# ViTAE-Transformer/LeMeViT

Measured on AMD Instinct MI355X. Metric: images/sec LeMeViT-Base 224^2 bf16 fwd+bwd, higher is better.
Workload: dtype bf16; 1 GPU; lemevit_base 224x224 bf16-autocast train step (fwd+bwd+AdamW), batch 128/GPU, drop_path 0.1, random-init weights; global_batch=128, parallelism=dp1, launch=eager, weight-gradient GEMMs on a side stream

## Files before the change

include/lemevit_hip.h:

```cpp
#ifndef LEMEVIT_HIP_H
#define LEMEVIT_HIP_H

#include <stddef.h>
#include <stdint.h>

#ifdef __cplusplus
extern "C" {
#endif

#define LMV_ABI_VERSION 14

enum { LMV_F32 = 0, LMV_BF16 = 1, LMV_U8 = 2  };
enum {
  LMV_OK = 0,
  LMV_ERR_SHAPE = -1,
  LMV_ERR_DTYPE = -2,
  LMV_ERR_WORKSPACE = -3,
  LMV_ERR_LAUNCH = -4
};

int lmv_abi_version(void);
const char* lmv_last_error(void);
int lmv_config_set(const char* key, int value);
int lmv_config_get(const char* key, int* value);

enum { LMV_ACT_NONE = 0, LMV_ACT_GELU = 1, LMV_ACT_GELU_GRAD = 2, LMV_ACT_GELU_BWD = 3 };

typedef struct {
  const void* a;
  const void* w;
  const float* bias;
  const void* res;
  const float* row_scale;
  const void* aux;
  void* out;
  void* out_pre;
  float* bias_grad;
  int64_t rows;
  int32_t rows_per_sample;
  int32_t _pad;
} lmv_linear_problem;

int lmv_linear_fwd(const lmv_linear_problem* p, int nproblems, int N, int K, int act, int dtype, void* stream);
int lmv_linear_dx(const lmv_linear_problem* p, int nproblems, int N, int K, int act, int dtype, void* stream);
size_t lmv_linear_dw_workspace_bytes(const lmv_linear_problem* p, int nproblems, int N, int K, int dtype);
int lmv_linear_dw(const lmv_linear_problem* p, int nproblems, int N, int K, void* workspace, size_t workspace_bytes, int dtype, void* stream);
#define LMV_REDUCE_MAX_SEGS 12
#define LMV_REDUCE_SLABS 0
#define LMV_REDUCE_ROWS  1
typedef struct {
  const float* ws;
  float* out_w;
  float* out_b;
  int64_t slab_stride;
  int64_t nw;
  int32_t nslabs, nb;
  int32_t kind, mode;
} lmv_reduce_seg;
int lmv_linear_dw_partial(const lmv_linear_problem* p, int nproblems, int N, int K, void* workspace, size_t workspace_bytes, int dtype, void* stream,
                          lmv_reduce_seg* segs, int* nsegs);
int lmv_reduce_batch(const lmv_reduce_seg* segs, int nsegs, void* stream);

int lmv_ln_fold(const float* w, const float* bias, const float* gamma, const float* beta, int N, int K, void* wf, float* colsum, float* bf,
                int dtype, void* stream);
int lmv_ln_linear_fwd(const lmv_linear_problem* p, int nproblems, int N, int K, float eps, int act, int dtype, void* stream);
typedef struct {
  const void* x;
  void* out;
  const float* row_scale;
  int64_t rows;
  int32_t rows_per_sample;
  int32_t _pad;
} lmv_mlp_problem;
typedef struct {
  const void* w1f; const float* colsum1; const float* b1f;
  const void* w2; const float* b2;
} lmv_mlp_weights;
int lmv_mlp_fused_supported(int C, int hidden, int dtype);
int lmv_gelu_poly_eval(const float* x, float* y, int64_t n, void* stream);
int lmv_mlp_fused_fwd(const lmv_mlp_problem* p, int nproblems, const lmv_mlp_weights* w, int C, int hidden, float eps, int dtype, void* stream);
typedef struct { const void* g; const void* u; void* dn2; int64_t rows; } lmv_mlp_dx_problem;
int lmv_mlp_dx_fused_supported(int C, int hidden, int dtype);
int lmv_mlp_dx_fused(const lmv_mlp_dx_problem* p, int nproblems, const void* fc2_wt, const void* fc1_wt, int C, int hidden, int dtype, void* stream);
int lmv_attn_out_proj_residual(const lmv_linear_problem* p, int nproblems, int C, int dtype, void* stream);

typedef struct {
  const void* x;
  void* y;
  float* stats;
  const void* dy;
  const void* dres;
  void* dx;
  int64_t rows;
  const float* dx_scale;
  void* dx_scaled;
  int64_t rows_per_sample;
} lmv_ln_segment;

int lmv_layernorm_fwd(const lmv_ln_segment* seg, int nseg, const float* gamma, const float* beta, int C, float eps,
                      int dtype, void* stream);
int lmv_layernorm_gelu_fwd(const lmv_ln_segment* seg, int nseg, const float* gamma, const float* beta, int C, float eps,
                           int dtype, void* stream);
int lmv_layernorm_gelu_bwd(const lmv_ln_segment* seg, int nseg, const float* gamma, const float* beta, float* dgamma, float* dbeta, int C,
                           void* workspace, size_t workspace_bytes, int dtype, void* stream);
size_t lmv_layernorm_bwd_workspace_bytes(int64_t total_rows, int C, int dtype);
int lmv_layernorm_bwd(const lmv_ln_segment* seg, int nseg, const float* gamma, float* dgamma, float* dbeta, int C,
                      void* workspace, size_t workspace_bytes, int dtype, void* stream);
int lmv_layernorm_bwd_partial(const lmv_ln_segment* seg, int nseg, const float* gamma, int C, void* workspace, size_t workspace_bytes,
                              int* partial_rows, int dtype, void* stream);
int lmv_layernorm_bwd_reduce(const void* workspace, int partial_rows, int C, float* dgamma, float* dbeta, void* stream);
int lmv_ln_linear_exact_fwd_supported(int N, int K, int dtype);
int lmv_ln_linear_exact_fwd(const lmv_linear_problem* p, const lmv_ln_segment* seg, int nproblems, int N, int K, const float* gamma, const float* beta,
                            float eps, int dtype, void* stream);
int lmv_linear_res_ln_fwd_supported(int N, int K, int dtype);
int lmv_linear_res_ln_fwd(const lmv_linear_problem* p, const lmv_ln_segment* seg, int nproblems, int N, int K, const float* gamma, const float* beta,
                          float eps, int dtype, void* stream);
int lmv_linear_dx_ln_bwd_supported(int C, int N, int dtype);
size_t lmv_linear_dx_ln_bwd_workspace_bytes(int64_t total_rows, int C);
int lmv_linear_dx_ln_bwd(const lmv_linear_problem* p, const lmv_ln_segment* seg, int nproblems, int C, int N, const float* gamma,
                         void* workspace, size_t workspace_bytes, int* partial_rows, int dtype, void* stream);

size_t lmv_batchnorm_workspace_bytes(int C);
int lmv_batchnorm_train_fwd(const void* x, const float* gamma, const float* beta, float* running_mean, float* running_var, float momentum,
                            float eps, int act, void* y, float* stats, int64_t rows, int C, void* workspace, size_t workspace_bytes,
                            int dtype, void* stream);
int lmv_batchnorm_train_bwd(const void* dy, const void* x, const float* gamma, const float* beta, const float* stats, int act, void* dx,
                            float* dgamma, float* dbeta, int64_t rows, int C, void* workspace, size_t workspace_bytes, int dtype,
                            void* stream);
int lmv_batchnorm_apply_fwd(const void* x, const float* gamma, const float* beta, const float* stats, int act, void* y, int64_t rows, int C,
                            int dtype, void* stream);

int lmv_dwconv3x3_residual_fwd(const void* x, const float* weight, const float* bias, void* y,
                               int B, int H, int W, int C, int dtype, void* stream);
int lmv_dwconv3x3_residual_bwd_data(const void* dy, const float* weight, void* dx,
                                    int B, int H, int W, int C, int dtype, void* stream);
size_t lmv_dwconv3x3_bwd_weight_workspace_bytes(int B, int H, int W, int C, int dtype);
int lmv_dwconv3x3_bwd_weight(const void* dy, const void* x, float* dweight, float* dbias,
                             int B, int H, int W, int C, void* workspace, size_t workspace_bytes, int dtype, void* stream);
int lmv_dwconv3x3_bwd_weight_partial(const void* dy, const void* x, int B, int H, int W, int C, void* workspace, size_t workspace_bytes,
                                     int* partial_rows, int dtype, void* stream);

typedef struct {
  const void* q; const void* k; const void* v;
  void* o;
  float* lse;
  const void* d_o;
  void* dq; void* dk; void* dv;
  int64_t q_bs, q_rs, k_bs, k_rs, v_bs, v_rs, o_bs, o_rs;
  int32_t B, H, Lq, Lk;
  float scale;
  int32_t _pad;
} lmv_attn_desc;

size_t lmv_attn_workspace_bytes(int B, int H, int Lq, int Lk, int backward);
int lmv_attn_fwd(const lmv_attn_desc* d, void* workspace, size_t workspace_bytes, int dtype, void* stream);
int lmv_attn_bwd(const lmv_attn_desc* d, void* workspace, size_t workspace_bytes, int dtype, void* stream);
int lmv_attn_fwd_pair(const lmv_attn_desc* d, void* workspace, size_t workspace_bytes, int dtype, void* stream);
int lmv_attn_bwd_pair(const lmv_attn_desc* d, void* workspace, size_t workspace_bytes, int dtype, void* stream);
int lmv_attn_probs(const lmv_attn_desc* d, float* p, int head_mean, int dtype, void* stream);

int lmv_sa_core_fwd(const void* qkv, void* o, float* lse, int B, int L, int C, void* ws, size_t ws_bytes, int dtype, void* stream);
int lmv_ca_core_fwd(const void* q, const void* kv, void* o, float* lse, int B, int M, int N, int C,
                    void* ws, size_t ws_bytes, int dtype, void* stream);
int lmv_dca_core_fwd(const void* qkv1, const void* qkv2, void* ox, void* oc, float* lse_x, float* lse_c,
                     int B, int N, int M, int C, void* ws, size_t ws_bytes, int dtype, void* stream);

int lmv_cast(const void* src, int src_dtype, void* dst, int dst_dtype, int64_t n, void* stream);
int lmv_im2col3x3s2_c3(const void* x, int x_dtype, void* patches, int dtype, int B, int H, int W, int64_t sb, int64_t sc, int64_t sh,
                       int64_t sw, void* stream);
int lmv_im2col3x3s2_nchw(const void* x, int x_dtype, void* patches, int dtype, int B, int Cin, int H, int W, int KP, int64_t sb, int64_t sc, int64_t sh, int64_t sw,
                         void* stream);
int lmv_conv3x3s2_nchw_dx(const void* dy, const void* wm, void* dx, int dx_dtype, int B, int Cin, int H, int W, int Co, int KP, int64_t sb, int64_t sc, int64_t sh,
                          int64_t sw, int dtype, void* stream);
int lmv_row_scale(const void* x, const float* scale, void* y, int64_t rows, int C, int rows_per_sample, int dtype, void* stream);
typedef struct lmv_row_scale_segment {
  const void* x; const float* scale; void* y;
  int64_t rows; int rows_per_sample;
} lmv_row_scale_segment;
int lmv_row_scale_multi(const lmv_row_scale_segment* seg, int nseg, int C, int dtype, void* stream);
#define LMV_TRANSPOSE_MAX_SEGS 48
typedef struct { const void* src; void* dst; int32_t rows, cols; } lmv_transpose_seg;
int lmv_transpose_batch(const lmv_transpose_seg* segs, int nsegs, int dtype, void* stream);
int lmv_im2col3x3s2_nhwc(const void* x, void* patches, int B, int H, int W, int C, int KP, int dtype, void* stream);
int lmv_col2im3x3s2_nhwc(const void* dpatches, void* dx, int B, int H, int W, int C, int KP, int dtype, void* stream);
int lmv_conv3x3s2_fwd(const void* x, const void* wm, const float* bias, void* y, int B, int H, int W, int Cin, int Cout, int KP, int act, int dtype, void* stream);
size_t lmv_conv3x3s2_dw_workspace_bytes(int B, int H, int W, int Cin, int Cout, int KP, int dtype);
int lmv_conv3x3s2_dw(const void* dy, const void* x, float* dwm, float* dbias, int B, int H, int W, int Cin, int Cout, int KP, void* workspace, size_t workspace_bytes, int dtype,
                     void* stream);
enum { LMV_FOLD_CI_TAP = 0, LMV_FOLD_TAP_CI = 1 };
int lmv_conv_bn_fold(const float* w, const float* b, const float* gamma, const float* beta, const float* mean, const float* var, float eps, int Co, int Cin, int KP,
                     int layout, void* wm, float* bf, float* sc, int dtype, void* stream);
int lmv_conv_bn_fold_bwd(const float* dwm, const float* dbf, const float* w, const float* b, const float* gamma, const float* mean, const float* var, float eps, int Co,
                         int Cin, int KP, int layout, float* dW, float* db, float* dgamma, float* dbeta, void* stream);
int lmv_token_mean2_fwd(const void* x, int L, const void* c, int M, int C, int B, void* out, int dtype, void* stream);
int lmv_token_mean2_bwd(const void* g, void* dx, int L, void* dc, int M, int C, int B, int dtype, void* stream);
int lmv_token_mean2_affine_fwd(const void* x, int L, const void* c, int M, int C, int B, const float* xscale, const float* xshift, void* out, int dtype,
                               void* stream);
int lmv_adamw_flat(float* param, const float* grad, float* exp_avg, float* exp_avg_sq, const float* wd_mask, void* shadow_bf16,
                   int64_t n, float lr, float beta1, float beta2, float eps, float weight_decay, int step, const int* step_dev,
                   void* stream);
typedef struct { const float* ptr; int64_t n; } lmv_norm_seg;
#define LMV_GRAD_STAT_FLOATS 8
#define LMV_NORM_CHUNK 16384
enum { LMV_NORM_SKIP_NONFINITE = 1 };
size_t lmv_grad_norm_workspace_bytes(const lmv_norm_seg* segs, int nsegs);
int lmv_grad_norm(const lmv_norm_seg* segs, int nsegs, float max_norm, int flags, float* stat, int* step_dev, void* ws, size_t ws_bytes,
                  void* stream);
int lmv_adamw_flat_clip(float* param, const float* grad, float* exp_avg, float* exp_avg_sq, const float* wd_mask, void* shadow_bf16,
                        int64_t n, float lr, float beta1, float beta2, float eps, float weight_decay, int step, const int* step_dev,
                        const float* stat, float clip_value, void* stream);
#define LMV_ADAMW_UNIT 8
#define LMV_ADAMW_MAX_GROUPS 256
typedef struct { float lr; float weight_decay; } lmv_adamw_group;
int lmv_adamw_flat_groups(float* param, const float* grad, float* exp_avg, float* exp_avg_sq, void* shadow_bf16, int64_t n,
                          const uint8_t* group_of_unit, const lmv_adamw_group* groups, int ngroups, float beta1, float beta2, float eps, int step,
                          const int* step_dev, const float* stat, float clip_value, void* stream);
int lmv_ema_flat(float* ema, const float* param, int64_t n, float decay, void* stream);

typedef struct lmv_mix_record { float w; int32_t yl, yh, xl, xh; float lam_t; } lmv_mix_record;
int lmv_mix_images(const void* x, int x_dtype, int64_t sb, int64_t sc, int64_t sh, int64_t sw, void* out, int out_dtype, int B, int C, int H, int W,
                   const lmv_mix_record* table, const lmv_mix_record* host_records, const float* scale, const float* shift, void* stream);
int lmv_soft_ce(const void* logits, int dtype, int64_t row_stride, int B, int N, const int64_t* labels, const lmv_mix_record* table, float smoothing,
                const void* target, int target_dtype, int64_t target_stride, float* row_loss, float* mean_loss, void* dlogits, void* stream);

#define LMV_ERASE_MAX_BOXES 4
enum { LMV_ERASE_CONST = 0, LMV_ERASE_RAND = 1, LMV_ERASE_PIXEL = 2 };
typedef struct lmv_erase_record { int32_t box[LMV_ERASE_MAX_BOXES][4]; } lmv_erase_record;
int lmv_augment_images(const void* x, int x_dtype, int64_t sb, int64_t sc, int64_t sh, int64_t sw, void* out, int out_dtype, int B, int C, int H, int W,
                       const lmv_mix_record* mix_table, const lmv_mix_record* host_records, const lmv_erase_record* erase_table, const uint32_t* erase_key,
                       int erase_mode, const lmv_erase_record* host_erase_records, const float* scale, const float* shift, void* stream);

enum { LMV_BLOCK_S = 0, LMV_BLOCK_D = 1, LMV_BLOCK_C = 2 };
enum { LMV_BLOCK_NO_JOIN = 1, LMV_BLOCK_FUSED = 2, LMV_BLOCK_DATA_ONLY = 4 };
typedef struct lmv_block_desc {
  int32_t kind, dtype, B, H, W, M, C, hidden;
  float eps;
// ... 80 lines not shown
```

lemevit_amd/_lib.py:

```python
from __future__ import annotations

import ctypes as C
import os

import torch

_HERE = os.path.dirname(os.path.abspath(__file__))
LIB_PATH = os.environ.get("LMV_LIB_PATH") or os.path.join(_HERE, "csrc", "liblemevit_hip.so")

LMV_F32, LMV_BF16, LMV_U8 = 0, 1, 2
ACT_NONE, ACT_GELU, ACT_GELU_GRAD, ACT_GELU_BWD = 0, 1, 2, 3
FOLD_CI_TAP, FOLD_TAP_CI = 0, 1
ABI_VERSION = 14
BLOCK_NO_JOIN, BLOCK_FUSED, BLOCK_DATA_ONLY = 1, 2, 4
GRAD_STAT_FLOATS, NORM_CHUNK, NORM_SKIP_NONFINITE = 8, 16384, 1
ADAMW_UNIT, ADAMW_MAX_GROUPS = 8, 256
ERASE_MAX_BOXES = 4
ERASE_CONST, ERASE_RAND, ERASE_PIXEL = 0, 1, 2


class LinearProblem(C.Structure):
    _fields_ = [("a", C.c_void_p), ("w", C.c_void_p), ("bias", C.c_void_p), ("res", C.c_void_p),
                ("row_scale", C.c_void_p), ("aux", C.c_void_p), ("out", C.c_void_p), ("out_pre", C.c_void_p),
                ("bias_grad", C.c_void_p), ("rows", C.c_int64), ("rows_per_sample", C.c_int32), ("_pad", C.c_int32)]


class MlpProblem(C.Structure):
    _fields_ = [("x", C.c_void_p), ("out", C.c_void_p), ("row_scale", C.c_void_p), ("rows", C.c_int64), ("rows_per_sample", C.c_int32), ("_pad", C.c_int32)]


class MlpDxProblem(C.Structure):
    _fields_ = [("g", C.c_void_p), ("u", C.c_void_p), ("dn2", C.c_void_p), ("rows", C.c_int64)]


class MlpWeights(C.Structure):
    _fields_ = [("w1f", C.c_void_p), ("colsum1", C.c_void_p), ("b1f", C.c_void_p), ("w2", C.c_void_p), ("b2", C.c_void_p)]


class ReduceSeg(C.Structure):
    _fields_ = [("ws", C.c_void_p), ("out_w", C.c_void_p), ("out_b", C.c_void_p), ("slab_stride", C.c_int64), ("nw", C.c_int64),
                ("nslabs", C.c_int32), ("nb", C.c_int32), ("kind", C.c_int32), ("mode", C.c_int32)]


class LnSegment(C.Structure):
    _fields_ = [("x", C.c_void_p), ("y", C.c_void_p), ("stats", C.c_void_p), ("dy", C.c_void_p), ("dres", C.c_void_p),
                ("dx", C.c_void_p), ("rows", C.c_int64), ("dx_scale", C.c_void_p), ("dx_scaled", C.c_void_p), ("rows_per_sample", C.c_int64)]


class RowScaleSegment(C.Structure):
    _fields_ = [("x", C.c_void_p), ("scale", C.c_void_p), ("y", C.c_void_p), ("rows", C.c_int64), ("rows_per_sample", C.c_int)]


class AttnDesc(C.Structure):
    _fields_ = [("q", C.c_void_p), ("k", C.c_void_p), ("v", C.c_void_p), ("o", C.c_void_p), ("lse", C.c_void_p),
                ("d_o", C.c_void_p), ("dq", C.c_void_p), ("dk", C.c_void_p), ("dv", C.c_void_p),
                ("q_bs", C.c_int64), ("q_rs", C.c_int64), ("k_bs", C.c_int64), ("k_rs", C.c_int64),
                ("v_bs", C.c_int64), ("v_rs", C.c_int64), ("o_bs", C.c_int64), ("o_rs", C.c_int64),
                ("B", C.c_int32), ("H", C.c_int32), ("Lq", C.c_int32), ("Lk", C.c_int32),
                ("scale", C.c_float), ("_pad", C.c_int32)]


class BlockDesc(C.Structure):
    _fields_ = ([(n, C.c_int32) for n in ("kind", "dtype", "B", "H", "W", "M", "C", "hidden")] + [("eps", C.c_float), ("flags", C.c_int32)] +
                [(n, C.c_void_p) for n in ("pos_w", "pos_b", "n1_w", "n1_b")] + [("attn_w", C.c_void_p * 4), ("attn_b", C.c_void_p * 4)] +
                [(n, C.c_void_p) for n in ("n2_w", "n2_b", "fc1_w", "fc1_b", "fc2_w", "fc2_b")] + [("masks", C.c_void_p * 4)] +
                [(n, C.c_void_p) for n in ("g_pos_w", "g_pos_b", "g_n1_w", "g_n1_b")] + [("g_attn_w", C.c_void_p * 4), ("g_attn_b", C.c_void_p * 4)] +
                [(n, C.c_void_p) for n in ("g_n2_w", "g_n2_b", "g_fc1_w", "g_fc1_b", "g_fc2_w", "g_fc2_b")] +
                [("fold_attn_w", C.c_void_p * 2), ("fold_attn_s", C.c_void_p * 2), ("fold_attn_b", C.c_void_p * 2)] +
                [(n, C.c_void_p) for n in ("fold_fc1_w", "fold_fc1_s", "fold_fc1_b", "fc2_wt", "fc1_wt")] + [("attn_wt", C.c_void_p * 2)])


class SStageBlockParams(C.Structure):
    _fields_ = ([(n, C.c_int32) for n in ("C", "heads", "hidden", "_pad")] +
                [(n, C.c_void_p) for n in ("qkv_w", "proj_w", "fc1_w", "fc2_w", "n1_w", "n1_b", "qkv_b", "proj_b", "n2_w", "n2_b", "fc1_b", "fc2_b", "pos_w", "pos_b")])


class SStageDesc(C.Structure):
    _fields_ = ([(n, C.c_int32) for n in ("B", "H", "W", "M", "C", "heads", "hidden", "nblocks", "dtype")] + [("eps", C.c_float), ("wpk", C.c_void_p), ("vec", C.c_void_p), ("timing", C.c_void_p), ("timing_block", C.c_int32), ("kind", C.c_int32)])


class DStageBlockParams(C.Structure):
    _fields_ = ([(n, C.c_int32) for n in ("C", "heads", "hidden", "_pad")] +
                [(n, C.c_void_p) for n in ("qkv1_w", "qkv2_w", "projx_w", "projc_w", "fc1_w", "fc2_w", "n1_w", "n1_b", "qkv1_b", "qkv2_b", "projx_b", "projc_b",
                                           "n2_w", "n2_b", "fc1_b", "fc2_b", "pos_w", "pos_b")])


class TransposeSeg(C.Structure):
    _fields_ = [("src", C.c_void_p), ("dst", C.c_void_p), ("rows", C.c_int32), ("cols", C.c_int32)]


class NormSeg(C.Structure):
    _fields_ = [("ptr", C.c_void_p), ("n", C.c_int64)]


class AdamWGroup(C.Structure):
    _fields_ = [("lr", C.c_float), ("weight_decay", C.c_float)]


class MixRecord(C.Structure):
    _fields_ = [("w", C.c_float), ("yl", C.c_int32), ("yh", C.c_int32), ("xl", C.c_int32), ("xh", C.c_int32), ("lam_t", C.c_float)]


class EraseRecord(C.Structure):
    _fields_ = [("box", (C.c_int32 * 4) * ERASE_MAX_BOXES)]


_P, _I, _L, _F, _Z = C.c_void_p, C.c_int, C.c_int64, C.c_float, C.c_size_t

SIGNATURES = {
    "lmv_abi_version": (_I, []),
    "lmv_config_set": (_I, [C.c_char_p, _I]),
    "lmv_config_get": (_I, [C.c_char_p, C.POINTER(C.c_int)]),
    "lmv_last_error": (C.c_char_p, []),
    "lmv_linear_fwd": (_I, [C.POINTER(LinearProblem), _I, _I, _I, _I, _I, _P]),
    "lmv_linear_dx": (_I, [C.POINTER(LinearProblem), _I, _I, _I, _I, _I, _P]),
    "lmv_linear_dw_workspace_bytes": (_Z, [C.POINTER(LinearProblem), _I, _I, _I, _I]),
    "lmv_linear_dw": (_I, [C.POINTER(LinearProblem), _I, _I, _I, _P, _Z, _I, _P]),
    "lmv_linear_dw_partial": (_I, [C.POINTER(LinearProblem), _I, _I, _I, _P, _Z, _I, _P, C.POINTER(ReduceSeg), C.POINTER(C.c_int)]),
    "lmv_reduce_batch": (_I, [C.POINTER(ReduceSeg), _I, _P]),
    "lmv_ln_fold": (_I, [_P, _P, _P, _P, _I, _I, _P, _P, _P, _I, _P]),
    "lmv_ln_linear_fwd": (_I, [C.POINTER(LinearProblem), _I, _I, _I, _F, _I, _I, _P]),
    "lmv_mlp_fused_supported": (_I, [_I, _I, _I]),
    "lmv_gelu_poly_eval": (_I, [_P, _P, C.c_int64, _P]),
    "lmv_mlp_fused_fwd": (_I, [C.POINTER(MlpProblem), _I, C.POINTER(MlpWeights), _I, _I, _F, _I, _P]),
    "lmv_mlp_dx_fused_supported": (_I, [_I, _I, _I]),
    "lmv_mlp_dx_fused": (_I, [C.POINTER(MlpDxProblem), _I, _P, _P, _I, _I, _I, _P]),
    "lmv_attn_out_proj_residual": (_I, [C.POINTER(LinearProblem), _I, _I, _I, _P]),
    "lmv_layernorm_fwd": (_I, [C.POINTER(LnSegment), _I, _P, _P, _I, _F, _I, _P]),
    "lmv_layernorm_gelu_fwd": (_I, [C.POINTER(LnSegment), _I, _P, _P, _I, _F, _I, _P]),
    "lmv_layernorm_gelu_bwd": (_I, [C.POINTER(LnSegment), _I, _P, _P, _P, _P, _I, _P, _Z, _I, _P]),
    "lmv_layernorm_bwd_workspace_bytes": (_Z, [_L, _I, _I]),
    "lmv_layernorm_bwd": (_I, [C.POINTER(LnSegment), _I, _P, _P, _P, _I, _P, _Z, _I, _P]),
    "lmv_layernorm_bwd_partial": (_I, [C.POINTER(LnSegment), _I, _P, _I, _P, _Z, C.POINTER(C.c_int), _I, _P]),
    "lmv_layernorm_bwd_reduce": (_I, [_P, _I, _I, _P, _P, _P]),
    "lmv_ln_linear_exact_fwd_supported": (_I, [_I, _I, _I]),
    "lmv_ln_linear_exact_fwd": (_I, [C.POINTER(LinearProblem), C.POINTER(LnSegment), _I, _I, _I, _P, _P, _F, _I, _P]),
    "lmv_linear_res_ln_fwd_supported": (_I, [_I, _I, _I]),
    "lmv_linear_res_ln_fwd": (_I, [C.POINTER(LinearProblem), C.POINTER(LnSegment), _I, _I, _I, _P, _P, _F, _I, _P]),
    "lmv_linear_dx_ln_bwd_supported": (_I, [_I, _I, _I]),
    "lmv_linear_dx_ln_bwd_workspace_bytes": (_Z, [_L, _I]),
    "lmv_linear_dx_ln_bwd": (_I, [C.POINTER(LinearProblem), C.POINTER(LnSegment), _I, _I, _I, _P, _P, _Z, C.POINTER(C.c_int), _I, _P]),
    "lmv_batchnorm_workspace_bytes": (_Z, [_I]),
    "lmv_batchnorm_train_fwd": (_I, [_P, _P, _P, _P, _P, _F, _F, _I, _P, _P, _L, _I, _P, _Z, _I, _P]),
    "lmv_batchnorm_train_bwd": (_I, [_P, _P, _P, _P, _P, _I, _P, _P, _P, _L, _I, _P, _Z, _I, _P]),
    "lmv_batchnorm_apply_fwd": (_I, [_P, _P, _P, _P, _I, _P, _L, _I, _I, _P]),
    "lmv_dwconv3x3_residual_fwd": (_I, [_P, _P, _P, _P, _I, _I, _I, _I, _I, _P]),
    "lmv_dwconv3x3_residual_bwd_data": (_I, [_P, _P, _P, _I, _I, _I, _I, _I, _P]),
    "lmv_dwconv3x3_bwd_weight_workspace_bytes": (_Z, [_I, _I, _I, _I, _I]),
    "lmv_dwconv3x3_bwd_weight": (_I, [_P, _P, _P, _P, _I, _I, _I, _I, _P, _Z, _I, _P]),
    "lmv_dwconv3x3_bwd_weight_partial": (_I, [_P, _P, _I, _I, _I, _I, _P, _Z, C.POINTER(C.c_int), _I, _P]),
    "lmv_attn_workspace_bytes": (_Z, [_I, _I, _I, _I, _I]),
    "lmv_attn_fwd": (_I, [C.POINTER(AttnDesc), _P, _Z, _I, _P]),
    "lmv_attn_bwd": (_I, [C.POINTER(AttnDesc), _P, _Z, _I, _P]),
    "lmv_attn_fwd_pair": (_I, [C.POINTER(AttnDesc), _P, _Z, _I, _P]),
    "lmv_attn_bwd_pair": (_I, [C.POINTER(AttnDesc), _P, _Z, _I, _P]),
    "lmv_attn_probs": (_I, [C.POINTER(AttnDesc), _P, _I, _I, _P]),
    "lmv_sa_core_fwd": (_I, [_P, _P, _P, _I, _I, _I, _P, _Z, _I, _P]),
    "lmv_ca_core_fwd": (_I, [_P, _P, _P, _P, _I, _I, _I, _I, _P, _Z, _I, _P]),
    "lmv_dca_core_fwd": (_I, [_P, _P, _P, _P, _P, _P, _I, _I, _I, _I, _P, _Z, _I, _P]),
    "lmv_cast": (_I, [_P, _I, _P, _I, _L, _P]),
    "lmv_im2col3x3s2_c3": (_I, [_P, _I, _P, _I, _I, _I, _I, _L, _L, _L, _L, _P]),
    "lmv_im2col3x3s2_nchw": (_I, [_P, _I, _P, _I, _I, _I, _I, _I, _I, _L, _L, _L, _L, _P]),
    "lmv_conv3x3s2_nchw_dx": (_I, [_P, _P, _P, _I, _I, _I, _I, _I, _I, _I, _L, _L, _L, _L, _I, _P]),
    "lmv_row_scale_multi": (_I, [_P, _I, _I, _I, _P]),
    "lmv_transpose_batch": (_I, [C.POINTER(TransposeSeg), _I, _I, _P]),
    "lmv_row_scale": (_I, [_P, _P, _P, _L, _I, _I, _I, _P]),
    "lmv_im2col3x3s2_nhwc": (_I, [_P, _P, _I, _I, _I, _I, _I, _I, _P]),
    "lmv_conv3x3s2_fwd": (_I, [_P, _P, _P, _P, _I, _I, _I, _I, _I, _I, _I, _I, _P]),
    "lmv_conv3x3s2_dw_workspace_bytes": (_Z, [_I, _I, _I, _I, _I, _I, _I]),
    "lmv_conv3x3s2_dw": (_I, [_P, _P, _P, _P, _I, _I, _I, _I, _I, _I, _P, _Z, _I, _P]),
    "lmv_conv_bn_fold": (_I, [_P, _P, _P, _P, _P, _P, _F, _I, _I, _I, _I, _P, _P, _P, _I, _P]),
    "lmv_conv_bn_fold_bwd": (_I, [_P, _P, _P, _P, _P, _P, _P, _F, _I, _I, _I, _I, _P, _P, _P, _P, _P]),
    "lmv_col2im3x3s2_nhwc": (_I, [_P, _P, _I, _I, _I, _I, _I, _I, _P]),
    "lmv_token_mean2_fwd": (_I, [_P, _I, _P, _I, _I, _I, _P, _I, _P]),
    "lmv_token_mean2_affine_fwd": (_I, [_P, _I, _P, _I, _I, _I, _P, _P, _P, _I, _P]),
    "lmv_token_mean2_bwd": (_I, [_P, _P, _I, _P, _I, _I, _I, _I, _P]),
    "lmv_adamw_flat": (_I, [_P, _P, _P, _P, _P, _P, _L, _F, _F, _F, _F, _F, _I, _P, _P]),
    "lmv_grad_norm_workspace_bytes": (_Z, [C.POINTER(NormSeg), _I]),
    "lmv_grad_norm": (_I, [C.POINTER(NormSeg), _I, _F, _I, _P, _P, _P, _Z, _P]),
    "lmv_adamw_flat_clip": (_I, [_P, _P, _P, _P, _P, _P, _L, _F, _F, _F, _F, _F, _I, _P, _P, _F, _P]),
    "lmv_adamw_flat_groups": (_I, [_P, _P, _P, _P, _P, _L, _P, _P, _I, _F, _F, _F, _I, _P, _P, _F, _P]),
    "lmv_ema_flat": (_I, [_P, _P, _L, _F, _P]),
    "lmv_mix_images": (_I, [_P, _I, _L, _L, _L, _L, _P, _I, _I, _I, _I, _I, _P, _P, _P, _P, _P]),
    "lmv_soft_ce": (_I, [_P, _I, _L, _I, _I, _P, _P, _F, _P, _I, _L, _P, _P, _P, _P]),
    "lmv_augment_images": (_I, [_P, _I, _L, _L, _L, _L, _P, _I, _I, _I, _I, _I, _P, _P, _P, _P, _I, _P, _P, _P, _P]),
    "lmv_block_arena_bytes": (_Z, [C.POINTER(BlockDesc)]),
    "lmv_block_bwd_scratch_bytes": (_Z, [C.POINTER(BlockDesc)]),
    "lmv_block_fwd": (_I, [C.POINTER(BlockDesc), _P, _P, _P, _P, _P, _Z, _I, _P]),
    "lmv_block_fwd_range": (_I, [C.POINTER(BlockDesc), _P, _P, _P, _P, _P, _Z, _I, _I, _I, _P]),
    "lmv_block_bwd": (_I, [C.POINTER(BlockDesc), _P, _P, _P, _Z, _P, _P, _P, _P, _P, _Z, _P, _P]),
    "lmv_block_fwd_scratch_bytes": (_Z, [C.POINTER(BlockDesc)]),
    "lmv_block_fwd_range_scratch": (_I, [C.POINTER(BlockDesc), _P, _P, _P, _P, _P, _Z, _I, _I, _I, _P, _Z, _P]),
    "lmv_debug_wgrad_launches": (C.c_longlong, []),
    "lmv_sstage_supported": (_I, [_I, _I, _I, _I, _I, _I, _I]),
    "lmv_sstage_wpk_bytes": (_Z, [_I, _I]),
    "lmv_sstage_vec_floats": (_Z, [_I, _I]),
    "lmv_sstage_workspace_bytes": (_Z, [_I, _I]),
    "lmv_sstage_max_images": (_I, [_I]),
    "lmv_sstage_max_concurrent": (_I, [_I]),
    "lmv_sstage_pack": (_I, [C.POINTER(SStageBlockParams), _P, _P, _P]),
    "lmv_sstage_fwd": (_I, [C.POINTER(SStageDesc), _P, _P, _P, _P, _P, _Z, _P]),
    "lmv_stem_supported": (_I, [_I, _I, _I, _I, _I]),
    "lmv_stem_wpk_bytes": (_Z, [_I, _I]),
    "lmv_stem_pack": (_I, [_P, _P, _I, _I, _I, _P, _P]),
    "lmv_stem_fwd": (_I, [_P, _I, _L, _L, _L, _L, _I, _I, _I, _I, _I, _P, _P, _P, _P, _P]),
    "lmv_stem_debug_timing": (None, [_P]),
    "lmv_stage_error_count": (_I, [_I]),
    "lmv_debug_stage_error_set": (_I, [_I]),
    "lmv_debug_launch_timing": (_I, [_I]),
    "lmv_debug_launch_timing_read": (_I, [_P, _P, _P, _P, _I]),
    "lmv_dstage_supported": (_I, [_I, _I, _I, _I, _I, _I, _I]),
    "lmv_dstage_wpk_bytes": (_Z, [_I, _I]),
    "lmv_dstage_vec_floats": (_Z, [_I, _I]),
    "lmv_dstage_workspace_bytes": (_Z, [_I, _I]),
    "lmv_dstage_max_concurrent": (_I, [_I, _I, _I]),
    "lmv_dstage_pack": (_I, [C.POINTER(DStageBlockParams), _P, _P, _P]),
    "lmv_dstage_fwd": (_I, [C.POINTER(SStageDesc), _P, _P, _P, _P, _P, _Z, _P]),
}


def _load():
    if not os.path.exists(LIB_PATH):
        raise RuntimeError(
            f"lemevit_amd: HIP kernel library not found at {LIB_PATH}. There is no CPU/PyTorch fallback; "
            "build it with `make -C lemevit_amd/csrc` (hipcc, --offload-arch=gfx950).")
    try:
        lib = C.CDLL(LIB_PATH)
    except OSError as e:
        raise RuntimeError(f"lemevit_amd: cannot load {LIB_PATH}: {e}") from e
    for name, (res, args) in SIGNATURES.items():
        fn = getattr(lib, name)
        fn.restype = res
        fn.argtypes = args
    v = lib.lmv_abi_version()
    if v != ABI_VERSION:
        raise RuntimeError(f"lemevit_amd: ABI version mismatch (library {v}, binding {ABI_VERSION}); rebuild csrc")
    return lib


lib = _load()


def config_set(key: str, value: int) -> None:
    if lib.lmv_config_set(key.encode(), int(value)):
        raise RuntimeError(f"lmv_config_set: {lib.lmv_last_error().decode(errors='replace')}")


def config_get(key: str) -> int:
    v = C.c_int(0)
    if lib.lmv_config_get(key.encode(), C.byref(v)):
        raise RuntimeError(f"lmv_config_get: {lib.lmv_last_error().decode(errors='replace')}")
    return int(v.value)


def check(rc: int, what: str) -> None:
    if rc != 0:
        raise RuntimeError(f"{what} failed (code {rc}): {lib.lmv_last_error().decode(errors='replace')}")
```

lemevit_amd/csrc/block.hip:

```cpp
#include <math.h>
#include <mutex>
#include "common.h"

namespace {

struct Bump {
  unsigned char* base; size_t off, cap;
  void* take(size_t n) {
    const size_t a = (off + 255) & ~(size_t)255;
    off = a + n;
    return base ? (void*)(base + a) : (void*)(uintptr_t)256;
  }
};

struct Dims {
  int kind, dtype, B, H, W, N, M, C, Hd, heads;
  size_t es;
  int64_t rows[2];
};

int dims_of(const lmv_block_desc* d, Dims* o) {
  if (!d) LMV_FAIL(LMV_ERR_SHAPE, "block: null descriptor");
  if (d->kind < LMV_BLOCK_S || d->kind > LMV_BLOCK_C) LMV_FAIL(LMV_ERR_SHAPE, "block: kind %d (0 = S, 1 = D, 2 = C)", d->kind);
  if (d->dtype != LMV_F32 && d->dtype != LMV_BF16) LMV_FAIL(LMV_ERR_DTYPE, "block: unsupported dtype %d", d->dtype);
  if (d->B <= 0 || d->H <= 0 || d->W <= 0 || d->M <= 0 || d->C <= 0 || (d->C % 32)) LMV_FAIL(LMV_ERR_SHAPE, "block: bad dims B=%d H=%d W=%d M=%d C=%d", d->B, d->H, d->W, d->M, d->C);
  o->kind = d->kind; o->dtype = d->dtype; o->B = d->B; o->H = d->H; o->W = d->W; o->N = d->H * d->W; o->M = d->M; o->C = d->C;
  o->Hd = d->hidden > 0 ? d->hidden : 4 * d->C; o->heads = d->C / 32;
  o->es = d->dtype == LMV_BF16 ? 2 : 4;
  o->rows[0] = (int64_t)d->B * o->N; o->rows[1] = (int64_t)d->B * d->M;
  return LMV_OK;
}

inline int proj_w(const Dims& D, int s) { return D.kind == LMV_BLOCK_C ? (s == 0 ? 2 * D.C : D.C) : 3 * D.C; }

struct Fwd {
  void *xp, *n1[2], *pj[2], *ao[2], *t2[2], *n2[2], *u[2], *h[2], *ws;
  float *st1[2], *lse[2], *st2[2];
  size_t ws_bytes;
};

inline size_t fwd_ws_attn(const Dims& D, int b) {
  size_t w, w2 = 0;
  if (D.kind == LMV_BLOCK_C) w = lmv_attn_workspace_bytes(b, D.heads, D.M, D.N, 0);
  else if (D.kind == LMV_BLOCK_D) { w = lmv_attn_workspace_bytes(b, D.heads, D.N, D.M, 0); w2 = lmv_attn_workspace_bytes(b, D.heads, D.M, D.N, 0); }
  else { w = lmv_attn_workspace_bytes(b, D.heads, D.N, D.N, 0); w2 = lmv_attn_workspace_bytes(b, D.heads, D.M, D.M, 0); }
  if (w2 > w) w = w2;
  return w < 256 ? 256 : w;
}
inline size_t fwd_ws_off(const Dims& D, int i0) { return i0 <= 0 ? 0 : fwd_ws_attn(D, i0) + (size_t)512 * i0; }
inline size_t fwd_ws_bytes(const Dims& D, int b) { return fwd_ws_attn(D, b) + (size_t)512 * b + 256; }

inline bool data_only(const lmv_block_desc* d) { return (d->flags & LMV_BLOCK_DATA_ONLY) != 0; }

void layout_transient(const Dims& D, Bump& t, Fwd* f) {
  const bool cb = D.kind == LMV_BLOCK_C;
  for (int s = 0; s < 2; ++s) {
    const bool has = !(cb && s == 0);
    f->n1[s] = t.take(D.rows[s] * D.C * D.es);
    f->n2[s] = has ? t.take(D.rows[s] * D.C * D.es) : nullptr;
    f->h[s] = has ? t.take(D.rows[s] * D.Hd * D.es) : nullptr;
  }
}

void layout_fwd(const Dims& D, Bump& a, Fwd* f, bool dataonly = false, Bump* tr = nullptr) {
  const bool cb = D.kind == LMV_BLOCK_C;
  if (dataonly) {
    for (int s = 0; s < 2; ++s) f->n1[s] = f->n2[s] = f->h[s] = nullptr;
    if (tr) layout_transient(D, *tr, f);
    f->xp = a.take(D.rows[0] * D.C * D.es);
    for (int s = 0; s < 2; ++s) {
      f->st1[s] = (float*)a.take(D.rows[s] * 2 * sizeof(float));
      f->pj[s] = a.take(D.rows[s] * proj_w(D, s) * D.es);
      const bool has = !(cb && s == 0);
      f->ao[s] = has ? a.take(D.rows[s] * D.C * D.es) : nullptr;
      f->lse[s] = has ? (float*)a.take((size_t)D.B * D.heads * (s == 0 ? D.N : D.M) * sizeof(float)) : nullptr;
      f->t2[s] = has ? a.take(D.rows[s] * D.C * D.es) : nullptr;
      f->st2[s] = has ? (float*)a.take(D.rows[s] * 2 * sizeof(float)) : nullptr;
      f->u[s] = has ? a.take(D.rows[s] * D.Hd * D.es) : nullptr;
    }
    f->ws_bytes = fwd_ws_bytes(D, D.B);
    f->ws = a.take(f->ws_bytes);
    return;
  }
  f->xp = a.take(D.rows[0] * D.C * D.es);
  for (int s = 0; s < 2; ++s) {
    f->n1[s] = a.take(D.rows[s] * D.C * D.es);
    f->st1[s] = (float*)a.take(D.rows[s] * 2 * sizeof(float));
    f->pj[s] = a.take(D.rows[s] * proj_w(D, s) * D.es);
    const bool has = !(cb && s == 0);
    f->ao[s] = has ? a.take(D.rows[s] * D.C * D.es) : nullptr;
    f->lse[s] = has ? (float*)a.take((size_t)D.B * D.heads * (s == 0 ? D.N : D.M) * sizeof(float)) : nullptr;
    f->t2[s] = has ? a.take(D.rows[s] * D.C * D.es) : nullptr;
    f->n2[s] = has ? a.take(D.rows[s] * D.C * D.es) : nullptr;
    f->st2[s] = has ? (float*)a.take(D.rows[s] * 2 * sizeof(float)) : nullptr;
    f->u[s] = has ? a.take(D.rows[s] * D.Hd * D.es) : nullptr;
    f->h[s] = has ? a.take(D.rows[s] * D.Hd * D.es) : nullptr;
  }
  f->ws_bytes = fwd_ws_bytes(D, D.B);
  f->ws = a.take(f->ws_bytes);
}

void attn_desc(lmv_attn_desc* a, const Dims& D, const void* q, int qw, int qo, const void* k, int kw, int ko, const void* v, int vw, int vo,
               void* o, float* lse, int Lq, int Lk, float scale) {
  *a = lmv_attn_desc{};
  a->q = (const unsigned char*)q + qo * D.es; a->k = (const unsigned char*)k + ko * D.es; a->v = (const unsigned char*)v + vo * D.es;
  a->o = o; a->lse = lse;
  a->q_bs = (int64_t)Lq * qw; a->q_rs = qw; a->k_bs = (int64_t)Lk * kw; a->k_rs = kw; a->v_bs = (int64_t)Lk * vw; a->v_rs = vw;
  a->o_bs = (int64_t)Lq * D.C; a->o_rs = D.C;
  a->B = D.B; a->H = D.heads; a->Lq = Lq; a->Lk = Lk; a->scale = scale;
}
void attn_grads(lmv_attn_desc* a, const Dims& D, const void* d_o, void* dq, int qo, void* dk, int ko, void* dv, int vo) {
  a->d_o = d_o;
  a->dq = (unsigned char*)dq + qo * D.es; a->dk = (unsigned char*)dk + ko * D.es; a->dv = (unsigned char*)dv + vo * D.es;
}

lmv_linear_problem prob(const void* a, const void* w, void* out, int64_t rows) {
  lmv_linear_problem p{};
  p.a = a; p.w = w; p.out = out; p.rows = rows;
  return p;
}

#define LMV_TRY(expr) do { const int rc__ = (expr); if (rc__) return rc__; } while (0)

const float SDPA_SCALE = 0.17677669529663687f;
inline void dca_scales(const Dims& D, float* sx, float* sc) {
  const double base = pow((double)D.C, -0.5);
  *sx = (float)(log((double)D.M) / log((double)D.N) * base);
  *sc = (float)base;
}

inline bool fused_on(const lmv_block_desc* d, const Dims& D, int save) {
  return (d->flags & LMV_BLOCK_FUSED) && !save && D.dtype == LMV_BF16 && d->fold_fc1_w && d->fold_fc1_s && d->fold_fc1_b && d->fold_attn_w[0] && d->fold_attn_s[0] &&
         d->fold_attn_b[0] && (D.kind == LMV_BLOCK_S || (d->fold_attn_w[1] && d->fold_attn_s[1] && d->fold_attn_b[1]));
}
inline bool fold_qkv(const Dims& D) { return D.C >= 192; }

inline bool mlp_split384(const Dims& D) { const int64_t r = D.rows[0] + D.rows[1]; return D.C == 384 && D.Hd == 1536 && r >= 16384 && r <= 65536; }
inline bool res_ln_ok(const lmv_block_desc* d, const Dims& D, int save) {
  if (D.kind != LMV_BLOCK_S || D.dtype != LMV_BF16 || D.rows[0] + D.rows[1] < 16384 || D.rows[0] + D.rows[1] > 32768) return false;
  if (!lmv_linear_res_ln_fwd_supported(D.C, D.C, D.dtype)) return false;
  return !(fused_on(d, D, save) && !mlp_split384(D));
}

int mlp_fwd(const lmv_block_desc* d, const Dims& D, const Fwd& f, int s0, void* const* outs, const float* const* ds, int save, void* st, bool ln_done = false) {
  const int ns = 2 - s0;
  const bool split384 = mlp_split384(D);
  if (fused_on(d, D, save) && !split384) {
    if (lmv_mlp_fused_supported(D.C, D.Hd, D.dtype)) {
      lmv_mlp_problem q[2] = {};
      for (int i = 0; i < ns; ++i) { const int s = s0 + i; q[i].x = f.t2[s]; q[i].out = outs[s]; q[i].row_scale = ds[s]; q[i].rows = D.rows[s]; q[i].rows_per_sample = s == 0 ? D.N : D.M; }
      lmv_mlp_weights w{d->fold_fc1_w, d->fold_fc1_s, d->fold_fc1_b, d->fc2_w, d->fc2_b};
      return lmv_mlp_fused_fwd(q, ns, &w, D.C, D.Hd, d->eps, D.dtype, st);
    }
    lmv_linear_problem p[2];
    for (int i = 0; i < ns; ++i) { const int s = s0 + i; p[i] = prob(f.t2[s], d->fold_fc1_w, f.h[s], D.rows[s]); p[i].bias = d->fold_fc1_b; p[i].aux = d->fold_fc1_s; }
    LMV_TRY(lmv_ln_linear_fwd(p, ns, D.Hd, D.C, d->eps, LMV_ACT_GELU, D.dtype, st));
    for (int i = 0; i < ns; ++i) {
      const int s = s0 + i;
      p[i] = prob(f.h[s], d->fc2_w, outs[s], D.rows[s]); p[i].bias = d->fc2_b; p[i].res = f.t2[s]; p[i].row_scale = ds[s];
      p[i].rows_per_sample = s == 0 ? D.N : D.M;
    }
    return lmv_linear_fwd(p, ns, D.C, D.Hd, LMV_ACT_NONE, D.dtype, st);
  }
  if (!ln_done) {
    lmv_ln_segment seg[2] = {};
    for (int i = 0; i < ns; ++i) { const int s = s0 + i; seg[i].x = f.t2[s]; seg[i].y = f.n2[s]; seg[i].stats = save ? f.st2[s] : nullptr; seg[i].rows = D.rows[s]; }
    LMV_TRY(lmv_layernorm_fwd(seg, ns, d->n2_w, d->n2_b, D.C, d->eps, D.dtype, st));
  }
  lmv_linear_problem p[2];
  for (int i = 0; i < ns; ++i) { const int s = s0 + i; p[i] = prob(f.n2[s], d->fc1_w, f.h[s], D.rows[s]); p[i].bias = d->fc1_b; p[i].out_pre = save ? f.u[s] : nullptr; }
  LMV_TRY(lmv_linear_fwd(p, ns, D.Hd, D.C, LMV_ACT_GELU, D.dtype, st));
  for (int i = 0; i < ns; ++i) {
    const int s = s0 + i;
    p[i] = prob(f.h[s], d->fc2_w, outs[s], D.rows[s]); p[i].bias = d->fc2_b; p[i].res = f.t2[s]; p[i].row_scale = ds[s];
    p[i].rows_per_sample = s == 0 ? D.N : D.M;
  }
  return lmv_linear_fwd(p, ns, D.C, D.Hd, LMV_ACT_NONE, D.dtype, st);
}

struct Side {
  hipStream_t main, side; hipEvent_t fork, join; bool used;
  void* ws; size_t ws_bytes;
  void* ws_tail; size_t ws_tail_bytes;
  lmv_reduce_seg segs[LMV_REDUCE_MAX_SEGS]; int nsegs = 0;
  bool dataonly = false;
  hipStream_t begin() {
    if (!side) return main;
    lmv_count_wgrad();
    (void)hipEventRecord(fork, main);
    (void)hipStreamWaitEvent(side, fork, 0);
    used = true;
    return side;
  }
  void finish() {
    if (side && used) { (void)hipEventRecord(join, side); (void)hipStreamWaitEvent(main, join, 0); used = false; }
  }
};

struct EventPool {
  std::mutex mu;
  hipEvent_t free_ev[64][32];
  int nfree[64] = {};
  int take(hipEvent_t* fork, hipEvent_t* join) {
    int dev = 0;
    (void)hipGetDevice(&dev);
    dev &= 63;
    hipEvent_t out[2];
    int got = 0;
    {
      std::lock_guard<std::mutex> lk(mu);
      while (got < 2 && nfree[dev] > 0) out[got++] = free_ev[dev][--nfree[dev]];
    }
    for (; got < 2; ++got)
      if (hipEventCreateWithFlags(&out[got], hipEventDisableTiming) != hipSuccess) {
        give(dev, out, got);
        LMV_FAIL(LMV_ERR_LAUNCH, "block_bwd: cannot create stream events");
      }
    *fork = out[0]; *join = out[1];
    return LMV_OK;
  }
  void give(int dev, const hipEvent_t* ev, int n) {
    std::lock_guard<std::mutex> lk(mu);
    for (int i = 0; i < n; ++i) {
      if (nfree[dev] < 32) free_ev[dev][nfree[dev]++] = ev[i];
      else (void)hipEventDestroy(ev[i]);
    }
  }
  void give(hipEvent_t fork, hipEvent_t join) {
    int dev = 0;
    (void)hipGetDevice(&dev);
    const hipEvent_t ev[2] = {fork, join};
    give(dev & 63, ev, 2);
  }
};
EventPool& event_pool() { static EventPool p; return p; }

int dw(Side& sd, const lmv_linear_problem* p, int np, int N, int K, int dtype) {
  lmv_count_wgrad();
  const size_t need = lmv_linear_dw_workspace_bytes(p, np, N, K, dtype);
  if (need > sd.ws_bytes) LMV_FAIL(LMV_ERR_WORKSPACE, "block_bwd: weight-gradient workspace %zu > %zu bytes", need, sd.ws_bytes);
  return lmv_linear_dw(p, np, N, K, sd.ws, sd.ws_bytes, dtype, sd.begin());
}
int flush_reduces(Side& sd) {
  if (!sd.nsegs) return LMV_OK;
  lmv_count_wgrad();
  const int rc = lmv_reduce_batch(sd.segs, sd.nsegs, sd.begin());
  sd.nsegs = 0;
  return rc;
}

struct Bwd {
  void *g[2], *du[2], *dn2[2], *dt2[2], *g2[2], *dao[2], *dpj[2], *dn1[2], *dxp, *ws_main, *ws_side, *ws_conv, *ws_ln[2];
  size_t ws_main_bytes, ws_side_bytes, ws_conv_bytes, ws_ln_bytes;
};

size_t max_dw_ws(const Dims& D) {
  const void* fake = (const void*)(uintptr_t)256;
  size_t m = 256;
  auto one = [&](int np, int64_t r0, int64_t r1, int N, int K, bool shared) {
    lmv_linear_problem p[2];
    float* o0 = (float*)(uintptr_t)256; float* o1 = shared ? o0 : (float*)(uintptr_t)512;
    p[0] = prob(fake, fake, o0, r0); p[0].bias_grad = (float*)(uintptr_t)1024;
    p[1] = prob(fake, fake, o1, r1); p[1].bias_grad = shared ? p[0].bias_grad : (float*)(uintptr_t)2048;
    const size_t w = lmv_linear_dw_workspace_bytes(p, np, N, K, D.dtype);
    if (w > m) m = w;
  };
  const int C = D.C, Hd = D.Hd;
  if (D.kind == LMV_BLOCK_C) {
    one(1, D.rows[1], 0, C, Hd, true); one(1, D.rows[1], 0, Hd, C, true);
    one(1, D.rows[1], 0, C, C, true); one(1, D.rows[1], 0, C, C, true); one(1, D.rows[0], 0, 2 * C, C, true);
  } else {
    const bool sh = D.kind == LMV_BLOCK_S;
    one(2, D.rows[0], D.rows[1], C, Hd, true); one(2, D.rows[0], D.rows[1], Hd, C, true);
    one(2, D.rows[0], D.rows[1], C, C, sh); one(2, D.rows[0], D.rows[1], 3 * C, C, sh);
  }
  return (m + 255) & ~(size_t)255;
}

void layout_bwd(const Dims& D, Bump& a, Bwd* b) {
  const bool cb = D.kind == LMV_BLOCK_C;
  for (int s = 0; s < 2; ++s) {
    const bool has = !(cb && s == 0);
    b->g[s] = has ? a.take(D.rows[s] * D.C * D.es) : nullptr;
    b->du[s] = has ? a.take(D.rows[s] * D.Hd * D.es) : nullptr;
    b->dn2[s] = has ? a.take(D.rows[s] * D.C * D.es) : nullptr;
    b->dt2[s] = has ? a.take(D.rows[s] * D.C * D.es) : nullptr;
    b->g2[s] = has ? a.take(D.rows[s] * D.C * D.es) : nullptr;
    b->dao[s] = has ? a.take(D.rows[s] * D.C * D.es) : nullptr;
    b->dpj[s] = a.take(D.rows[s] * proj_w(D, s) * D.es);
    b->dn1[s] = a.take(D.rows[s] * D.C * D.es);
  }
  b->dxp = a.take(D.rows[0] * D.C * D.es);
  size_t w = lmv_layernorm_bwd_workspace_bytes(D.rows[0] + D.rows[1], D.C, D.dtype);
  size_t w2;
  if (cb) w2 = lmv_attn_workspace_bytes(D.B, D.heads, D.M, D.N, 1);
  else if (D.kind == LMV_BLOCK_D) { w2 = lmv_attn_workspace_bytes(D.B, D.heads, D.N, D.M, 1); const size_t w3 = lmv_attn_workspace_bytes(D.B, D.heads, D.M, D.N, 1); if (w3 > w2) w2 = w3; }
  else { w2 = lmv_attn_workspace_bytes(D.B, D.heads, D.N, D.N, 1); const size_t w3 = lmv_attn_workspace_bytes(D.B, D.heads, D.M, D.M, 1); if (w3 > w2) w2 = w3; }
  if (w2 > w) w = w2;
  if (w < 256) w = 256;
  b->ws_main_bytes = w; b->ws_main = a.take(w);
  b->ws_side_bytes = max_dw_ws(D); b->ws_side = a.take(b->ws_side_bytes);
  b->ws_conv_bytes = lmv_dwconv3x3_bwd_weight_workspace_bytes(D.B, D.H, D.W, D.C, D.dtype); b->ws_conv = a.take(b->ws_conv_bytes);
  b->ws_ln_bytes = lmv_layernorm_bwd_workspace_bytes(D.rows[0] + D.rows[1], D.C, D.dtype);
  { const size_t w2 = lmv_linear_dx_ln_bwd_workspace_bytes(D.rows[0] + D.rows[1], D.C); if (w2 > b->ws_ln_bytes) b->ws_ln_bytes = w2; }
  for (int i = 0; i < 2; ++i) b->ws_ln[i] = a.take(b->ws_ln_bytes);
}

int ln_bwd(Side& sd, const lmv_ln_segment* seg, int nseg, const float* gamma, float* dgamma, float* dbeta, const Dims& D, void* ws, size_t ws_bytes) {
  if (sd.dataonly) return lmv_layernorm_bwd_partial(seg, nseg, gamma, D.C, nullptr, 0, nullptr, D.dtype, sd.main);
  int rows = 0;
  LMV_TRY(lmv_layernorm_bwd_partial(seg, nseg, gamma, D.C, ws, ws_bytes, &rows, D.dtype, sd.main));
  if (sd.nsegs + 1 > LMV_REDUCE_MAX_SEGS) LMV_FAIL(LMV_ERR_WORKSPACE, "block_bwd: too many deferred reductions");
  lmv_reduce_seg& sg = sd.segs[sd.nsegs++];
  sg = lmv_reduce_seg{};
  sg.ws = (const float*)ws; sg.out_w = dgamma; sg.out_b = dbeta; sg.slab_stride = 2 * D.C; sg.nw = D.C; sg.nslabs = rows; sg.nb = D.C;
  sg.kind = LMV_REDUCE_ROWS; sg.mode = 0;
  return LMV_OK;
}

inline bool dx_ln_fused_ok(const Dims& D, const void* wt, int N) {
  const int64_t rows = D.rows[0] + D.rows[1];
  return wt && D.dtype == LMV_BF16 && lmv_linear_dx_ln_bwd_supported(D.C, N, D.dtype) && rows >= 16384 && rows <= 32768;
}
int dx_ln_bwd(Side& sd, const lmv_linear_problem* p, const lmv_ln_segment* seg, int nseg, int N, const float* gamma, float* dgamma, float* dbeta, const Dims& D,
              void* ws, size_t ws_bytes) {
  if (sd.dataonly) return lmv_linear_dx_ln_bwd(p, seg, nseg, D.C, N, gamma, nullptr, 0, nullptr, D.dtype, sd.main);
  int rows = 0;
  LMV_TRY(lmv_linear_dx_ln_bwd(p, seg, nseg, D.C, N, gamma, ws, ws_bytes, &rows, D.dtype, sd.main));
  if (sd.nsegs + 1 > LMV_REDUCE_MAX_SEGS) LMV_FAIL(LMV_ERR_WORKSPACE, "block_bwd: too many deferred reductions");
  lmv_reduce_seg& sg = sd.segs[sd.nsegs++];
  sg = lmv_reduce_seg{};
  sg.ws = (const float*)ws; sg.out_w = dgamma; sg.out_b = dbeta; sg.slab_stride = 2 * D.C; sg.nw = D.C; sg.nslabs = rows; sg.nb = D.C;
  sg.kind = LMV_REDUCE_ROWS; sg.mode = 0;
  return LMV_OK;
}

inline bool mlp_dx_fused_on(const lmv_block_desc* d, const Dims& D) {
  const int mode = lmv_config().mlp_dx_fused;
  if (mode == 0 || D.dtype != LMV_BF16 || !d->fc2_wt || !d->fc1_wt || !lmv_mlp_dx_fused_supported(D.C, D.Hd, D.dtype)) return false;
  return mode == 2;
}

int mlp_bwd(const lmv_block_desc* d, const Dims& D, const Fwd& f, const Bwd& b, int s0, const void* const* douts, const float* const* ds, const float* const* nds,
            const void** g2_out, Side& sd) {
  const int ns = 2 - s0;
  hipStream_t st = sd.main;
  const void* g[2];
  lmv_row_scale_segment rs[2]; int nrs = 0;
  for (int s = s0; s < 2; ++s) {
    g[s] = douts[s];
    if (ds[s]) { rs[nrs].x = douts[s]; rs[nrs].scale = ds[s]; rs[nrs].y = b.g[s]; rs[nrs].rows = D.rows[s]; rs[nrs].rows_per_sample = s == 0 ? D.N : D.M; ++nrs; g[s] = b.g[s]; }
  }
  if (nrs) LMV_TRY(lmv_row_scale_multi(rs, nrs, D.C, D.dtype, st));
  lmv_linear_problem p[2];
  lmv_ln_segment seg[2] = {};
  for (int i = 0; i < ns; ++i) {
    const int s = s0 + i;
    seg[i].x = f.t2[s]; seg[i].dy = b.dn2[s]; seg[i].stats = f.st2[s]; seg[i].dres = douts[s]; seg[i].dx = b.dt2[s]; seg[i].rows = D.rows[s];
    g2_out[s] = b.dt2[s];
    if (nds && nds[s]) { seg[i].dx_scale = nds[s]; seg[i].dx_scaled = b.g2[s]; seg[i].rows_per_sample = s == 0 ? D.N : D.M; g2_out[s] = b.g2[s]; }
  }
  if (sd.dataonly && mlp_dx_fused_on(d, D)) {
    lmv_mlp_dx_problem q[2] = {};
    for (int i = 0; i < ns; ++i) { const int s = s0 + i; q[i].g = g[s]; q[i].u = f.u[s]; q[i].dn2 = b.dn2[s]; q[i].rows = D.rows[s]; }
    LMV_TRY(lmv_mlp_dx_fused(q, ns, d->fc2_wt, d->fc1_wt, D.C, D.Hd, D.dtype, st));
    return ln_bwd(sd, seg, ns, d->n2_w, d->g_n2_w, d->g_n2_b, D, b.ws_ln[0], b.ws_ln_bytes);
  }
  if (!sd.dataonly) {
    for (int i = 0; i < ns; ++i) { const int s = s0 + i; p[i] = prob(g[s], f.h[s], d->g_fc2_w, D.rows[s]); p[i].bias_grad = d->g_fc2_b; }
    LMV_TRY(dw(sd, p, ns, D.C, D.Hd, D.dtype));
  }
  if (d->fc2_wt && D.dtype == LMV_BF16) {
    for (int i = 0; i < ns; ++i) { const int s = s0 + i; p[i] = prob(g[s], d->fc2_wt, b.du[s], D.rows[s]); p[i].aux = f.u[s]; }
    LMV_TRY(lmv_linear_fwd(p, ns, D.Hd, D.C, LMV_ACT_GELU_GRAD, D.dtype, st));
  } else {
    for (int i = 0; i < ns; ++i) { const int s = s0 + i; p[i] = prob(g[s], d->fc2_w, b.du[s], D.rows[s]); p[i].aux = f.u[s]; }
    LMV_TRY(lmv_linear_dx(p, ns, D.C, D.Hd, LMV_ACT_GELU_GRAD, D.dtype, st));
  }
  if (!sd.dataonly) {
    for (int i = 0; i < ns; ++i) { const int s = s0 + i; p[i] = prob(b.du[s], f.n2[s], d->g_fc1_w, D.rows[s]); p[i].bias_grad = d->g_fc1_b; }
    LMV_TRY(dw(sd, p, ns, D.Hd, D.C, D.dtype));
  }
  const bool fuse2 = dx_ln_fused_ok(D, d->fc1_wt, D.Hd);
  if (fuse2) {
  } else if (d->fc1_wt && D.dtype == LMV_BF16) {
    for (int i = 0; i < ns; ++i) { const int s = s0 + i; p[i] = prob(b.du[s], d->fc1_wt, b.dn2[s], D.rows[s]); }
    LMV_TRY(lmv_linear_fwd(p, ns, D.C, D.Hd, LMV_ACT_NONE, D.dtype, st));
  } else {
    for (int i = 0; i < ns; ++i) { const int s = s0 + i; p[i] = prob(b.du[s], d->fc1_w, b.dn2[s], D.rows[s]); }
    LMV_TRY(lmv_linear_dx(p, ns, D.Hd, D.C, LMV_ACT_NONE, D.dtype, st));
  }
  if (fuse2) {
    for (int i = 0; i < ns; ++i) { const int s = s0 + i; p[i] = prob(b.du[s], d->fc1_wt, b.dn2[s], D.rows[s]); }
    return dx_ln_bwd(sd, p, seg, ns, D.Hd, d->n2_w, d->g_n2_w, d->g_n2_b, D, b.ws_ln[0], b.ws_ln_bytes);
  }
  return ln_bwd(sd, seg, ns, d->n2_w, d->g_n2_w, d->g_n2_b, D, b.ws_ln[0], b.ws_ln_bytes);
}

int check_ptrs(const lmv_block_desc* d, bool grads) {
  const void* need[] = {d->pos_w, d->pos_b, d->n1_w, d->n1_b, d->attn_w[0], d->attn_b[0], d->attn_w[1], d->attn_b[1], d->n2_w, d->n2_b, d->fc1_w, d->fc1_b, d->fc2_w, d->fc2_b};
  for (const void* p : need) if (!p) LMV_FAIL(LMV_ERR_SHAPE, "block: null parameter pointer");
  if (d->kind != LMV_BLOCK_S && (!d->attn_w[2] || !d->attn_b[2])) LMV_FAIL(LMV_ERR_SHAPE, "block: null parameter pointer");
  if (d->kind == LMV_BLOCK_D && (!d->attn_w[3] || !d->attn_b[3])) LMV_FAIL(LMV_ERR_SHAPE, "block: null parameter pointer");
  if (grads) {
    const void* gn[] = {d->g_pos_w, d->g_pos_b, d->g_n1_w, d->g_n1_b, d->g_attn_w[0], d->g_attn_b[0], d->g_attn_w[1], d->g_attn_b[1], d->g_n2_w, d->g_n2_b, d->g_fc1_w, d->g_fc1_b,
                        d->g_fc2_w, d->g_fc2_b};
    for (const void* p : gn) if (!p) LMV_FAIL(LMV_ERR_SHAPE, "block_bwd: null gradient pointer");
    if (d->kind != LMV_BLOCK_S && (!d->g_attn_w[2] || !d->g_attn_b[2])) LMV_FAIL(LMV_ERR_SHAPE, "block_bwd: null gradient pointer");
    if (d->kind == LMV_BLOCK_D && (!d->g_attn_w[3] || !d->g_attn_b[3])) LMV_FAIL(LMV_ERR_SHAPE, "block_bwd: null gradient pointer");
  }
  return LMV_OK;
}

}

extern "C" size_t lmv_block_arena_bytes(const lmv_block_desc* d) {
  Dims D;
  if (dims_of(d, &D)) return 0;
  Bump a{nullptr, 0, 0};
  Fwd f;
  layout_fwd(D, a, &f, data_only(d));
  return a.off + 256;
}

extern "C" size_t lmv_block_fwd_scratch_bytes(const lmv_block_desc* d) {
  Dims D;
  if (dims_of(d, &D)) return 0;
  Bump t{nullptr, 0, 0};
  Fwd f;
  layout_transient(D, t, &f);
  return t.off + 256;
}

extern "C" size_t lmv_block_bwd_scratch_bytes(const lmv_block_desc* d) {
  Dims D;
  if (dims_of(d, &D)) return 0;
  Bump a{nullptr, 0, 0};
  Bwd b;
  layout_bwd(D, a, &b);
  return a.off + 256;
}

namespace {
int block_fwd_body(const lmv_block_desc* d, const Dims& D, const Fwd& f, const void* x, const void* c, void* x_out, void* c_out, int save, void* stream);
}

extern "C" int lmv_block_fwd_range(const lmv_block_desc* d, const void* x, const void* c, void* x_out, void* c_out, void* arena, size_t arena_bytes, int save,
                                   int image0, int nimages, void* stream) {
  return lmv_block_fwd_range_scratch(d, x, c, x_out, c_out, arena, arena_bytes, save, image0, nimages, nullptr, 0, stream);
}

extern "C" int lmv_block_fwd_range_scratch(const lmv_block_desc* d, const void* x, const void* c, void* x_out, void* c_out, void* arena, size_t arena_bytes, int save,
                                           int image0, int nimages, void* scratch, size_t scratch_bytes, void* stream) {
  Dims DF;
  LMV_TRY(dims_of(d, &DF));
  LMV_TRY(check_ptrs(d, false));
  const bool cb = DF.kind == LMV_BLOCK_C;
  if (!x || !c || !c_out || (!cb && !x_out) || !arena || !lmv_aligned16(arena)) LMV_FAIL(LMV_ERR_SHAPE, "block_fwd: null / misaligned tensor");
  if (image0 < 0 || nimages <= 0 || image0 + nimages > DF.B) LMV_FAIL(LMV_ERR_SHAPE, "block_fwd: images [%d, %d) outside the batch of %d", image0, image0 + nimages, DF.B);
  const bool dataonly = data_only(d);
  if (dataonly && (!scratch || !lmv_aligned16(scratch))) LMV_FAIL(LMV_ERR_SHAPE, "block_fwd: LMV_BLOCK_DATA_ONLY needs the transient buffer of lmv_block_fwd_range_scratch");
  Bump a{(unsigned char*)arena, 0, arena_bytes};
  Bump t{(unsigned char*)scratch, 0, scratch_bytes};
  Fwd f;
  layout_fwd(DF, a, &f, dataonly, &t);
  if (a.off > arena_bytes) LMV_FAIL(LMV_ERR_WORKSPACE, "block_fwd: arena %zu < %zu bytes", arena_bytes, a.off);
  if (dataonly && t.off > scratch_bytes) LMV_FAIL(LMV_ERR_WORKSPACE, "block_fwd: transient buffer %zu < %zu bytes", scratch_bytes, t.off);
  if (image0 == 0 && nimages == DF.B) return block_fwd_body(d, DF, f, x, c, x_out, c_out, save, stream);
  lmv_block_desc dr = *d;
  dr.B = nimages;
  for (int k = 0; k < 4; ++k) if (dr.masks[k]) dr.masks[k] += image0;
  Dims D;
  LMV_TRY(dims_of(&dr, &D));
  const size_t es = D.es;
  auto adv = [&](void* ptr, int s, size_t width_bytes) -> void* { return ptr ? (void*)((unsigned char*)ptr + (size_t)image0 * (s == 0 ? D.N : D.M) * width_bytes) : nullptr; };
  f.xp = adv(f.xp, 0, D.C * es);
  for (int s = 0; s < 2; ++s) {
    f.n1[s] = adv(f.n1[s], s, D.C * es); f.st1[s] = (float*)adv(f.st1[s], s, 2 * sizeof(float)); f.pj[s] = adv(f.pj[s], s, proj_w(D, s) * es);
    f.ao[s] = adv(f.ao[s], s, D.C * es); f.lse[s] = (float*)adv(f.lse[s], s, D.heads * sizeof(float)); f.t2[s] = adv(f.t2[s], s, D.C * es);
    f.n2[s] = adv(f.n2[s], s, D.C * es); f.st2[s] = (float*)adv(f.st2[s], s, 2 * sizeof(float)); f.u[s] = adv(f.u[s], s, D.Hd * es); f.h[s] = adv(f.h[s], s, D.Hd * es);
  }
  const size_t w0 = fwd_ws_off(DF, image0), w1 = fwd_ws_attn(DF, nimages);
  if (w0 + w1 > f.ws_bytes) LMV_FAIL(LMV_ERR_WORKSPACE, "block_fwd: attention workspace slice [%zu, %zu) outside %zu bytes", w0, w0 + w1, f.ws_bytes);
  f.ws = (unsigned char*)f.ws + w0; f.ws_bytes = w1;
  return block_fwd_body(&dr, D, f, adv(const_cast<void*>(x), 0, D.C * es), adv(const_cast<void*>(c), 1, D.C * es), adv(x_out, 0, D.C * es), adv(c_out, 1, D.C * es), save, stream);
}

extern "C" int lmv_block_fwd(const lmv_block_desc* d, const void* x, const void* c, void* x_out, void* c_out, void* arena, size_t arena_bytes, int save, void* stream) {
  return lmv_block_fwd_range(d, x, c, x_out, c_out, arena, arena_bytes, save, 0, d ? d->B : 0, stream);
}

namespace {

int block_fwd_body(const lmv_block_desc* d, const Dims& D, const Fwd& f, const void* x, const void* c, void* x_out, void* c_out, int save, void* stream) {
  const bool cb = D.kind == LMV_BLOCK_C;
  const int C = D.C, N = D.N, M = D.M;
  LMV_TRY(lmv_dwconv3x3_residual_fwd(x, d->pos_w, d->pos_b, f.xp, D.B, D.H, D.W, C, D.dtype, stream));
  const bool fq = fused_on(d, D, save) && fold_qkv(D);
  const bool ex = !fq && D.dtype == LMV_BF16 && D.kind != LMV_BLOCK_S &&
                  lmv_ln_linear_exact_fwd_supported(cb ? 2 * D.C : 3 * D.C, D.C, D.dtype) && lmv_ln_linear_exact_fwd_supported(D.C, D.C, D.dtype);
  const void* src[2] = {f.xp, c};
  if (!fq && !ex) {
    lmv_ln_segment seg[2] = {};
    seg[0].x = f.xp; seg[0].y = f.n1[0]; seg[0].stats = save ? f.st1[0] : nullptr; seg[0].rows = D.rows[0];
    seg[1].x = c; seg[1].y = f.n1[1]; seg[1].stats = save ? f.st1[1] : nullptr; seg[1].rows = D.rows[1];
    LMV_TRY(lmv_layernorm_fwd(seg, 2, d->n1_w, d->n1_b, C, d->eps, D.dtype, stream));
    src[0] = f.n1[0]; src[1] = f.n1[1];
  }
  auto project = [&](lmv_linear_problem* p, int np, const int* streams, const int* slots, int width) -> int {
    for (int i = 0; i < np; ++i) {
      const int s = streams[i], k = slots[i];
      p[i] = prob(src[s], fq ? d->fold_attn_w[k] : d->attn_w[k], f.pj[s], D.rows[s]);
      p[i].bias = fq ? d->fold_attn_b[k] : d->attn_b[k];
      if (fq) p[i].aux = d->fold_attn_s[k];
    }
    if (ex) {
      lmv_ln_segment seg[2] = {};
      for (int i = 0; i < np; ++i) { const int s = streams[i]; seg[i].y = save ? f.n1[s] : nullptr; seg[i].stats = save ? f.st1[s] : nullptr; seg[i].rows = D.rows[s]; }
      return lmv_ln_linear_exact_fwd(p, seg, np, width, C, d->n1_w, d->n1_b, d->eps, D.dtype, stream);
    }
    return fq ? lmv_ln_linear_fwd(p, np, width, C, d->eps, LMV_ACT_NONE, D.dtype, stream) : lmv_linear_fwd(p, np, width, C, LMV_ACT_NONE, D.dtype, stream);
  };
  lmv_linear_problem p[2];
  lmv_attn_desc ad[2];
  void* outs[2] = {x_out, c_out};
  bool ln2_done = false;
  if (D.kind == LMV_BLOCK_S) {
    { const int st_[2] = {0, 1}, sl_[2] = {0, 0}; LMV_TRY(project(p, 2, st_, sl_, 3 * C)); }
    for (int s = 0; s < 2; ++s) { const int L = s == 0 ? N : M; attn_desc(&ad[s], D, f.pj[s], 3 * C, 0, f.pj[s], 3 * C, C, f.pj[s], 3 * C, 2 * C, f.ao[s], save ? f.lse[s] : nullptr, L, L, SDPA_SCALE); }
    LMV_TRY(lmv_attn_fwd_pair(ad, f.ws, f.ws_bytes, D.dtype, stream));
    for (int s = 0; s < 2; ++s) {
      p[s] = prob(f.ao[s], d->attn_w[1], f.t2[s], D.rows[s]); p[s].bias = d->attn_b[1]; p[s].res = s == 0 ? f.xp : c;
      p[s].row_scale = d->masks[s == 0 ? 0 : 2]; p[s].rows_per_sample = s == 0 ? N : M;
    }
    if (res_ln_ok(d, D, save)) {
      lmv_ln_segment seg[2] = {};
      for (int s = 0; s < 2; ++s) { seg[s].y = f.n2[s]; seg[s].stats = save ? f.st2[s] : nullptr; seg[s].rows = D.rows[s]; }
      LMV_TRY(lmv_linear_res_ln_fwd(p, seg, 2, C, C, d->n2_w, d->n2_b, d->eps, D.dtype, stream));
      ln2_done = true;
    } else {
      LMV_TRY(lmv_linear_fwd(p, 2, C, C, LMV_ACT_NONE, D.dtype, stream));
    }
  } else if (D.kind == LMV_BLOCK_D) {
    float sx, sc;
    dca_scales(D, &sx, &sc);
    { const int st_[2] = {0, 1}, sl_[2] = {0, 1}; LMV_TRY(project(p, 2, st_, sl_, 3 * C)); }
    attn_desc(&ad[0], D, f.pj[0], 3 * C, 0, f.pj[1], 3 * C, C, f.pj[1], 3 * C, 2 * C, f.ao[0], save ? f.lse[0] : nullptr, N, M, sx);
    attn_desc(&ad[1], D, f.pj[1], 3 * C, 0, f.pj[0], 3 * C, C, f.pj[0], 3 * C, 2 * C, f.ao[1], save ? f.lse[1] : nullptr, M, N, sc);
    LMV_TRY(lmv_attn_fwd(&ad[0], f.ws, f.ws_bytes, D.dtype, stream));
    LMV_TRY(lmv_attn_fwd(&ad[1], f.ws, f.ws_bytes, D.dtype, stream));
    for (int s = 0; s < 2; ++s) {
      p[s] = prob(f.ao[s], d->attn_w[2 + s], f.t2[s], D.rows[s]); p[s].bias = d->attn_b[2 + s]; p[s].res = s == 0 ? f.xp : c;
      p[s].row_scale = d->masks[s == 0 ? 0 : 2]; p[s].rows_per_sample = s == 0 ? N : M;
    }
    LMV_TRY(lmv_linear_fwd(p, 2, C, C, LMV_ACT_NONE, D.dtype, stream));
  } else {
    { const int st_[1] = {0}, sl_[1] = {1}; LMV_TRY(project(p, 1, st_, sl_, 2 * C)); }
    { const int st_[1] = {1}, sl_[1] = {0}; LMV_TRY(project(p, 1, st_, sl_, C)); }
    attn_desc(&ad[0], D, f.pj[1], C, 0, f.pj[0], 2 * C, 0, f.pj[0], 2 * C, C, f.ao[1], save ? f.lse[1] : nullptr, M, N, SDPA_SCALE);
    LMV_TRY(lmv_attn_fwd(&ad[0], f.ws, f.ws_bytes, D.dtype, stream));
    p[0] = prob(f.ao[1], d->attn_w[2], f.t2[1], D.rows[1]); p[0].bias = d->attn_b[2]; p[0].res = c; p[0].row_scale = d->masks[0]; p[0].rows_per_sample = M;
    LMV_TRY(lmv_linear_fwd(p, 1, C, C, LMV_ACT_NONE, D.dtype, stream));
  }
  const float* ds[2] = {cb ? nullptr : d->masks[1], cb ? d->masks[1] : d->masks[3]};
  return mlp_fwd(d, D, f, cb ? 1 : 0, outs, ds, save, stream, ln2_done);
}

}

extern "C" int lmv_block_bwd(const lmv_block_desc* d, const void* x, const void* c, const void* arena, size_t arena_bytes, const void* dx_out, const void* dc_out, void* dx, void* dc,
                             void* scratch, size_t scratch_bytes, void* stream, void* side_stream) {
  Dims D;
  LMV_TRY(dims_of(d, &D));
  const bool dataonly = data_only(d);
  LMV_TRY(check_ptrs(d, !dataonly));
  const bool cb = D.kind == LMV_BLOCK_C;
  if (dataonly) side_stream = nullptr;
  if ((!x && !dataonly) || !c || !arena || !dc_out || (!cb && !dx_out) || !dx || !dc || !scratch || !lmv_aligned16(scratch)) LMV_FAIL(LMV_ERR_SHAPE, "block_bwd: null / misaligned tensor");
  Bump a{(unsigned char*)const_cast<void*>(arena), 0, arena_bytes};
  Fwd f;
  layout_fwd(D, a, &f, dataonly);
  if (a.off > arena_bytes) LMV_FAIL(LMV_ERR_WORKSPACE, "block_bwd: arena %zu < %zu bytes", arena_bytes, a.off);
  Bump s{(unsigned char*)scratch, 0, scratch_bytes};
  Bwd b;
  layout_bwd(D, s, &b);
  if (s.off > scratch_bytes) LMV_FAIL(LMV_ERR_WORKSPACE, "block_bwd: scratch %zu < %zu bytes", scratch_bytes, s.off);
  Side sd{};
  sd.main = (hipStream_t)stream; sd.side = (hipStream_t)side_stream; sd.ws = b.ws_side; sd.ws_bytes = b.ws_side_bytes;
  sd.ws_tail = b.ws_conv; sd.ws_tail_bytes = b.ws_conv_bytes;
  sd.dataonly = dataonly;
  if (side_stream) LMV_TRY(event_pool().take(&sd.fork, &sd.join));
  hipStream_t st = sd.main;
  const int C = D.C, N = D.N, M = D.M;
  lmv_linear_problem p[2];
  lmv_attn_desc ad[2];
  const void* g2[2] = {nullptr, nullptr};
  int rc = LMV_OK;
  auto body = [&]() -> int {
    if (cb) {
      const void* douts[2] = {nullptr, dc_out};
      const float* ds[2] = {nullptr, d->masks[1]};
      LMV_TRY(mlp_bwd(d, D, f, b, 1, douts, ds, nullptr, g2, sd));
      const void* dc1 = b.dt2[1];
      const void* g = dc1;
      if (d->masks[0]) { LMV_TRY(lmv_row_scale(dc1, d->masks[0], b.g2[1], D.rows[1], C, M, D.dtype, st)); g = b.g2[1]; }
      if (!dataonly) {
        p[0] = prob(g, f.ao[1], d->g_attn_w[2], D.rows[1]); p[0].bias_grad = d->g_attn_b[2];
        LMV_TRY(dw(sd, p, 1, C, C, D.dtype));
      }
      p[0] = prob(g, d->attn_w[2], b.dao[1], D.rows[1]);
      LMV_TRY(lmv_linear_dx(p, 1, C, C, LMV_ACT_NONE, D.dtype, st));
      attn_desc(&ad[0], D, f.pj[1], C, 0, f.pj[0], 2 * C, 0, f.pj[0], 2 * C, C, f.ao[1], f.lse[1], M, N, SDPA_SCALE);
      attn_grads(&ad[0], D, b.dao[1], b.dpj[1], 0, b.dpj[0], 0, b.dpj[0], C);
      LMV_TRY(lmv_attn_bwd(&ad[0], b.ws_main, b.ws_main_bytes, D.dtype, st));
      if (!dataonly) {
        p[0] = prob(b.dpj[1], f.n1[1], d->g_attn_w[0], D.rows[1]); p[0].bias_grad = d->g_attn_b[0];
        LMV_TRY(dw(sd, p, 1, C, C, D.dtype));
        p[0] = prob(b.dpj[0], f.n1[0], d->g_attn_w[1], D.rows[0]); p[0].bias_grad = d->g_attn_b[1];
        LMV_TRY(dw(sd, p, 1, 2 * C, C, D.dtype));
      }
      p[0] = prob(b.dpj[1], d->attn_w[0], b.dn1[1], D.rows[1]);
      LMV_TRY(lmv_linear_dx(p, 1, C, C, LMV_ACT_NONE, D.dtype, st));
      p[0] = prob(b.dpj[0], d->attn_w[1], b.dn1[0], D.rows[0]);
      LMV_TRY(lmv_linear_dx(p, 1, 2 * C, C, LMV_ACT_NONE, D.dtype, st));
      lmv_ln_segment seg[2] = {};
      seg[0].x = c; seg[0].dy = b.dn1[1]; seg[0].stats = f.st1[1]; seg[0].dres = dc1; seg[0].dx = dc; seg[0].rows = D.rows[1];
      seg[1].x = f.xp; seg[1].dy = b.dn1[0]; seg[1].stats = f.st1[0]; seg[1].dres = nullptr; seg[1].dx = b.dxp; seg[1].rows = D.rows[0];
      LMV_TRY(ln_bwd(sd, seg, 2, d->n1_w, d->g_n1_w, d->g_n1_b, D, b.ws_ln[1], b.ws_ln_bytes));
    } else {
      const void* douts[2] = {dx_out, dc_out};
      const float* ds[2] = {d->masks[1], d->masks[3]};
      const float* nds[2] = {d->masks[0], d->masks[2]};
      LMV_TRY(mlp_bwd(d, D, f, b, 0, douts, ds, nds, g2, sd));
      const bool sh = D.kind == LMV_BLOCK_S;
      if (!dataonly) {
        for (int s2 = 0; s2 < 2; ++s2) { p[s2] = prob(g2[s2], f.ao[s2], sh ? d->g_attn_w[1] : d->g_attn_w[2 + s2], D.rows[s2]); p[s2].bias_grad = sh ? d->g_attn_b[1] : d->g_attn_b[2 + s2]; }
        LMV_TRY(dw(sd, p, 2, C, C, D.dtype));
// ... 68 lines not shown
```

lemevit_amd/csrc/common.h:

```cpp
#pragma once
#include <hip/hip_runtime.h>
#include <stdint.h>
#include <stdio.h>
#include "../../include/lemevit_hip.h"

typedef unsigned short bf16_t;
typedef __attribute__((ext_vector_type(8))) __bf16 bf16x8_t;
typedef __attribute__((ext_vector_type(4))) __bf16 bf16x4_t;
typedef __attribute__((ext_vector_type(4))) float f32x4_t;

#define LMV_WAVE 64

void lmv_set_error(const char* fmt, ...);
#define LMV_FAIL(code, ...)          \
  do {                               \
    lmv_set_error(__VA_ARGS__);      \
    return (code);                   \
  } while (0)
unsigned* lmv_stage_errword(void* stream);
int lmv_stage_capacity(const void* kernel, int threads, size_t lds_bytes);

extern bool g_lmv_timing_on;
void lmv_timing_begin(void* stream, double flops, double bytes, int kind);
void lmv_timing_end(void* stream);
void lmv_timing_set_kind(int kind);
enum { LMV_TK_GEMM_NT = 0, LMV_TK_SSTAGE = 1, LMV_TK_DSTAGE = 2, LMV_TK_STEM = 3, LMV_TK_GEMM_DX = 4, LMV_TK_GEMM_DW = 5, LMV_TK_SPLITK_REDUCE = 6, LMV_TK_ATTN_FWD = 7,
       LMV_TK_RS_GEMM = 8, LMV_TK_WN_GEMM = 9, LMV_TK_ATTN_BWD = 10, LMV_TK_RSW_GEMM = 11, LMV_TK_MLP_DX = 12 };
struct LmvTimedLaunch {
  void* st; bool on;
  LmvTimedLaunch(void* stream, double flops, double bytes, int kind = 0) : st(stream), on(g_lmv_timing_on) { if (on) lmv_timing_begin(st, flops, bytes, kind); }
  void kind(int k) { if (on) lmv_timing_set_kind(k); }
  ~LmvTimedLaunch() { if (on) lmv_timing_end(st); }
};
void lmv_count_wgrad();
#define LMV_CHECK_LAUNCH(name)                                                \
  do {                                                                        \
    hipError_t e__ = hipGetLastError();                                       \
    if (e__ != hipSuccess) LMV_FAIL(LMV_ERR_LAUNCH, "%s: %s", name, hipGetErrorString(e__)); \
  } while (0)

int lmv_launch_partial_reduce(const float* partial, int nrows, int width, float* out_a, int na, float* out_b, int mode, hipStream_t st);

static __device__ __forceinline__ void lmv_partial_reduce_block(float4* red, int blk, const float* __restrict__ partial, int nrows, int width,
                                                                float* __restrict__ out_a, int na, float* __restrict__ out_b, int mode) {
  const int cx = threadIdx.x & 7, rg = threadIdx.x >> 3, i = (blk * 8 + cx) * 4;
  float4 a = make_float4(0.f, 0.f, 0.f, 0.f);
  if (i < width) {
    const float* p = partial + i;
    int r = rg;
    for (; r + 96 < nrows; r += 128) {
      const float4 v0 = *reinterpret_cast<const float4*>(p + (int64_t)r * width);
      const float4 v1 = *reinterpret_cast<const float4*>(p + (int64_t)(r + 32) * width);
      const float4 v2 = *reinterpret_cast<const float4*>(p + (int64_t)(r + 64) * width);
      const float4 v3 = *reinterpret_cast<const float4*>(p + (int64_t)(r + 96) * width);
      a.x += (v0.x + v1.x) + (v2.x + v3.x); a.y += (v0.y + v1.y) + (v2.y + v3.y);
      a.z += (v0.z + v1.z) + (v2.z + v3.z); a.w += (v0.w + v1.w) + (v2.w + v3.w);
    }
    for (; r < nrows; r += 32) {
      const float4 v = *reinterpret_cast<const float4*>(p + (int64_t)r * width);
      a.x += v.x; a.y += v.y; a.z += v.z; a.w += v.w;
    }
  }
  red[rg * 8 + cx] = a;
  __syncthreads();
  if (rg == 0 && i < width) {
#pragma unroll 8
    for (int k = 1; k < 32; ++k) { const float4 v = red[k * 8 + cx]; a.x += v.x; a.y += v.y; a.z += v.z; a.w += v.w; }
    const float s[4] = {a.x, a.y, a.z, a.w};
#pragma unroll
    for (int e = 0; e < 4; ++e) {
      const int j = i + e;
      if (mode == 0) { if (j < na) out_a[j] += s[e]; else out_b[j - na] += s[e]; }
      else { const int t = j / na, ch = j - t * na; if (t < 9) out_a[ch * 9 + t] += s[e]; else out_b[ch] += s[e]; }
    }
  }
}

struct LmvConfig {
  int gemm_rs = 1;
  int gemm_wn = 1;
  int mlp_rw96 = 1;
  int mlp_tm = 0;
  int mlp_dx_fused = 1;
  int stage_ticket_skew = 0;
};
LmvConfig& lmv_config();

bool lmv_rs_eligible(const lmv_linear_problem* p, int nproblems, int N, int K, int act, bool force);
int lmv_rs_linear(const lmv_linear_problem* p, int nproblems, int N, int K, int act, hipStream_t st);
bool lmv_wn_eligible(const lmv_linear_problem* p, int nproblems, int N, int K, int act, bool force);
bool lmv_mlp_rw96_eligible(const lmv_mlp_problem* p, int nproblems, int C, int hidden);
int lmv_mlp_rw96_fwd(const lmv_mlp_problem* p, int nproblems, const lmv_mlp_weights* w, float eps, hipStream_t st);
int lmv_wn_linear(const lmv_linear_problem* p, int nproblems, int N, int K, int act, hipStream_t st);
int lmv_gelu_bwd_linear(const lmv_linear_problem* p, int nproblems, int N, int K, int dtype, hipStream_t st);

static inline bool lmv_aligned16(const void* p) { return (((uintptr_t)p) & 15u) == 0; }

__device__ __forceinline__ float bf2f(bf16_t v) { return __uint_as_float(((unsigned)v) << 16); }
typedef __attribute__((ext_vector_type(2))) __bf16 bf16x2_t;
typedef __attribute__((ext_vector_type(2))) float f32x2_t;
__device__ __forceinline__ unsigned pack_bf2(float lo, float hi) {
  const f32x2_t f = {lo, hi};
  return __builtin_bit_cast(unsigned, __builtin_convertvector(f, bf16x2_t));
}
__device__ __forceinline__ bf16_t f2bf(float f) { return (bf16_t)(pack_bf2(f, 0.f) & 0xffffu); }

template <typename T> struct DT;
template <> struct DT<float> {
  static constexpr int EPC = 4;
  static __device__ __forceinline__ float ld(const float* p) { return *p; }
  static __device__ __forceinline__ void st(float* p, float v) { *p = v; }
};
template <> struct DT<bf16_t> {
  static constexpr int EPC = 8;
  static __device__ __forceinline__ float ld(const bf16_t* p) { return bf2f(*p); }
  static __device__ __forceinline__ void st(bf16_t* p, float v) { *p = f2bf(v); }
};

template <typename T> __device__ __forceinline__ void chunk_to_f(const uint4& c, float* f);
template <> __device__ __forceinline__ void chunk_to_f<float>(const uint4& c, float* f) {
  f[0] = __uint_as_float(c.x); f[1] = __uint_as_float(c.y); f[2] = __uint_as_float(c.z); f[3] = __uint_as_float(c.w);
}
template <> __device__ __forceinline__ void chunk_to_f<bf16_t>(const uint4& c, float* f) {
  f[0] = __uint_as_float(c.x << 16); f[1] = __uint_as_float(c.x & 0xffff0000u);
  f[2] = __uint_as_float(c.y << 16); f[3] = __uint_as_float(c.y & 0xffff0000u);
  f[4] = __uint_as_float(c.z << 16); f[5] = __uint_as_float(c.z & 0xffff0000u);
  f[6] = __uint_as_float(c.w << 16); f[7] = __uint_as_float(c.w & 0xffff0000u);
}
template <typename T> __device__ __forceinline__ uint4 f_to_chunk(const float* f);
template <> __device__ __forceinline__ uint4 f_to_chunk<float>(const float* f) {
  return make_uint4(__float_as_uint(f[0]), __float_as_uint(f[1]), __float_as_uint(f[2]), __float_as_uint(f[3]));
}
template <> __device__ __forceinline__ uint4 f_to_chunk<bf16_t>(const float* f) {
  return make_uint4(pack_bf2(f[0], f[1]), pack_bf2(f[2], f[3]), pack_bf2(f[4], f[5]), pack_bf2(f[6], f[7]));
}

__device__ __forceinline__ void ld4(const float* p, float* f) {
  float4 v = *reinterpret_cast<const float4*>(p); f[0] = v.x; f[1] = v.y; f[2] = v.z; f[3] = v.w;
}
__device__ __forceinline__ void ld4(const bf16_t* p, float* f) {
  uint2 v = *reinterpret_cast<const uint2*>(p);
  f[0] = __uint_as_float(v.x << 16); f[1] = __uint_as_float(v.x & 0xffff0000u);
  f[2] = __uint_as_float(v.y << 16); f[3] = __uint_as_float(v.y & 0xffff0000u);
}
__device__ __forceinline__ void st4(float* p, const float* f) { *reinterpret_cast<float4*>(p) = make_float4(f[0], f[1], f[2], f[3]); }
__device__ __forceinline__ void st4(bf16_t* p, const float* f) { *reinterpret_cast<uint2*>(p) = make_uint2(pack_bf2(f[0], f[1]), pack_bf2(f[2], f[3])); }

__device__ __forceinline__ float gelu_f(float x) { return 0.5f * x * (1.0f + erff(x * 0.70710678118654752f)); }
__device__ __forceinline__ float gelu_grad_f(float x) {
  return 0.5f * (1.0f + erff(x * 0.70710678118654752f)) + x * 0.39894228040143268f * expf(-0.5f * x * x);
}
__device__ __forceinline__ void erf_as(float x, float* erfv, float* gauss) {
  const float z = fabsf(x) * 0.70710678118654752f;
  const float t = __builtin_amdgcn_rcpf(1.0f + 0.3275911f * z);
  const float ex = __expf(-z * z);
  const float poly = t * (0.254829592f + t * (-0.284496736f + t * (1.421413741f + t * (-1.453152027f + t * 1.061405429f))));
  *erfv = copysignf(1.0f - poly * ex, x);
  *gauss = ex;
}
__device__ __forceinline__ float gelu_fast_f(float x) { float e, g; erf_as(x, &e, &g); return 0.5f * x * (1.0f + e); }
__device__ __forceinline__ float gelu_grad_fast_f(float x) {
  float e, g; erf_as(x, &e, &g);
  return 0.5f * (1.0f + e) + x * 0.39894228040143268f * g;
}

__device__ __forceinline__ f32x2_t gelu_poly2(f32x2_t x) {
  f32x2_t s = x * 0.25f;
  s[0] = __builtin_amdgcn_fmed3f(s[0], -1.0f, 1.0f); s[1] = __builtin_amdgcn_fmed3f(s[1], -1.0f, 1.0f);
  const f32x2_t u = s * s;
  f32x2_t q = {-1.6300047636032104f, -1.6300047636032104f};
  q = __builtin_elementwise_fma(q, u, f32x2_t{7.93373966217041f, 7.93373966217041f});
  q = __builtin_elementwise_fma(q, u, f32x2_t{-16.877059936523438f, -16.877059936523438f});
  q = __builtin_elementwise_fma(q, u, f32x2_t{20.921268463134766f, 20.921268463134766f});
  q = __builtin_elementwise_fma(q, u, f32x2_t{-17.09065055847168f, -17.09065055847168f});
  q = __builtin_elementwise_fma(q, u, f32x2_t{9.8812894821167f, 9.8812894821167f});
  q = __builtin_elementwise_fma(q, u, f32x2_t{-4.233964920043945f, -4.233964920043945f});
  q = __builtin_elementwise_fma(q, u, f32x2_t{1.595382571220398f, 1.595382571220398f});
  const f32x2_t phi = __builtin_elementwise_fma(s, q, f32x2_t{0.5f, 0.5f});
  return x * phi;
}

__device__ __forceinline__ float lmv_xsum4(float v) {
  auto r = __builtin_amdgcn_permlane16_swap(__float_as_uint(v), __float_as_uint(v), false, false);
  v = __uint_as_float(r[0]) + __uint_as_float(r[1]);
  auto q = __builtin_amdgcn_permlane32_swap(__float_as_uint(v), __float_as_uint(v), false, false);
  return __uint_as_float(q[0]) + __uint_as_float(q[1]);
}
__device__ __forceinline__ float lmv_xmax4(float v) {
  auto r = __builtin_amdgcn_permlane16_swap(__float_as_uint(v), __float_as_uint(v), false, false);
  v = fmaxf(__uint_as_float(r[0]), __uint_as_float(r[1]));
  auto q = __builtin_amdgcn_permlane32_swap(__float_as_uint(v), __float_as_uint(v), false, false);
  return fmaxf(__uint_as_float(q[0]), __uint_as_float(q[1]));
}
__device__ __forceinline__ float wave_sum(float v) {
#pragma unroll
  for (int o = 32; o > 0; o >>= 1) v += __shfl_xor(v, o, 64);
  return v;
}
__device__ __forceinline__ float wave_max(float v) {
#pragma unroll
  for (int o = 32; o > 0; o >>= 1) v = fmaxf(v, __shfl_xor(v, o, 64));
  return v;
}
```

lemevit_amd/csrc/misc.hip:

```cpp
#include <stdarg.h>
#include <string.h>
#include <atomic>
#include <mutex>
#include <vector>
#include "common.h"

static thread_local char g_err[512] = "";

void lmv_set_error(const char* fmt, ...) {
  va_list ap;
  va_start(ap, fmt);
  vsnprintf(g_err, sizeof(g_err), fmt, ap);
  va_end(ap);
}
extern "C" const char* lmv_last_error(void) { return g_err; }

namespace {
struct ErrWord { unsigned* host = nullptr; unsigned* dev = nullptr; };
ErrWord g_errword[64];
std::mutex g_errword_mu;
}
unsigned* lmv_stage_errword(void* stream) {
  int dev = 0;
  (void)hipGetDevice(&dev);
  std::lock_guard<std::mutex> lock(g_errword_mu);
  ErrWord& w = g_errword[dev & 63];
  if (!w.dev) {
    if (stream) {
      hipStreamCaptureStatus cs = hipStreamCaptureStatusNone;
      if (hipStreamIsCapturing((hipStream_t)stream, &cs) == hipSuccess && cs != hipStreamCaptureStatusNone) return nullptr;
    }
    void* h = nullptr; void* d = nullptr;
    if (hipHostMalloc(&h, 256, hipHostMallocMapped) != hipSuccess) return nullptr;
    memset(h, 0, 256);
    if (hipHostGetDevicePointer(&d, h, 0) != hipSuccess) { (void)hipHostFree(h); return nullptr; }
    w.host = (unsigned*)h; w.dev = (unsigned*)d;
  }
  return w.dev;
}
extern "C" int lmv_stage_error_count(int reset) {
  if (!lmv_stage_errword(nullptr)) LMV_FAIL(LMV_ERR_LAUNCH, "stage_error_count: cannot allocate the error word");
  int dev = 0;
  (void)hipGetDevice(&dev);
  volatile unsigned* h = g_errword[dev & 63].host;
  const unsigned v = *h;
  if (reset && v) *h = 0;
  return (int)(v & 0x7fffffffu);
}
extern "C" int lmv_debug_stage_error_set(int value) {
  if (!lmv_stage_errword(nullptr)) LMV_FAIL(LMV_ERR_LAUNCH, "debug_stage_error_set: cannot allocate the error word");
  int dev = 0;
  (void)hipGetDevice(&dev);
  *(volatile unsigned*)g_errword[dev & 63].host = (unsigned)value;
  return LMV_OK;
}
int lmv_stage_capacity(const void* kernel, int threads, size_t lds_bytes) {
  int dev = 0, cus = 0, per_cu = 0;
  (void)hipGetDevice(&dev);
  if (hipDeviceGetAttribute(&cus, hipDeviceAttributeMultiprocessorCount, dev) != hipSuccess || cus <= 0) return 0;
  if (hipOccupancyMaxActiveBlocksPerMultiprocessor(&per_cu, kernel, threads, lds_bytes) != hipSuccess || per_cu <= 0) return 0;
  return cus * per_cu;
}

bool g_lmv_timing_on = false;
namespace {
struct TimingRec { hipEvent_t e0, e1; double flops, bytes; int kind; };
std::vector<TimingRec> g_timing;
size_t g_timing_n = 0;
}
void lmv_timing_begin(void* stream, double flops, double bytes, int kind) {
  if (g_timing_n >= g_timing.size()) return;
  TimingRec& r = g_timing[g_timing_n];
  r.flops = flops; r.bytes = bytes; r.kind = kind;
  (void)hipEventRecord(r.e0, (hipStream_t)stream);
}
void lmv_timing_end(void* stream) {
  if (g_timing_n >= g_timing.size()) return;
  (void)hipEventRecord(g_timing[g_timing_n++].e1, (hipStream_t)stream);
}
void lmv_timing_set_kind(int kind) {
  if (g_timing_n < g_timing.size()) g_timing[g_timing_n].kind = kind;
}
extern "C" int lmv_debug_launch_timing(int capacity) {
  g_lmv_timing_on = false;
  for (auto& r : g_timing) { (void)hipEventDestroy(r.e0); (void)hipEventDestroy(r.e1); }
  g_timing.clear(); g_timing_n = 0;
  if (capacity <= 0) return LMV_OK;
  g_timing.resize((size_t)capacity);
  for (auto& r : g_timing)
    if (hipEventCreate(&r.e0) != hipSuccess || hipEventCreate(&r.e1) != hipSuccess) LMV_FAIL(LMV_ERR_LAUNCH, "launch timing: cannot create events");
  g_lmv_timing_on = true;
  return LMV_OK;
}
extern "C" int lmv_debug_launch_timing_read(float* ms, double* flops, double* bytes, int* kinds, int capacity) {
  g_lmv_timing_on = false;
  int n = 0;
  for (size_t i = 0; i < g_timing_n && n < capacity; ++i) {
    float t = 0.f;
    if (hipEventElapsedTime(&t, g_timing[i].e0, g_timing[i].e1) != hipSuccess) continue;
    ms[n] = t; flops[n] = g_timing[i].flops; bytes[n] = g_timing[i].bytes; kinds[n] = g_timing[i].kind; ++n;
  }
  return n;
}

namespace { std::atomic<long long> g_wgrad_launches{0}; }
void lmv_count_wgrad() { g_wgrad_launches.fetch_add(1, std::memory_order_relaxed); }
extern "C" long long lmv_debug_wgrad_launches(void) { return g_wgrad_launches.load(std::memory_order_relaxed); }

extern "C" int lmv_abi_version(void) { return LMV_ABI_VERSION; }

namespace {
struct ConfigKey { const char* key; int LmvConfig::*field; };
const ConfigKey kConfigKeys[] = {
    {"gemm_rs", &LmvConfig::gemm_rs}, {"gemm_wn", &LmvConfig::gemm_wn}, {"mlp_rw96", &LmvConfig::mlp_rw96}, {"mlp_tm", &LmvConfig::mlp_tm}, {"mlp_dx_fused", &LmvConfig::mlp_dx_fused},
    {"stage_ticket_skew", &LmvConfig::stage_ticket_skew},
};
LmvConfig g_config;
}
LmvConfig& lmv_config() { return g_config; }
extern "C" int lmv_config_set(const char* key, int value) {
  if (!key) LMV_FAIL(LMV_ERR_SHAPE, "config_set: null key");
  for (const ConfigKey& k : kConfigKeys)
    if (!strcmp(k.key, key)) { g_config.*(k.field) = value; return LMV_OK; }
  LMV_FAIL(LMV_ERR_SHAPE, "config_set: unknown key '%s'", key);
}
extern "C" int lmv_config_get(const char* key, int* value) {
  if (!key || !value) LMV_FAIL(LMV_ERR_SHAPE, "config_get: null argument");
  for (const ConfigKey& k : kConfigKeys)
    if (!strcmp(k.key, key)) { *value = g_config.*(k.field); return LMV_OK; }
  LMV_FAIL(LMV_ERR_SHAPE, "config_get: unknown key '%s'", key);
}

namespace {

constexpr int TPB = 256;
inline int grid_for(int64_t work_items) {
  int64_t b = (work_items + TPB - 1) / TPB;
  if (b > 2048) b = 2048;
  if (b < 1) b = 1;
  return (int)b;
}

template <typename S, typename D>
__global__ __launch_bounds__(TPB) void cast_kernel(const S* __restrict__ src, D* __restrict__ dst, int64_t n) {
  const int64_t n4 = n >> 2;
  for (int64_t i = blockIdx.x * (int64_t)TPB + threadIdx.x; i < n4; i += (int64_t)gridDim.x * TPB) {
    float f[4];
    ld4(src + i * 4, f);
    st4(dst + i * 4, f);
  }
  if (blockIdx.x == 0 && threadIdx.x < (n & 3)) {
    const int64_t i = (n4 << 2) + threadIdx.x;
    DT<D>::st(dst + i, DT<S>::ld(src + i));
  }
}

struct RowScaleSeg { const void* x; const float* scale; void* y; unsigned chunks, cpr, rps; };
struct RowScaleArgs { RowScaleSeg s[2]; unsigned total; };

template <typename T>
__global__ __launch_bounds__(TPB) void row_scale_kernel(const RowScaleArgs a) {
  constexpr int EPC = DT<T>::EPC;
  for (unsigned i = blockIdx.x * TPB + threadIdx.x; i < a.total; i += gridDim.x * TPB) {
    const bool second = i >= a.s[0].chunks;
    const RowScaleSeg& g = a.s[second ? 1 : 0];
    const unsigned j = second ? i - a.s[0].chunks : i;
    const float sc = g.scale[(j / g.cpr) / g.rps];
    float f[EPC];
    chunk_to_f<T>(reinterpret_cast<const uint4*>(g.x)[j], f);
#pragma unroll
    for (int e = 0; e < EPC; ++e) f[e] *= sc;
    reinterpret_cast<uint4*>(g.y)[j] = f_to_chunk<T>(f);
  }
}

template <typename T>
__global__ __launch_bounds__(TPB) void token_mean2_fwd_kernel(const T* __restrict__ x, int L, const T* __restrict__ c, int M, int C, int B,
                                                            T* __restrict__ out, const float* __restrict__ xs = nullptr, const float* __restrict__ xb = nullptr) {
  constexpr int EPC = DT<T>::EPC;
  const int cpr = C / EPC;
  const unsigned i = blockIdx.x * TPB + threadIdx.x;
  if (i >= (unsigned)B * cpr) return;
  const int b = i / cpr, ch = i % cpr;
  float acc[EPC], f[EPC];
#pragma unroll
  for (int e = 0; e < EPC; ++e) acc[e] = 0.f;
  const uint4* px = reinterpret_cast<const uint4*>(x) + (size_t)b * L * cpr + ch;
  int l = 0;
  for (; l + 8 <= L; l += 8) {
    uint4 v[8];
#pragma unroll
    for (int j = 0; j < 8; ++j) v[j] = px[(size_t)(l + j) * cpr];
#pragma unroll
    for (int j = 0; j < 8; ++j) {
      chunk_to_f<T>(v[j], f);
#pragma unroll
      for (int e = 0; e < EPC; ++e) acc[e] += f[e];
    }
  }
  for (; l < L; ++l) {
    chunk_to_f<T>(px[(size_t)l * cpr], f);
#pragma unroll
    for (int e = 0; e < EPC; ++e) acc[e] += f[e];
  }
  const float il = 1.f / (float)L;
#pragma unroll
  for (int e = 0; e < EPC; ++e) acc[e] *= il;
  if (xs) {
#pragma unroll
    for (int e = 0; e < EPC; ++e) acc[e] = fmaf(acc[e], xs[ch * EPC + e], xb[ch * EPC + e]);
  }
  if (c) {
    float a2[EPC];
#pragma unroll
    for (int e = 0; e < EPC; ++e) a2[e] = 0.f;
    const uint4* pc = reinterpret_cast<const uint4*>(c) + (size_t)b * M * cpr + ch;
    int m = 0;
    for (; m + 8 <= M; m += 8) {
      uint4 v[8];
#pragma unroll
      for (int j = 0; j < 8; ++j) v[j] = pc[(size_t)(m + j) * cpr];
#pragma unroll
      for (int j = 0; j < 8; ++j) {
        chunk_to_f<T>(v[j], f);
#pragma unroll
        for (int e = 0; e < EPC; ++e) a2[e] += f[e];
      }
    }
    for (; m < M; ++m) {
      chunk_to_f<T>(pc[(size_t)m * cpr], f);
#pragma unroll
      for (int e = 0; e < EPC; ++e) a2[e] += f[e];
    }
    const float im = 1.f / (float)M;
#pragma unroll
    for (int e = 0; e < EPC; ++e) acc[e] += a2[e] * im;
  }
  reinterpret_cast<uint4*>(out)[i] = f_to_chunk<T>(acc);
}

template <typename T>
__global__ __launch_bounds__(TPB) void token_mean2_bwd_kernel(const T* __restrict__ g, T* __restrict__ dx, int L, T* __restrict__ dc, int M, int C, int B) {
  constexpr int EPC = DT<T>::EPC;
  const int cpr = C / EPC;
  const unsigned tot = (unsigned)B * (L + M) * cpr;
  for (unsigned i = blockIdx.x * TPB + threadIdx.x; i < tot; i += gridDim.x * TPB) {
    const unsigned row = i / cpr, ch = i % cpr;
    const unsigned b = row / (L + M), t = row % (L + M);
    float f[EPC];
    chunk_to_f<T>(reinterpret_cast<const uint4*>(g)[(size_t)b * cpr + ch], f);
    const float sc = t < (unsigned)L ? 1.f / (float)L : 1.f / (float)M;
#pragma unroll
    for (int e = 0; e < EPC; ++e) f[e] *= sc;
    if (t < (unsigned)L) reinterpret_cast<uint4*>(dx)[((size_t)b * L + t) * cpr + ch] = f_to_chunk<T>(f);
    else if (dc) reinterpret_cast<uint4*>(dc)[((size_t)b * M + (t - L)) * cpr + ch] = f_to_chunk<T>(f);
  }
}

template <typename T>
__global__ __launch_bounds__(TPB) void im2col_nhwc_kernel(const T* __restrict__ x, T* __restrict__ out, int B, int H, int W, int C, int Ho, int Wo, int KP) {
  constexpr int EPC = DT<T>::EPC;
  const int cpr = KP / EPC, cpt = C / EPC;
  const int64_t total = (int64_t)B * Ho * Wo * cpr;
  for (int64_t i = blockIdx.x * (int64_t)TPB + threadIdx.x; i < total; i += (int64_t)gridDim.x * TPB) {
    const int j = (int)(i % cpr);
    const int64_t r = i / cpr;
    const int wo = (int)(r % Wo), ho = (int)((r / Wo) % Ho), b = (int)(r / ((int64_t)Wo * Ho));
// ... 562 lines not shown
```

lemevit_amd/csrc/rwmlp.hip:

```cpp
#include <atomic>
#include "common.h"

namespace {

struct RwProb { const bf16_t* x; bf16_t* out; const float* row_scale; int M, rps, wg_begin, nwg; };
struct RwArgs {
  RwProb p[2];
  const bf16_t* w1; const float* s1; const float* b1; const bf16_t* w2; const float* b2;
  int nwg0; float eps;
};

constexpr int RW_C = 96, RW_H = 384, RW_W1ROW = 192, RW_W2ROW = 768;
constexpr int RW_W1_BYTES = RW_H * RW_W1ROW, RW_W2_BYTES = RW_C * RW_W2ROW;
constexpr int RW_LDS = RW_W1_BYTES + RW_W2_BYTES + (2 * RW_H + RW_C) * (int)sizeof(float);

__device__ __forceinline__ int rw_nmap(int t, int i) { return 8 * (i >> 2) + 4 * t + (i & 3); }
__device__ __forceinline__ int rw_swz1(int n) { return (n >> 2) & 3; }
__device__ __forceinline__ int rw_swz2(int c) { return (((c >> 3) & 3) << 2) | (c & 3); }

__device__ __forceinline__ void rw_unpack8(const bf16x8_t& c, float* f) {
  typedef __attribute__((ext_vector_type(4))) unsigned u32x4_t;
  const u32x4_t r = __builtin_bit_cast(u32x4_t, c);
#pragma unroll
  for (int e = 0; e < 4; ++e) { f[2 * e] = __uint_as_float(r[e] << 16); f[2 * e + 1] = __uint_as_float(r[e] & 0xffff0000u); }
// ... 46 lines not shown
    for (int i = 0; i < 9; ++i) {
      const int idx = tid + i * 512, c = idx / 48, c8 = idx - c * 48;
      *reinterpret_cast<uint4*>(sw2 + c * RW_W2ROW + (((c8 & ~15) | ((c8 & 15) ^ rw_swz2(c))) << 4)) = v2[i];
    }
  }
  for (int i = tid; i < RW_H; i += 512) { scs[i] = g.s1[i]; sb1[i] = g.b1[i]; }
  if (tid < RW_C) sb2[tid] = g.b2[tid];
  __syncthreads();

  const int npanels = (P.M + 31) / 32;
  const int gw = ((int)blockIdx.x - P.wg_begin) * 8 + wave, stride = P.nwg * 8;
  const int grp = lane >> 4, li = lane & 15;
  const unsigned lds0 = (unsigned)(uintptr_t)smem;
  unsigned w1off[2], w2off[2];
  int w2x[2];
#pragma unroll
  for (int t = 0; t < 2; ++t) {
    const int n = rw_nmap(t, li);
    w1off[t] = n * RW_W1ROW + ((grp ^ rw_swz1(n)) << 4);
    w2off[t] = n * RW_W2ROW;
    w2x[t] = rw_swz2(n);
  }

  auto load_panel = [&](int pn, bf16x8_t (&af)[2][3]) {
#pragma unroll
    for (int rt = 0; rt < 2; ++rt) {
      const int row = min(pn * 32 + rt * 16 + li, P.M - 1);
      const bf16_t* p = P.x + (long long)row * RW_C + grp * 8;
#pragma unroll
      for (int ks = 0; ks < 3; ++ks) af[rt][ks] = *reinterpret_cast<const bf16x8_t*>(p + ks * 32);
    }
  };

  bf16x8_t cur[2][3], nxt[2][3];
  if (gw < npanels) load_panel(gw, cur);
  for (int pn = gw; pn < npanels; pn += stride) {
    float mean[2], rstd[2], rsc[2];
#pragma unroll
    for (int rt = 0; rt < 2; ++rt) {
      float v[8], s = 0.f;
#pragma unroll
      for (int ks = 0; ks < 3; ++ks) {
        rw_unpack8(cur[rt][ks], v);
#pragma unroll
        for (int e = 0; e < 8; ++e) s += v[e];
      }
      s += __shfl_xor(s, 16, 64); s += __shfl_xor(s, 32, 64);
      mean[rt] = s * (1.f / RW_C);
      float q = 0.f;
#pragma unroll
      for (int ks = 0; ks < 3; ++ks) {
        rw_unpack8(cur[rt][ks], v);
#pragma unroll
        for (int e = 0; e < 8; ++e) { const float d = v[e] - mean[rt]; q = fmaf(d, d, q); }
      }
      q += __shfl_xor(q, 16, 64); q += __shfl_xor(q, 32, 64);
      rstd[rt] = rsqrtf(q * (1.f / RW_C) + g.eps);
      const int row = min(pn * 32 + rt * 16 + li, P.M - 1);
      rsc[rt] = P.row_scale ? P.row_scale[row / P.rps] : 1.f;
    }
    f32x4_t acc2[2][3][2];
#pragma unroll
    for (int rt = 0; rt < 2; ++rt)
#pragma unroll
      for (int s = 0; s < 3; ++s)
#pragma unroll
        for (int t = 0; t < 2; ++t) acc2[rt][s][t] = f32x4_t{0.f, 0.f, 0.f, 0.f};
    bf16x8_t w2f[3][2];
#pragma unroll 1
    for (int hc = 0; hc < RW_H / 32; ++hc) {
      if (hc == 2 && pn + stride < npanels) load_panel(pn + stride, nxt);
      f32x4_t acc1[2][2];
#pragma unroll
      for (int rt = 0; rt < 2; ++rt)
#pragma unroll
        for (int t = 0; t < 2; ++t) acc1[rt][t] = f32x4_t{0.f, 0.f, 0.f, 0.f};
      const unsigned char* w1b = sw1 + hc * 32 * RW_W1ROW;
#pragma unroll
      for (int ks = 0; ks < 3; ++ks) {
        bf16x8_t wf[2];
#pragma unroll
        for (int t = 0; t < 2; ++t) wf[t] = *reinterpret_cast<const bf16x8_t*>(w1b + w1off[t] + ks * 64);
#pragma unroll
        for (int rt = 0; rt < 2; ++rt)
#pragma unroll
          for (int t = 0; t < 2; ++t) acc1[rt][t] = __builtin_amdgcn_mfma_f32_16x16x32_bf16(wf[t], cur[rt][ks], acc1[rt][t], 0, 0, 0);
      }
      const int h0 = hc * 32 + 8 * grp;
      const float4 c0 = *reinterpret_cast<const float4*>(scs + h0), c1 = *reinterpret_cast<const float4*>(scs + h0 + 4);
      const float4 d0 = *reinterpret_cast<const float4*>(sb1 + h0), d1 = *reinterpret_cast<const float4*>(sb1 + h0 + 4);
      const int c8 = hc * 4 + grp;
#pragma unroll
      for (int s = 0; s < 3; ++s)
#pragma unroll
        for (int t = 0; t < 2; ++t) {
          const unsigned a = lds0 + RW_W1_BYTES + s * 32 * RW_W2ROW + w2off[t] + (((c8 & ~15) | ((c8 & 15) ^ w2x[t])) << 4);
          asm volatile("ds_read_b128 %0, %1" : "=v"(w2f[s][t]) : "v"(a) : "memory");
        }
      bf16x8_t hf[2];
      {
        typedef __attribute__((ext_vector_type(4))) unsigned u32x4_t;
#pragma unroll
        for (int rt = 0; rt < 2; ++rt) {
          const float nm = -mean[rt];
          u32x4_t pk;
#pragma unroll
          for (int t = 0; t < 2; ++t) {
            const float4 c4 = t ? c1 : c0, d4 = t ? d1 : d0;
            f32x2_t y0 = f32x2_t{fmaf(rstd[rt], fmaf(nm, c4.x, acc1[rt][t][0]), d4.x), fmaf(rstd[rt], fmaf(nm, c4.y, acc1[rt][t][1]), d4.y)};
            f32x2_t y1 = f32x2_t{fmaf(rstd[rt], fmaf(nm, c4.z, acc1[rt][t][2]), d4.z), fmaf(rstd[rt], fmaf(nm, c4.w, acc1[rt][t][3]), d4.w)};
            rw_gelu2x2(y0, y1);
            pk[2 * t] = pack_bf2(y0[0], y0[1]); pk[2 * t + 1] = pack_bf2(y1[0], y1[1]);
          }
          hf[rt] = __builtin_bit_cast(bf16x8_t, pk);
        }
      }
      asm volatile("s_waitcnt lgkmcnt(0)" ::: "memory");
#pragma unroll
      for (int s = 0; s < 3; ++s)
#pragma unroll
        for (int t = 0; t < 2; ++t) asm volatile("" : "+v"(w2f[s][t]));
#pragma unroll
      for (int rt = 0; rt < 2; ++rt) asm volatile("" : "+v"(hf[rt]));
#pragma unroll
      for (int s = 0; s < 3; ++s)
#pragma unroll
        for (int rt = 0; rt < 2; ++rt)
#pragma unroll
          for (int t = 0; t < 2; ++t) acc2[rt][s][t] = __builtin_amdgcn_mfma_f32_16x16x32_bf16(w2f[s][t], hf[rt], acc2[rt][s][t], 0, 0, 0);
    }
#pragma unroll
    for (int s = 0; s < 3; ++s) {
      const int c0 = s * 32 + 8 * grp;
      const float4 b0 = *reinterpret_cast<const float4*>(sb2 + c0), b1 = *reinterpret_cast<const float4*>(sb2 + c0 + 4);
#pragma unroll
      for (int rt = 0; rt < 2; ++rt) {
        const int row = pn * 32 + rt * 16 + li;
        float xr[8];
        rw_unpack8(cur[rt][s], xr);
        const float v[8] = {fmaf(rsc[rt], acc2[rt][s][0][0] + b0.x, xr[0]), fmaf(rsc[rt], acc2[rt][s][0][1] + b0.y, xr[1]),
                            fmaf(rsc[rt], acc2[rt][s][0][2] + b0.z, xr[2]), fmaf(rsc[rt], acc2[rt][s][0][3] + b0.w, xr[3]),
                            fmaf(rsc[rt], acc2[rt][s][1][0] + b1.x, xr[4]), fmaf(rsc[rt], acc2[rt][s][1][1] + b1.y, xr[5]),
                            fmaf(rsc[rt], acc2[rt][s][1][2] + b1.z, xr[6]), fmaf(rsc[rt], acc2[rt][s][1][3] + b1.w, xr[7])};
        if (row < P.M) *reinterpret_cast<bf16x8_t*>(P.out + (long long)row * RW_C + c0) = rw_pack8(v);
      }
    }
#pragma unroll
    for (int rt = 0; rt < 2; ++rt)
#pragma unroll
      for (int ks = 0; ks < 3; ++ks) cur[rt][ks] = nxt[rt][ks];
  }
}

}

bool lmv_mlp_rw96_eligible(const lmv_mlp_problem* p, int nproblems, int C, int hidden) {
  if (C != RW_C || hidden != RW_H || !lmv_config().mlp_rw96) return false;
  for (int i = 0; i < nproblems; ++i)
    if (p[i].rows <= 0 || p[i].rows > 0x7fffffffLL / 2048) return false;
  return true;
}

int lmv_mlp_rw96_fwd(const lmv_mlp_problem* p, int nproblems, const lmv_mlp_weights* w, float eps, hipStream_t st) {
  RwArgs a{};
  a.w1 = (const bf16_t*)w->w1f; a.s1 = w->colsum1; a.b1 = w->b1f; a.w2 = (const bf16_t*)w->w2; a.b2 = w->b2; a.eps = eps;
  int want[2] = {0, 0}, nwg = 0;
  for (int i = 0; i < nproblems; ++i) { const int panels = (int)((p[i].rows + 31) / 32); want[i] = (panels + 7) / 8; }
  if (want[0] + want[1] > 256) {
    const int small = want[0] <= want[1] ? 0 : 1, big = 1 - small;
    if (want[small] > 128) want[small] = 128;
    want[big] = 256 - want[small];
  }
  for (int i = 0; i < nproblems; ++i) {
    RwProb& q = a.p[i];
    q.x = (const bf16_t*)p[i].x; q.out = (bf16_t*)p[i].out; q.row_scale = p[i].row_scale; q.M = (int)p[i].rows;
    q.rps = p[i].rows_per_sample > 0 ? p[i].rows_per_sample : 1;
    q.wg_begin = nwg; q.nwg = want[i];
    nwg += want[i];
  }
  a.nwg0 = a.p[0].nwg;
  static std::atomic<unsigned long long> attr_done{0};
  int dev = 0;
  (void)hipGetDevice(&dev);
  const unsigned long long bit = 1ull << (dev & 63);
  if (!(attr_done.load(std::memory_order_acquire) & bit)) {
    if (hipFuncSetAttribute(reinterpret_cast<const void*>(rw_mlp96_kernel), hipFuncAttributeMaxDynamicSharedMemorySize, RW_LDS) != hipSuccess)
      LMV_FAIL(LMV_ERR_LAUNCH, "mlp_fused: cannot reserve LDS");
    attr_done.fetch_or(bit, std::memory_order_release);
  }
  hipLaunchKernelGGL(rw_mlp96_kernel, dim3(nwg), dim3(512), RW_LDS, st, a);
  LMV_CHECK_LAUNCH("mlp_fused (resident weights)");
  return LMV_OK;
}
```

lemevit_amd/ops.py:

```python
from __future__ import annotations

import ctypes as C
import math
from typing import List, Optional, Sequence, Tuple

import torch

from . import _lib
from ._lib import ACT_GELU, ACT_GELU_BWD, ACT_GELU_GRAD, ACT_NONE, FOLD_CI_TAP, FOLD_TAP_CI, AttnDesc, LinearProblem, LnSegment, check, lib

Tensor = torch.Tensor
HEAD_DIM = 32


def dtype_code(t: Tensor) -> int:
    if t.dtype == torch.float32:
        return _lib.LMV_F32
    if t.dtype == torch.bfloat16:
        return _lib.LMV_BF16
    raise TypeError(f"lemevit_amd: unsupported dtype {t.dtype} (float32 and bfloat16 only)")


_raw_stream = getattr(torch._C, "_cuda_getCurrentRawStream", None)


def _stream() -> int:
    if _raw_stream is not None:
        return _raw_stream(torch.cuda.current_device())
    return torch.cuda.current_stream().cuda_stream


def _ptr(t: Optional[Tensor]) -> Optional[int]:
    if t is None:
        return None
    if not t.is_cuda:
        raise RuntimeError("lemevit_amd: tensors must be on the GPU (no CPU fallback exists)")
    if not t.is_contiguous():
        raise RuntimeError("lemevit_amd: tensors must be contiguous")
    return t.data_ptr()


_ws_cache = {}


def _workspace(nbytes: int, device, stream: Optional[int] = None) -> Tensor:
    key = (device, _stream() if stream is None else stream)
    ws = _ws_cache.get(key)
    if ws is None or ws.numel() < nbytes:
        if ws is not None and stream is not None:
            ws.record_stream(torch.cuda.ExternalStream(stream, device=device))
        ws = torch.empty(max(int(nbytes * 1.25), 1 << 22), device=device, dtype=torch.uint8)
        _ws_cache[key] = ws
    return ws


def _f32(t: Optional[Tensor]) -> Optional[int]:
    if t is not None and t.dtype != torch.float32:
        raise TypeError("lemevit_amd: vector operands (bias, LN affine, scales, gradient accumulators) must be float32")
    return _ptr(t)


class Prob:
    __slots__ = ("a", "w", "bias", "res", "row_scale", "aux", "out", "out_pre", "bias_grad", "rows", "rps")

    def __init__(self, a, w, out, bias=None, res=None, row_scale=None, aux=None, out_pre=None, bias_grad=None, rps=0):
        self.a, self.w, self.out, self.bias, self.res = a, w, out, bias, res
        self.row_scale, self.aux, self.out_pre, self.bias_grad, self.rps = row_scale, aux, out_pre, bias_grad, rps
        self.rows = a.numel() // a.shape[-1]


def _pack(probs: Sequence[Prob]):
    arr = (LinearProblem * len(probs))()
    for s, p in zip(arr, probs):
        s.a, s.w, s.out = _ptr(p.a), _ptr(p.w), _ptr(p.out)
        s.bias, s.row_scale, s.bias_grad = _f32(p.bias), _f32(p.row_scale), _f32(p.bias_grad)
        s.res, s.aux, s.out_pre = _ptr(p.res), _ptr(p.aux), _ptr(p.out_pre)
        s.rows, s.rows_per_sample = p.rows, p.rps
    return arr


def linear_fwd(probs: Sequence[Prob], N: int, K: int, act: int = ACT_NONE) -> None:
    check(lib.lmv_linear_fwd(_pack(probs), len(probs), N, K, act, dtype_code(probs[0].a), _stream()), "lmv_linear_fwd")


def linear_dx(probs: Sequence[Prob], N: int, K: int, act: int = ACT_NONE) -> None:
    check(lib.lmv_linear_dx(_pack(probs), len(probs), N, K, act, dtype_code(probs[0].a), _stream()), "lmv_linear_dx")


class Folded:
    __slots__ = ("wf", "colsum", "bf")

    def __init__(self, wf, colsum, bf):
        self.wf, self.colsum, self.bf = wf, colsum, bf


def ln_fold(weight: Tensor, bias: Optional[Tensor], gamma: Tensor, beta: Tensor, dtype: torch.dtype) -> Folded:
    N, K = weight.shape
    if weight.dtype != torch.float32:
        raise TypeError("lemevit_amd: ln_fold takes the fp32 master weight")
    wf = torch.empty((N, K), device=weight.device, dtype=dtype)
    colsum = torch.empty(N, device=weight.device, dtype=torch.float32)
    bf = torch.empty(N, device=weight.device, dtype=torch.float32)
    check(lib.lmv_ln_fold(_ptr(weight), _f32(bias), _f32(gamma), _f32(beta), N, K, _ptr(wf), _ptr(colsum), _ptr(bf), dtype_code(wf), _stream()), "lmv_ln_fold")
    return Folded(wf, colsum, bf)


def ln_linear_fwd(probs: Sequence[Prob], N: int, K: int, eps: float, act: int = ACT_NONE) -> None:
    arr = _pack(probs)
    for s, p in zip(arr, probs):
        s.aux = _f32(p.aux)
    check(lib.lmv_ln_linear_fwd(arr, len(probs), N, K, eps, act, dtype_code(probs[0].a), _stream()), "lmv_ln_linear_fwd")


def mlp_fused_supported(C_: int, hidden: int, dtype: torch.dtype) -> bool:
    return dtype == torch.bfloat16 and bool(lib.lmv_mlp_fused_supported(C_, hidden, _lib.LMV_BF16))


def mlp_fused_fwd(xs: Sequence[Tensor], fc1: Folded, w2: Tensor, b2: Tensor, eps: float, scales: Optional[Sequence[Optional[Tensor]]] = None) -> List[Tensor]:
    C_ = xs[0].shape[-1]
    Hd = w2.shape[1]
    outs = [torch.empty_like(x) for x in xs]
    arr = (_lib.MlpProblem * len(xs))()
    for i, (s, x, o) in enumerate(zip(arr, xs, outs)):
        s.x, s.out, s.rows = _ptr(x), _ptr(o), x.numel() // C_
        sc = scales[i] if scales is not None else None
        s.row_scale, s.rows_per_sample = _f32(sc), (x.shape[1] if sc is not None else 0)
    w = _lib.MlpWeights(_ptr(fc1.wf), _f32(fc1.colsum), _f32(fc1.bf), _ptr(w2), _f32(b2))
    check(lib.lmv_mlp_fused_fwd(arr, len(xs), C.byref(w), C_, Hd, eps, dtype_code(xs[0]), _stream()), "lmv_mlp_fused_fwd")
    return outs


def mlp_dx_fused_supported(C_: int, hidden: int, dtype: torch.dtype) -> bool:
    return dtype == torch.bfloat16 and bool(lib.lmv_mlp_dx_fused_supported(C_, hidden, _lib.LMV_BF16))


def mlp_dx_fused(gs: Sequence[Tensor], us: Sequence[Tensor], fc2_wt: Tensor, fc1_wt: Tensor) -> List[Tensor]:
    Hd, C_ = fc2_wt.shape
    if fc1_wt.shape != (C_, Hd) or not fc2_wt.is_contiguous() or not fc1_wt.is_contiguous():
        raise TypeError("mlp_dx_fused: fc2_wt [hidden, C] and fc1_wt [C, hidden], contiguous")
    outs = [torch.empty_like(g) for g in gs]
    arr = (_lib.MlpDxProblem * len(gs))()
    for s, g, u, o in zip(arr, gs, us, outs):
        if not g.is_contiguous() or not u.is_contiguous() or u.numel() // Hd != g.numel() // C_:
            raise TypeError("mlp_dx_fused: contiguous g [rows, C] and u [rows, hidden]")
        s.g, s.u, s.dn2, s.rows = _ptr(g), _ptr(u), _ptr(o), g.numel() // C_
    check(lib.lmv_mlp_dx_fused(arr, len(gs), _ptr(fc2_wt), _ptr(fc1_wt), C_, Hd, dtype_code(gs[0]), _stream()), "lmv_mlp_dx_fused")
    return outs


def wgrad_launches() -> int:
    return int(lib.lmv_debug_wgrad_launches())


def attn_out_proj_residual(probs: Sequence[Prob], C_: int) -> None:
    check(lib.lmv_attn_out_proj_residual(_pack(probs), len(probs), C_, dtype_code(probs[0].a), _stream()), "lmv_attn_out_proj_residual")


def linear_dw(probs: Sequence[Prob], N: int, K: int, stream: Optional[int] = None) -> None:
    arr, code = _pack(probs), dtype_code(probs[0].a)
    st = _stream() if stream is None else stream
    ws = _workspace(lib.lmv_linear_dw_workspace_bytes(arr, len(probs), N, K, code), probs[0].a.device, st)
    check(lib.lmv_linear_dw(arr, len(probs), N, K, ws.data_ptr(), ws.numel(), code, st), "lmv_linear_dw")


def batchnorm_train_fwd(x2d: Tensor, gamma: Tensor, beta: Tensor, running_mean: Optional[Tensor], running_var: Optional[Tensor],
                        momentum: float, eps: float, gelu: bool = False):
    rows, C_ = x2d.shape
    y = torch.empty_like(x2d)
    stats = torch.empty((2, C_), device=x2d.device, dtype=torch.float32)
    ws = _workspace(lib.lmv_batchnorm_workspace_bytes(C_), x2d.device)
    check(lib.lmv_batchnorm_train_fwd(_ptr(x2d), _f32(gamma), _f32(beta), _f32(running_mean), _f32(running_var), momentum, eps, ACT_GELU if gelu else ACT_NONE,
                                      _ptr(y), _f32(stats), rows, C_, ws.data_ptr(), ws.numel(), dtype_code(x2d), _stream()), "lmv_batchnorm_train_fwd")
    return y, stats


def batchnorm_apply_fwd(x2d: Tensor, gamma: Tensor, beta: Tensor, stats: Tensor, gelu: bool = False) -> Tensor:
    rows, C_ = x2d.shape
    y = torch.empty_like(x2d)
    check(lib.lmv_batchnorm_apply_fwd(_ptr(x2d), _f32(gamma), _f32(beta), _f32(stats), ACT_GELU if gelu else ACT_NONE, _ptr(y), rows, C_,
                                      dtype_code(x2d), _stream()), "lmv_batchnorm_apply_fwd")
    return y


def batchnorm_train_bwd(dy2d: Tensor, x2d: Tensor, gamma: Tensor, beta: Tensor, stats: Tensor, gelu: bool = False):
    rows, C_ = x2d.shape
    dx = torch.empty_like(x2d)
    dgamma = torch.empty((C_,), device=x2d.device, dtype=torch.float32)
    dbeta = torch.empty((C_,), device=x2d.device, dtype=torch.float32)
    ws = _workspace(lib.lmv_batchnorm_workspace_bytes(C_), x2d.device)
    check(lib.lmv_batchnorm_train_bwd(_ptr(dy2d), _ptr(x2d), _f32(gamma), _f32(beta), _f32(stats), ACT_GELU if gelu else ACT_NONE, _ptr(dx), _f32(dgamma),
                                      _f32(dbeta), rows, C_, ws.data_ptr(), ws.numel(), dtype_code(x2d), _stream()), "lmv_batchnorm_train_bwd")
    return dx, dgamma, dbeta


def layernorm_fwd_multi(xs: Sequence[Tensor], gamma: Tensor, beta: Tensor, eps: float, want_stats: bool = False, gelu: bool = False):
    C_ = xs[0].shape[-1]
    seg = (LnSegment * len(xs))()
    ys, sts = [], []
    for s, x in zip(seg, xs):
        rows = x.numel() // C_
        y = torch.empty_like(x)
        st = torch.empty((rows, 2), device=x.device, dtype=torch.float32) if want_stats else None
        s.x, s.y, s.stats, s.rows = _ptr(x), _ptr(y), _ptr(st), rows
        ys.append(y); sts.append(st)
    fn = lib.lmv_layernorm_gelu_fwd if gelu else lib.lmv_layernorm_fwd
    check(fn(seg, len(xs), _f32(gamma), _f32(beta), C_, eps, dtype_code(xs[0]), _stream()), "lmv_layernorm_fwd")
    return ys, sts


def layernorm_bwd_multi(dys: Sequence[Tensor], xs: Sequence[Tensor], stats: Sequence[Tensor], gamma: Tensor, dgamma: Tensor, dbeta: Tensor,
                        dres: Sequence[Optional[Tensor]], next_scales: Optional[Sequence[Optional[Tensor]]] = None, gelu_beta: Optional[Tensor] = None,
                        split_reduce: bool = False):
    C_ = xs[0].shape[-1]
    seg = (LnSegment * len(xs))()
    dxs, scaled, total = [], [], 0
    for i, (s, dy, x, st, dr) in enumerate(zip(seg, dys, xs, stats, dres)):
        dx = torch.empty_like(x)
        s.x, s.dy, s.stats, s.dres, s.dx, s.rows = _ptr(x), _ptr(dy), _f32(st), _ptr(dr), _ptr(dx), x.numel() // C_
        sc = None if next_scales is None else next_scales[i]
        if sc is not None:
            d2 = torch.empty_like(x)
            s.dx_scale, s.dx_scaled, s.rows_per_sample = _f32(sc), _ptr(d2), x.shape[1]
            scaled.append(d2)
        else:
            scaled.append(dx)
        total += s.rows
        dxs.append(dx)
    code = dtype_code(xs[0])
    if dgamma is None and dbeta is None:
        if gelu_beta is not None:
            check(lib.lmv_layernorm_gelu_bwd(seg, len(xs), _f32(gamma), _f32(gelu_beta), None, None, C_, None, 0, code, _stream()), "lmv_layernorm_gelu_bwd")
        else:
            check(lib.lmv_layernorm_bwd_partial(seg, len(xs), _f32(gamma), C_, None, 0, None, code, _stream()), "lmv_layernorm_bwd_partial")
        return dxs if next_scales is None else (dxs, scaled)
    ws = _workspace(lib.lmv_layernorm_bwd_workspace_bytes(total, C_, code), xs[0].device)
    if split_reduce:
        rows = C.c_int(0)
        check(lib.lmv_layernorm_bwd_partial(seg, len(xs), _f32(gamma), C_, ws.data_ptr(), ws.numel(), C.byref(rows), code, _stream()), "lmv_layernorm_bwd_partial")
        check(lib.lmv_layernorm_bwd_reduce(ws.data_ptr(), rows.value, C_, _f32(dgamma), _f32(dbeta), _stream()), "lmv_layernorm_bwd_reduce")
        return dxs if next_scales is None else (dxs, scaled)
    if gelu_beta is not None:
        check(lib.lmv_layernorm_gelu_bwd(seg, len(xs), _f32(gamma), _f32(gelu_beta), _f32(dgamma), _f32(dbeta), C_, ws.data_ptr(), ws.numel(), code,
                                         _stream()), "lmv_layernorm_gelu_bwd")
    else:
        check(lib.lmv_layernorm_bwd(seg, len(xs), _f32(gamma), _f32(dgamma), _f32(dbeta), C_, ws.data_ptr(), ws.numel(), code, _stream()),
              "lmv_layernorm_bwd")
    return dxs if next_scales is None else (dxs, scaled)


def ln_exact_fused(N: int, K: int, dtype) -> bool:
    return dtype == torch.bfloat16 and bool(lib.lmv_ln_linear_exact_fwd_supported(N, K, _lib.LMV_BF16))


def ln_linear_exact_fwd(probs: Sequence[Prob], N: int, K: int, gamma: Tensor, beta: Tensor, eps: float, want_stats: bool, want_ln: bool = True):
    arr = _pack(probs)
    seg = (LnSegment * len(probs))()
    ys, sts = [], []
    for s, p in zip(seg, probs):
        y = torch.empty_like(p.a) if want_ln else None
        st = torch.empty((p.rows, 2), device=p.a.device, dtype=torch.float32) if want_stats else None
        s.y, s.stats, s.rows = (_ptr(y) if want_ln else None), _f32(st), p.rows
        ys.append(y); sts.append(st)
    check(lib.lmv_ln_linear_exact_fwd(arr, seg, len(probs), N, K, _f32(gamma), _f32(beta), eps, dtype_code(probs[0].a), _stream()), "lmv_ln_linear_exact_fwd")
    return ys, sts


def res_ln_fused(C_: int, K: int, rows: int, dtype) -> bool:
    return dtype == torch.bfloat16 and 16384 <= rows <= 32768 and bool(lib.lmv_linear_res_ln_fwd_supported(C_, K, _lib.LMV_BF16))


def linear_res_ln_fwd(probs: Sequence[Prob], N: int, K: int, gamma: Tensor, beta: Tensor, eps: float, want_stats: bool):
    arr = _pack(probs)
    seg = (LnSegment * len(probs))()
    ys, sts = [], []
    for s, p in zip(seg, probs):
        y = torch.empty_like(p.out)
        st = torch.empty((p.rows, 2), device=p.out.device, dtype=torch.float32) if want_stats else None
        s.y, s.stats, s.rows = _ptr(y), _f32(st), p.rows
        ys.append(y); sts.append(st)
    check(lib.lmv_linear_res_ln_fwd(arr, seg, len(probs), N, K, _f32(gamma), _f32(beta), eps, dtype_code(probs[0].a), _stream()), "lmv_linear_res_ln_fwd")
    return ys, sts


def linear_dx_ln_bwd(dys: Sequence[Tensor], wt: Tensor, xs: Sequence[Tensor], stats: Sequence[Tensor], gamma: Tensor, dgamma: Tensor, dbeta: Tensor,
                     dres: Sequence[Optional[Tensor]], next_scales: Optional[Sequence[Optional[Tensor]]] = None):
    C_, N = wt.shape
    seg = (LnSegment * len(xs))()
    pr = (LinearProblem * len(xs))()
    dxs, scaled, total = [], [], 0
    for i, (s, q, dy, x, st, dr) in enumerate(zip(seg, pr, dys, xs, stats, dres)):
        dx = torch.empty_like(x)
        s.x, s.stats, s.dres, s.dx, s.rows = _ptr(x), _f32(st), _ptr(dr), _ptr(dx), x.numel() // C_
        q.a, q.w, q.rows = _ptr(dy), _ptr(wt), s.rows
        sc = None if next_scales is None else next_scales[i]
        if sc is not None:
            d2 = torch.empty_like(x)
            s.dx_scale, s.dx_scaled, s.rows_per_sample = _f32(sc), _ptr(d2), x.shape[1]
            scaled.append(d2)
        else:
            scaled.append(dx)
# ... 734 lines not shown
```

Before: 4397 images/sec.

## Add fused LN+MLP train kernels for C=96 stage with fwd and bwd

Adds new persistent kernels for the C=96/hidden=384 stage. The forward kernel fuses LayerNorm, fc1, GELU and fc2 while saving n2, stats, u and h for backward. The backward kernel fuses the MLP data gradient with the LayerNorm backward and writes per-workgroup dgamma/dbeta partials that feed a deferred reduction, while the weight-gradient GEMMs are still issued on the side stream. It is on by default when a stage has at least 8192 rows, and it aims to cut the launches and HBM round-trips between the separate LN, GEMM and activation kernels, at the cost of more LDS use and a grid capped per image chunk.

```diff
diff --git a/include/lemevit_hip.h b/include/lemevit_hip.h
--- a/include/lemevit_hip.h
+++ b/include/lemevit_hip.h
@@ -82,6 +82,27 @@
 typedef struct { const void* g; const void* u; void* dn2; int64_t rows; } lmv_mlp_dx_problem;
 int lmv_mlp_dx_fused_supported(int C, int hidden, int dtype);
 int lmv_mlp_dx_fused(const lmv_mlp_dx_problem* p, int nproblems, const void* fc2_wt, const void* fc1_wt, int C, int hidden, int dtype, void* stream);
+typedef struct {
+  const void* x; void* n2; float* st2; void* u; void* h; void* out;
+  const float* row_scale;
+  int64_t rows;
+  int32_t rows_per_sample;
+  int32_t _pad;
+} lmv_mlp96_fwd_problem;
+typedef struct {
+  const void* dout; const float* ds;
+  const void* u; const void* t2; const float* st2;
+  void* g; void* du; void* dt2;
+  const float* nds; void* g2;
+  int64_t rows;
+  int32_t rows_per_sample;
+  int32_t _pad;
+} lmv_mlp96_bwd_problem;
+typedef struct { const void* fc1_w; const float* fc1_b; const void* fc2_w; const float* fc2_b; const float* gamma; const float* beta; } lmv_mlp96_weights;
+int lmv_mlp96_train_supported(int C, int hidden, int dtype);
+int lmv_mlp96_train_fwd(const lmv_mlp96_fwd_problem* p, int nproblems, const lmv_mlp96_weights* w, float eps, void* stream);
+size_t lmv_mlp96_train_bwd_workspace_bytes(void);
+int lmv_mlp96_train_bwd(const lmv_mlp96_bwd_problem* p, int nproblems, const lmv_mlp96_weights* w, void* workspace, size_t workspace_bytes, int* ws_rows, void* stream);
 int lmv_attn_out_proj_residual(const lmv_linear_problem* p, int nproblems, int C, int dtype, void* stream);
 
 typedef struct {
diff --git a/lemevit_amd/_lib.py b/lemevit_amd/_lib.py
--- a/lemevit_amd/_lib.py
+++ b/lemevit_amd/_lib.py
@@ -31,6 +31,20 @@
 
 class MlpDxProblem(C.Structure):
     _fields_ = [("g", C.c_void_p), ("u", C.c_void_p), ("dn2", C.c_void_p), ("rows", C.c_int64)]
+
+
+class Mlp96FwdProblem(C.Structure):
+    _fields_ = [("x", C.c_void_p), ("n2", C.c_void_p), ("st2", C.c_void_p), ("u", C.c_void_p), ("h", C.c_void_p), ("out", C.c_void_p), ("row_scale", C.c_void_p),
+                ("rows", C.c_int64), ("rows_per_sample", C.c_int32), ("_pad", C.c_int32)]
+
+
+class Mlp96BwdProblem(C.Structure):
+    _fields_ = [("dout", C.c_void_p), ("ds", C.c_void_p), ("u", C.c_void_p), ("t2", C.c_void_p), ("st2", C.c_void_p), ("g", C.c_void_p), ("du", C.c_void_p),
+                ("dt2", C.c_void_p), ("nds", C.c_void_p), ("g2", C.c_void_p), ("rows", C.c_int64), ("rows_per_sample", C.c_int32), ("_pad", C.c_int32)]
+
+
+class Mlp96Weights(C.Structure):
+    _fields_ = [("fc1_w", C.c_void_p), ("fc1_b", C.c_void_p), ("fc2_w", C.c_void_p), ("fc2_b", C.c_void_p), ("gamma", C.c_void_p), ("beta", C.c_void_p)]
 
 
 class MlpWeights(C.Structure):
@@ -125,6 +139,10 @@
     "lmv_mlp_fused_fwd": (_I, [C.POINTER(MlpProblem), _I, C.POINTER(MlpWeights), _I, _I, _F, _I, _P]),
     "lmv_mlp_dx_fused_supported": (_I, [_I, _I, _I]),
     "lmv_mlp_dx_fused": (_I, [C.POINTER(MlpDxProblem), _I, _P, _P, _I, _I, _I, _P]),
+    "lmv_mlp96_train_supported": (_I, [_I, _I, _I]),
+    "lmv_mlp96_train_fwd": (_I, [C.POINTER(Mlp96FwdProblem), _I, C.POINTER(Mlp96Weights), _F, _P]),
+    "lmv_mlp96_train_bwd_workspace_bytes": (_Z, []),
+    "lmv_mlp96_train_bwd": (_I, [C.POINTER(Mlp96BwdProblem), _I, C.POINTER(Mlp96Weights), _P, _Z, C.POINTER(C.c_int), _P]),
     "lmv_attn_out_proj_residual": (_I, [C.POINTER(LinearProblem), _I, _I, _I, _P]),
     "lmv_layernorm_fwd": (_I, [C.POINTER(LnSegment), _I, _P, _P, _I, _F, _I, _P]),
     "lmv_layernorm_gelu_fwd": (_I, [C.POINTER(LnSegment), _I, _P, _P, _I, _F, _I, _P]),
diff --git a/lemevit_amd/csrc/block.hip b/lemevit_amd/csrc/block.hip
--- a/lemevit_amd/csrc/block.hip
+++ b/lemevit_amd/csrc/block.hip
@@ -142,8 +142,27 @@
   return !(fused_on(d, D, save) && !mlp_split384(D));
 }
 
+constexpr int64_t MLP96_TRAIN_MIN_ROWS = 8192;
+inline bool mlp96_train_on(const lmv_block_desc* d, const Dims& D, int s0) {
+  const int mode = lmv_config().mlp96_train;
+  if (mode == 0 || data_only(d) || !lmv_mlp96_train_supported(D.C, D.Hd, D.dtype)) return false;
+  const int64_t rows = (s0 == 0 ? D.rows[0] : 0) + D.rows[1];
+  return mode == 2 || rows >= MLP96_TRAIN_MIN_ROWS;
+}
+thread_local int tl_mlp96_cap = 0;
+
 int mlp_fwd(const lmv_block_desc* d, const Dims& D, const Fwd& f, int s0, void* const* outs, const float* const* ds, int save, void* st, bool ln_done = false) {
   const int ns = 2 - s0;
+  if (save && !ln_done && mlp96_train_on(d, D, s0)) {
+    lmv_mlp96_fwd_problem q[2] = {};
+    for (int i = 0; i < ns; ++i) {
+      const int s = s0 + i;
+      q[i].x = f.t2[s]; q[i].n2 = f.n2[s]; q[i].st2 = f.st2[s]; q[i].u = f.u[s]; q[i].h = f.h[s]; q[i].out = outs[s];
+      q[i].row_scale = ds[s]; q[i].rows = D.rows[s]; q[i].rows_per_sample = s == 0 ? D.N : D.M;
+    }
+    const lmv_mlp96_weights w{d->fc1_w, d->fc1_b, d->fc2_w, d->fc2_b, d->n2_w, d->n2_b};
+    return lmv_mlp96_train_fwd_cap(q, ns, &w, d->eps, tl_mlp96_cap, (hipStream_t)st);
+  }
   const bool split384 = mlp_split384(D);
   if (fused_on(d, D, save) && !split384) {
     if (lmv_mlp_fused_supported(D.C, D.Hd, D.dtype)) {
@@ -303,6 +322,7 @@
   b->ws_conv_bytes = lmv_dwconv3x3_bwd_weight_workspace_bytes(D.B, D.H, D.W, D.C, D.dtype); b->ws_conv = a.take(b->ws_conv_bytes);
   b->ws_ln_bytes = lmv_layernorm_bwd_workspace_bytes(D.rows[0] + D.rows[1], D.C, D.dtype);
   { const size_t w2 = lmv_linear_dx_ln_bwd_workspace_bytes(D.rows[0] + D.rows[1], D.C); if (w2 > b->ws_ln_bytes) b->ws_ln_bytes = w2; }
+  if (lmv_mlp96_train_supported(D.C, D.Hd, D.dtype) && lmv_mlp96_train_bwd_workspace_bytes() > b->ws_ln_bytes) b->ws_ln_bytes = lmv_mlp96_train_bwd_workspace_bytes();
   for (int i = 0; i < 2; ++i) b->ws_ln[i] = a.take(b->ws_ln_bytes);
 }
 
@@ -345,6 +365,32 @@
             const void** g2_out, Side& sd) {
   const int ns = 2 - s0;
   hipStream_t st = sd.main;
+  if (!sd.dataonly && mlp96_train_on(d, D, s0)) {
+    lmv_mlp96_bwd_problem q[2] = {};
+    lmv_linear_problem p[2];
+    const void* gq[2] = {nullptr, nullptr};
+    for (int i = 0; i < ns; ++i) {
+      const int s = s0 + i;
+      q[i].dout = douts[s]; q[i].ds = ds[s]; q[i].u = f.u[s]; q[i].t2 = f.t2[s]; q[i].st2 = f.st2[s];
+      q[i].g = ds[s] ? b.g[s] : nullptr; q[i].du = b.du[s]; q[i].dt2 = b.dt2[s];
+      q[i].rows = D.rows[s]; q[i].rows_per_sample = s == 0 ? D.N : D.M;
+      gq[i] = ds[s] ? b.g[s] : douts[s];
+      g2_out[s] = b.dt2[s];
+      if (nds && nds[s]) { q[i].nds = nds[s]; q[i].g2 = b.g2[s]; g2_out[s] = b.g2[s]; }
+    }
+    const lmv_mlp96_weights w{d->fc1_w, d->fc1_b, d->fc2_w, d->fc2_b, d->n2_w, d->n2_b};
+    int rows = 0;
+    LMV_TRY(lmv_mlp96_train_bwd(q, ns, &w, b.ws_ln[0], b.ws_ln_bytes, &rows, st));
+    if (sd.nsegs + 1 > LMV_REDUCE_MAX_SEGS) LMV_FAIL(LMV_ERR_WORKSPACE, "block_bwd: too many deferred reductions");
+    lmv_reduce_seg& sg = sd.segs[sd.nsegs++];
+    sg = lmv_reduce_seg{};
+    sg.ws = (const float*)b.ws_ln[0]; sg.out_w = d->g_n2_w; sg.out_b = d->g_n2_b; sg.slab_stride = 2 * D.C; sg.nw = D.C; sg.nslabs = rows; sg.nb = D.C;
+    sg.kind = LMV_REDUCE_ROWS; sg.mode = 0;
+    for (int i = 0; i < ns; ++i) { const int s = s0 + i; p[i] = prob(gq[i], f.h[s], d->g_fc2_w, D.rows[s]); p[i].bias_grad = d->g_fc2_b; }
+    LMV_TRY(dw(sd, p, ns, D.C, D.Hd, D.dtype));
+    for (int i = 0; i < ns; ++i) { const int s = s0 + i; p[i] = prob(b.du[s], f.n2[s], d->g_fc1_w, D.rows[s]); p[i].bias_grad = d->g_fc1_b; }
+    return dw(sd, p, ns, D.Hd, D.C, D.dtype);
+  }
   const void* g[2];
   lmv_row_scale_segment rs[2]; int nrs = 0;
   for (int s = s0; s < 2; ++s) {
@@ -483,6 +529,9 @@
   const size_t w0 = fwd_ws_off(DF, image0), w1 = fwd_ws_attn(DF, nimages);
   if (w0 + w1 > f.ws_bytes) LMV_FAIL(LMV_ERR_WORKSPACE, "block_fwd: attention workspace slice [%zu, %zu) outside %zu bytes", w0, w0 + w1, f.ws_bytes);
   f.ws = (unsigned char*)f.ws + w0; f.ws_bytes = w1;
+  struct CapScope { CapScope(int c) { tl_mlp96_cap = c; } ~CapScope() { tl_mlp96_cap = 0; } };
+  const int share = (int)((int64_t)256 * nimages / DF.B);
+  const CapScope cap(share < 32 ? 32 : share);
   return block_fwd_body(&dr, D, f, adv(const_cast<void*>(x), 0, D.C * es), adv(const_cast<void*>(c), 1, D.C * es), adv(x_out, 0, D.C * es), adv(c_out, 1, D.C * es), save, stream);
 }
 
diff --git a/lemevit_amd/csrc/common.h b/lemevit_amd/csrc/common.h
--- a/lemevit_amd/csrc/common.h
+++ b/lemevit_amd/csrc/common.h
@@ -25,7 +25,7 @@
 void lmv_timing_end(void* stream);
 void lmv_timing_set_kind(int kind);
 enum { LMV_TK_GEMM_NT = 0, LMV_TK_SSTAGE = 1, LMV_TK_DSTAGE = 2, LMV_TK_STEM = 3, LMV_TK_GEMM_DX = 4, LMV_TK_GEMM_DW = 5, LMV_TK_SPLITK_REDUCE = 6, LMV_TK_ATTN_FWD = 7,
-       LMV_TK_RS_GEMM = 8, LMV_TK_WN_GEMM = 9, LMV_TK_ATTN_BWD = 10, LMV_TK_RSW_GEMM = 11, LMV_TK_MLP_DX = 12 };
+       LMV_TK_RS_GEMM = 8, LMV_TK_WN_GEMM = 9, LMV_TK_ATTN_BWD = 10, LMV_TK_RSW_GEMM = 11, LMV_TK_MLP_DX = 12, LMV_TK_MLP96_FWD = 13, LMV_TK_MLP96_BWD = 14 };
 struct LmvTimedLaunch {
   void* st; bool on;
   LmvTimedLaunch(void* stream, double flops, double bytes, int kind = 0) : st(stream), on(g_lmv_timing_on) { if (on) lmv_timing_begin(st, flops, bytes, kind); }
@@ -82,6 +82,8 @@
   int mlp_rw96 = 1;
   int mlp_tm = 0;
   int mlp_dx_fused = 1;
+  int mlp96_train = 1;
+  int mlp96_max_wg = 0;
   int stage_ticket_skew = 0;
 };
 LmvConfig& lmv_config();
@@ -91,6 +93,7 @@
 bool lmv_wn_eligible(const lmv_linear_problem* p, int nproblems, int N, int K, int act, bool force);
 bool lmv_mlp_rw96_eligible(const lmv_mlp_problem* p, int nproblems, int C, int hidden);
 int lmv_mlp_rw96_fwd(const lmv_mlp_problem* p, int nproblems, const lmv_mlp_weights* w, float eps, hipStream_t st);
+int lmv_mlp96_train_fwd_cap(const lmv_mlp96_fwd_problem* p, int nproblems, const lmv_mlp96_weights* w, float eps, int cap, hipStream_t st);
 int lmv_wn_linear(const lmv_linear_problem* p, int nproblems, int N, int K, int act, hipStream_t st);
 int lmv_gelu_bwd_linear(const lmv_linear_problem* p, int nproblems, int N, int K, int dtype, hipStream_t st);
 
diff --git a/lemevit_amd/csrc/misc.hip b/lemevit_amd/csrc/misc.hip
--- a/lemevit_amd/csrc/misc.hip
+++ b/lemevit_amd/csrc/misc.hip
@@ -113,6 +113,7 @@
 struct ConfigKey { const char* key; int LmvConfig::*field; };
 const ConfigKey kConfigKeys[] = {
     {"gemm_rs", &LmvConfig::gemm_rs}, {"gemm_wn", &LmvConfig::gemm_wn}, {"mlp_rw96", &LmvConfig::mlp_rw96}, {"mlp_tm", &LmvConfig::mlp_tm}, {"mlp_dx_fused", &LmvConfig::mlp_dx_fused},
+    {"mlp96_train", &LmvConfig::mlp96_train}, {"mlp96_max_wg", &LmvConfig::mlp96_max_wg},
     {"stage_ticket_skew", &LmvConfig::stage_ticket_skew},
 };
 LmvConfig g_config;
diff --git a/lemevit_amd/csrc/rwmlp.hip b/lemevit_amd/csrc/rwmlp.hip
--- a/lemevit_amd/csrc/rwmlp.hip
+++ b/lemevit_amd/csrc/rwmlp.hip
@@ -222,6 +222,555 @@
   }
 }
 
+struct RtFwdProb { const bf16_t* x; bf16_t *n2, *u, *h, *out; float* st2; const float* row_scale; int M, rps, wg_begin, nwg; };
+struct RtFwdArgs {
+  RtFwdProb p[2];
+  const bf16_t *w1, *w2; const float *b1, *b2, *gamma, *beta;
+  int nwg0; float eps;
+};
+struct RtBwdProb { const bf16_t *dout, *u, *t2; const float *st2, *ds, *nds; bf16_t *g, *du, *dt2, *g2; int M, rps, wg_begin, nwg; };
+struct RtBwdArgs {
+  RtBwdProb p[2];
+  const bf16_t *w1, *w2; const float* gamma; float* partial;
+  int nwg0;
+};
+constexpr int RT_LDS_FWD = RW_W1_BYTES + RW_W2_BYTES + (RW_H + 3 * RW_C) * (int)sizeof(float);
+constexpr int RT_LDS_BWD = RW_W1_BYTES + RW_W2_BYTES + RW_C * (int)sizeof(float);
+
+template <typename V> __device__ __forceinline__ V rt_ld(const void* base, unsigned byte_off) { return *reinterpret_cast<const V*>(reinterpret_cast<const char*>(base) + byte_off); }
+template <typename V> __device__ __forceinline__ void rt_st(void* base, unsigned byte_off, const V& v) { *reinterpret_cast<V*>(reinterpret_cast<char*>(base) + byte_off) = v; }
+__device__ __forceinline__ unsigned rw_w1_byte(int n, int c) { return n * RW_W1ROW + (((c & ~3) | ((c & 3) ^ rw_swz1(n))) << 4); }
+__device__ __forceinline__ unsigned rw_w2_byte(int c, int c8) { return c * RW_W2ROW + (((c8 & ~15) | ((c8 & 15) ^ rw_swz2(c))) << 4); }
+
+__global__ __launch_bounds__(512, 1) void rw_mlp96_train_fwd_kernel(const RtFwdArgs g) {
+  extern __shared__ __attribute__((aligned(16))) unsigned char smem[];
+  const int tid = threadIdx.x, lane = tid & 63, wave = tid >> 6;
+  const bool second = (int)blockIdx.x >= g.nwg0;
+  RtFwdProb P;
+#define RW_SEL(f) P.f = second ? g.p[1].f : g.p[0].f
+  RW_SEL(x); RW_SEL(n2); RW_SEL(u); RW_SEL(h); RW_SEL(out); RW_SEL(st2); RW_SEL(row_scale); RW_SEL(M); RW_SEL(rps); RW_SEL(wg_begin); RW_SEL(nwg);
+#undef RW_SEL
+  unsigned char* const sw1 = smem;
+  float* const sb1 = reinterpret_cast<float*>(smem + RW_W1_BYTES + RW_W2_BYTES);
+  float* const sb2 = sb1 + RW_H;
+  float* const sga = sb2 + RW_C;
+  float* const sbe = sga + RW_C;
+  {
+    uint4 v1[9], v2[9];
+#pragma unroll
+    for (int i = 0; i < 9; ++i) v1[i] = *reinterpret_cast<const uint4*>(g.w1 + (long long)(tid + i * 512) * 8);
+#pragma unroll
+    for (int i = 0; i < 9; ++i) v2[i] = *reinterpret_cast<const uint4*>(g.w2 + (long long)(tid + i * 512) * 8);
+#pragma unroll
+    for (int i = 0; i < 9; ++i) { const int idx = tid + i * 512, n = idx / 12; *reinterpret_cast<uint4*>(smem + rw_w1_byte(n, idx - n * 12)) = v1[i]; }
+#pragma unroll
+    for (int i = 0; i < 9; ++i) { const int idx = tid + i * 512, c = idx / 48; *reinterpret_cast<uint4*>(smem + RW_W1_BYTES + rw_w2_byte(c, idx - c * 48)) = v2[i]; }
+  }
+  if (tid < RW_H) sb1[tid] = g.b1[tid];
+  if (tid < RW_C) { sb2[tid] = g.b2[tid]; sga[tid] = g.gamma[tid]; sbe[tid] = g.beta[tid]; }
+  __syncthreads();
+
+  const int npanels = (P.M + 31) / 32;
+  const int gw = ((int)blockIdx.x - P.wg_begin) * 8 + wave, stride = P.nwg * 8;
+  const int grp = lane >> 4, li = lane & 15;
+  const unsigned lds0 = (unsigned)(uintptr_t)smem;
+  unsigned w1off[2], w2off[2];
+  int w2x[2];
+#pragma unroll
+  for (int t = 0; t < 2; ++t) {
+    const int n = rw_nmap(t, li);
+    w1off[t] = n * RW_W1ROW + ((grp ^ rw_swz1(n)) << 4);
+    w2off[t] = n * RW_W2ROW;
+    w2x[t] = rw_swz2(n);
+  }
+  auto load_panel = [&](int pn, bf16x8_t (&af)[2][3]) {
+#pragma unroll
+    for (int rt = 0; rt < 2; ++rt) {
+      const int row = min(pn * 32 + rt * 16 + li, P.M - 1);
+      const unsigned off = (unsigned)row * (RW_C * 2) + grp * 16;
+#pragma unroll
+      for (int ks = 0; ks < 3; ++ks) af[rt][ks] = rt_ld<bf16x8_t>(P.x, off + ks * 64);
+    }
+  };
+
+  bf16x8_t cur[2][3], nxt[2][3];
+  if (gw < npanels) load_panel(gw, cur);
+  for (int pn = gw; pn < npanels; pn += stride) {
+    bf16x8_t nrm[2][3];
+    float rsc[2];
+#pragma unroll
+    for (int rt = 0; rt < 2; ++rt) {
+      float v[3][8], s = 0.f;
+#pragma unroll
+      for (int ks = 0; ks < 3; ++ks) {
+        rw_unpack8(cur[rt][ks], v[ks]);
+        float t = 0.f;
+#pragma unroll
+        for (int e = 0; e < 8; ++e) t += v[ks][e];
+        s += t;
+      }
+      s += __shfl_xor(s, 32, 64); s += __shfl_xor(s, 16, 64);
+      const float mean = s * (1.f / (float)RW_C);
+      float q = 0.f;
+#pragma unroll
+      for (int ks = 0; ks < 3; ++ks) {
+        float t = 0.f;
+#pragma unroll
+        for (int e = 0; e < 8; ++e) { const float d = v[ks][e] - mean; t += d * d; }
+        q += t;
+      }
+      q += __shfl_xor(q, 32, 64); q += __shfl_xor(q, 16, 64);
+      const float rstd = 1.f / sqrtf(q * (1.f / (float)RW_C) + g.eps);
+      const int row = pn * 32 + rt * 16 + li, rowc = min(row, P.M - 1);
+      rsc[rt] = P.row_scale ? P.row_scale[rowc / P.rps] : 1.f;
+      if (grp == 0 && row < P.M) rt_st(P.st2, (unsigned)row * 8, make_float2(mean, rstd));
+#pragma unroll
+      for (int ks = 0; ks < 3; ++ks) {
+        const int c0 = ks * 32 + 8 * grp;
+        const float4 g0 = *reinterpret_cast<const float4*>(sga + c0), g1 = *reinterpret_cast<const float4*>(sga + c0 + 4);
+        const float4 e0 = *reinterpret_cast<const float4*>(sbe + c0), e1 = *reinterpret_cast<const float4*>(sbe + c0 + 4);
+        const float gg[8] = {g0.x, g0.y, g0.z, g0.w, g1.x, g1.y, g1.z, g1.w}, bb[8] = {e0.x, e0.y, e0.z, e0.w, e1.x, e1.y, e1.z, e1.w};
+        float o[8];
+#pragma unroll
+        for (int e = 0; e < 8; ++e) o[e] = (v[ks][e] - mean) * rstd * gg[e] + bb[e];
+        nrm[rt][ks] = rw_pack8(o);
+        if (row < P.M) rt_st(P.n2, ((unsigned)row * RW_C + c0) * 2, nrm[rt][ks]);
+      }
+    }
+    f32x4_t acc2[2][3][2];
+#pragma unroll
+    for (int rt = 0; rt < 2; ++rt)
+#pragma unroll
+      for (int s = 0; s < 3; ++s)
+#pragma unroll
+        for (int t = 0; t < 2; ++t) acc2[rt][s][t] = f32x4_t{0.f, 0.f, 0.f, 0.f};
+    bf16x8_t w2f[3][2];
+#pragma unroll 1
+    for (int hc = 0; hc < RW_H / 32; ++hc) {
+      if (hc == 2 && pn + stride < npanels) load_panel(pn + stride, nxt);
+      f32x4_t acc1[2][2];
+#pragma unroll
+      for (int rt = 0; rt < 2; ++rt)
+#pragma unroll
+        for (int t = 0; t < 2; ++t) acc1[rt][t] = f32x4_t{0.f, 0.f, 0.f, 0.f};
+      const unsigned char* w1b = sw1 + hc * 32 * RW_W1ROW;
+#pragma unroll
+      for (int ks = 0; ks < 3; ++ks) {
+        bf16x8_t wf[2];
+#pragma unroll
+        for (int t = 0; t < 2; ++t) wf[t] = *reinterpret_cast<const bf16x8_t*>(w1b + w1off[t] + ks * 64);
+#pragma unroll
+        for (int rt = 0; rt < 2; ++rt)
+#pragma unroll
+          for (int t = 0; t < 2; ++t) acc1[rt][t] = __builtin_amdgcn_mfma_f32_16x16x32_bf16(wf[t], nrm[rt][ks], acc1[rt][t], 0, 0, 0);
+      }
+      const int h0 = hc * 32 + 8 * grp;
+      const float4 d0 = *reinterpret_cast<const float4*>(sb1 + h0), d1 = *reinterpret_cast<const float4*>(sb1 + h0 + 4);
+      const int c8 = hc * 4 + grp;
+#pragma unroll
+      for (int s = 0; s < 3; ++s)
+#pragma unroll
+        for (int t = 0; t < 2; ++t) {
+          const unsigned a = lds0 + RW_W1_BYTES + s * 32 * RW_W2ROW + w2off[t] + (((c8 & ~15) | ((c8 & 15) ^ w2x[t])) << 4);
+          asm volatile("ds_read_b128 %0, %1" : "=v"(w2f[s][t]) : "v"(a) : "memory");
+        }
+      bf16x8_t hf[2];
+#pragma unroll
+      for (int rt = 0; rt < 2; ++rt) {
+        const float pre[8] = {acc1[rt][0][0] + d0.x, acc1[rt][0][1] + d0.y, acc1[rt][0][2] + d0.z, acc1[rt][0][3] + d0.w,
+                              acc1[rt][1][0] + d1.x, acc1[rt][1][1] + d1.y, acc1[rt][1][2] + d1.z, acc1[rt][1][3] + d1.w};
+        float act[8];
+#pragma unroll
+        for (int e = 0; e < 8; ++e) act[e] = gelu_fast_f(pre[e]);
+        hf[rt] = rw_pack8(act);
+        const int row = pn * 32 + rt * 16 + li;
+        if (row < P.M) {
+          rt_st(P.u, ((unsigned)row * RW_H + h0) * 2, rw_pack8(pre));
+          rt_st(P.h, ((unsigned)row * RW_H + h0) * 2, hf[rt]);
+        }
+      }
+      asm volatile("s_waitcnt lgkmcnt(0)" ::: "memory");
+#pragma unroll
+      for (int s = 0; s < 3; ++s)
+#pragma unroll
+        for (int t = 0; t < 2; ++t) asm volatile("" : "+v"(w2f[s][t]));
+#pragma unroll
+      for (int rt = 0; rt < 2; ++rt) asm volatile("" : "+v"(hf[rt]));
+#pragma unroll
+      for (int s = 0; s < 3; ++s)
+#pragma unroll
+        for (int rt = 0; rt < 2; ++rt)
+#pragma unroll
+          for (int t = 0; t < 2; ++t) acc2[rt][s][t] = __builtin_amdgcn_mfma_f32_16x16x32_bf16(w2f[s][t], hf[rt], acc2[rt][s][t], 0, 0, 0);
+    }
+#pragma unroll
+    for (int s = 0; s < 3; ++s) {
+      const int c0 = s * 32 + 8 * grp;
+      const float4 b0 = *reinterpret_cast<const float4*>(sb2 + c0), b1 = *reinterpret_cast<const float4*>(sb2 + c0 + 4);
+#pragma unroll
+      for (int rt = 0; rt < 2; ++rt) {
+        const int row = pn * 32 + rt * 16 + li;
+        float xr[8];
+        rw_unpack8(cur[rt][s], xr);
+        const float v[8] = {fmaf(rsc[rt], acc2[rt][s][0][0] + b0.x, xr[0]), fmaf(rsc[rt], acc2[rt][s][0][1] + b0.y, xr[1]),
+                            fmaf(rsc[rt], acc2[rt][s][0][2] + b0.z, xr[2]), fmaf(rsc[rt], acc2[rt][s][0][3] + b0.w, xr[3]),
+                            fmaf(rsc[rt], acc2[rt][s][1][0] + b1.x, xr[4]), fmaf(rsc[rt], acc2[rt][s][1][1] + b1.y, xr[5]),
+                            fmaf(rsc[rt], acc2[rt][s][1][2] + b1.z, xr[6]), fmaf(rsc[rt], acc2[rt][s][1][3] + b1.w, xr[7])};
+        if (row < P.M) rt_st(P.out, ((unsigned)row * RW_C + c0) * 2, rw_pack8(v));
+      }
+    }
+#pragma unroll
+    for (int rt = 0; rt < 2; ++rt)
+#pragma unroll
+      for (int ks = 0; ks < 3; ++ks) cur[rt][ks] = nxt[rt][ks];
+  }
+}
+
+__global__ __launch_bounds__(512, 1) void rw_mlp96_train_bwd_kernel(const RtBwdArgs g) {
+  extern __shared__ __attribute__((aligned(16))) unsigned char smem[];
+  const int tid = threadIdx.x, lane = tid & 63, wave = tid >> 6;
+  const bool second = (int)blockIdx.x >= g.nwg0;
+  RtBwdProb P;
+#define RW_SEL(f) P.f = second ? g.p[1].f : g.p[0].f
+  RW_SEL(dout); RW_SEL(u); RW_SEL(t2); RW_SEL(st2); RW_SEL(ds); RW_SEL(nds); RW_SEL(g); RW_SEL(du); RW_SEL(dt2); RW_SEL(g2); RW_SEL(M); RW_SEL(rps); RW_SEL(wg_begin); RW_SEL(nwg);
+#undef RW_SEL
+  unsigned char* const sw1 = smem;
+  float* const sga = reinterpret_cast<float*>(smem + RW_W1_BYTES + RW_W2_BYTES);
+  {
+    uint4 v1[9], v2[9];
+#pragma unroll
+    for (int i = 0; i < 9; ++i) { const int idx = tid + i * 512, cc = idx / RW_H, n = idx - cc * RW_H; v1[i] = *reinterpret_cast<const uint4*>(g.w1 + (n * 12 + cc) * 8); }
+#pragma unroll
+    for (int i = 0; i < 9; ++i) { const int idx = tid + i * 512, c8 = idx / RW_C, c = idx - c8 * RW_C; v2[i] = *reinterpret_cast<const uint4*>(g.w2 + (c * 48 + c8) * 8); }
+#pragma unroll
+    for (int i = 0; i < 9; ++i) {
+      const int idx = tid + i * 512, cc = idx / RW_H, n = idx - cc * RW_H;
+      const unsigned w[4] = {v1[i].x, v1[i].y, v1[i].z, v1[i].w};
+#pragma unroll
+      for (int j = 0; j < 8; ++j)
+        *reinterpret_cast<bf16_t*>(smem + RW_W1_BYTES + rw_w2_byte(8 * cc + j, n >> 3) + (n & 7) * 2) = (bf16_t)((j & 1) ? (w[j >> 1] >> 16) : (w[j >> 1] & 0xffffu));
+    }
+#pragma unroll
+    for (int i = 0; i < 9; ++i) {
+      const int idx = tid + i * 512, c8 = idx / RW_C, c = idx - c8 * RW_C;
+      const unsigned w[4] = {v2[i].x, v2[i].y, v2[i].z, v2[i].w};
+#pragma unroll
+      for (int j = 0; j < 8; ++j)
+        *reinterpret_cast<bf16_t*>(smem + rw_w1_byte(8 * c8 + j, c >> 3) + (c & 7) * 2) = (bf16_t)((j & 1) ? (w[j >> 1] >> 16) : (w[j >> 1] & 0xffffu));
+    }
+  }
+  if (tid < RW_C) sga[tid] = g.gamma[tid];
+  __syncthreads();
+
+  const int npanels = (P.M + 31) / 32;
+  const int gw = ((int)blockIdx.x - P.wg_begin) * 8 + wave, stride = P.nwg * 8;
+  const int grp = lane >> 4, li = lane & 15;
+  const unsigned lds0 = (unsigned)(uintptr_t)smem;
+  unsigned w1off[2], w2off[2];
+  int w2x[2];
+#pragma unroll
+  for (int t = 0; t < 2; ++t) {
+    const int n = rw_nmap(t, li);
+    w1off[t] = n * RW_W1ROW + ((grp ^ rw_swz1(n)) << 4);
+    w2off[t] = n * RW_W2ROW;
+    w2x[t] = rw_swz2(n);
+  }
+  auto load_rows = [&](const bf16_t* base, int pn, bf16x8_t (&af)[2][3]) {
+#pragma unroll
+    for (int rt = 0; rt < 2; ++rt) {
+      const int row = min(pn * 32 + rt * 16 + li, P.M - 1);
+      const unsigned off = (unsigned)row * (RW_C * 2) + grp * 16;
+#pragma unroll
+      for (int ks = 0; ks < 3; ++ks) af[rt][ks] = rt_ld<bf16x8_t>(base, off + ks * 64);
+    }
+  };
+  auto load_u = [&](int pn, int hc, bf16x8_t (&uf)[2]) {
+#pragma unroll
+    for (int rt = 0; rt < 2; ++rt) {
+      const int row = min(pn * 32 + rt * 16 + li, P.M - 1);
+      uf[rt] = rt_ld<bf16x8_t>(P.u, ((unsigned)row * RW_H + hc * 32 + 8 * grp) * 2);
+    }
+  };
+
+  float adg[3][8], adb[3][8];
+#pragma unroll
+  for (int s = 0; s < 3; ++s)
+#pragma unroll
+    for (int e = 0; e < 8; ++e) { adg[s][e] = 0.f; adb[s][e] = 0.f; }
+
+  bf16x8_t gB[2][3], nxt[2][3];
+  if (gw < npanels) load_rows(P.dout, gw, gB);
+  for (int pn = gw; pn < npanels; pn += stride) {
+    bf16x8_t ucur[2], unx[2];
+    load_u(pn, 0, ucur);
+    if (P.ds) {
+#pragma unroll
+      for (int rt = 0; rt < 2; ++rt) {
+        const int row = pn * 32 + rt * 16 + li;
+        const float sc = P.ds[min(row, P.M - 1) / P.rps];
+#pragma unroll
+        for (int ks = 0; ks < 3; ++ks) {
+          float v[8];
+          rw_unpack8(gB[rt][ks], v);
+#pragma unroll
+          for (int e = 0; e < 8; ++e) v[e] *= sc;
+          gB[rt][ks] = rw_pack8(v);
+          if (row < P.M) rt_st(P.g, ((unsigned)row * RW_C + ks * 32 + 8 * grp) * 2, gB[rt][ks]);
+        }
+      }
+    }
+    f32x4_t acc2[2][3][2];
+#pragma unroll
+    for (int rt = 0; rt < 2; ++rt)
+#pragma unroll
+      for (int s = 0; s < 3; ++s)
+#pragma unroll
+        for (int t = 0; t < 2; ++t) acc2[rt][s][t] = f32x4_t{0.f, 0.f, 0.f, 0.f};
+    bf16x8_t w2f[3][2];
+#pragma unroll 1
+    for (int hc = 0; hc < RW_H / 32; ++hc) {
+      if (hc == 2 && pn + stride < npanels) load_rows(P.dout, pn + stride, nxt);
+      load_u(pn, min(hc + 1, RW_H / 32 - 1), unx);
+      f32x4_t acc1[2][2];
+#pragma unroll
+      for (int rt = 0; rt < 2; ++rt)
+#pragma unroll
+        for (int t = 0; t < 2; ++t) acc1[rt][t] = f32x4_t{0.f, 0.f, 0.f, 0.f};
+      const unsigned char* w1b = sw1 + hc * 32 * RW_W1ROW;
+#pragma unroll
+      for (int ks = 0; ks < 3; ++ks) {
+        bf16x8_t wf[2];
+#pragma unroll
+        for (int t = 0; t < 2; ++t) wf[t] = *reinterpret_cast<const bf16x8_t*>(w1b + w1off[t] + ks * 64);
+#pragma unroll
+        for (int rt = 0; rt < 2; ++rt)
+#pragma unroll
+          for (int t = 0; t < 2; ++t) acc1[rt][t] = __builtin_amdgcn_mfma_f32_16x16x32_bf16(wf[t], gB[rt][ks], acc1[rt][t], 0, 0, 0);
+      }
+      const int h0 = hc * 32 + 8 * grp;
+      const int c8 = hc * 4 + grp;
+#pragma unroll
+      for (int s = 0; s < 3; ++s)
+#pragma unroll
+        for (int t = 0; t < 2; ++t) {
+          const unsigned a = lds0 + RW_W1_BYTES + s * 32 * RW_W2ROW + w2off[t] + (((c8 & ~15) | ((c8 & 15) ^ w2x[t])) << 4);
+          asm volatile("ds_read_b128 %0, %1" : "=v"(w2f[s][t]) : "v"(a) : "memory");
+        }
+      bf16x8_t hf[2];
+#pragma unroll
+      for (int rt = 0; rt < 2; ++rt) {
+        float uv[8];
+        rw_unpack8(ucur[rt], uv);
+        const float d[8] = {acc1[rt][0][0] * gelu_grad_fast_f(uv[0]), acc1[rt][0][1] * gelu_grad_fast_f(uv[1]), acc1[rt][0][2] * gelu_grad_fast_f(uv[2]),
+                            acc1[rt][0][3] * gelu_grad_fast_f(uv[3]), acc1[rt][1][0] * gelu_grad_fast_f(uv[4]), acc1[rt][1][1] * gelu_grad_fast_f(uv[5]),
+                            acc1[rt][1][2] * gelu_grad_fast_f(uv[6]), acc1[rt][1][3] * gelu_grad_fast_f(uv[7])};
+        hf[rt] = rw_pack8(d);
+        const int row = pn * 32 + rt * 16 + li;
+        if (row < P.M) rt_st(P.du, ((unsigned)row * RW_H + h0) * 2, hf[rt]);
+        ucur[rt] = unx[rt];
+      }
+      asm volatile("s_waitcnt lgkmcnt(0)" ::: "memory");
+#pragma unroll
+      for (int s = 0; s < 3; ++s)
+#pragma unroll
+        for (int t = 0; t < 2; ++t) asm volatile("" : "+v"(w2f[s][t]));
+#pragma unroll
+      for (int rt = 0; rt < 2; ++rt) asm volatile("" : "+v"(hf[rt]));
+#pragma unroll
+      for (int s = 0; s < 3; ++s)
+#pragma unroll
+        for (int rt = 0; rt < 2; ++rt)
+#pragma unroll
+          for (int t = 0; t < 2; ++t) acc2[rt][s][t] = __builtin_amdgcn_mfma_f32_16x16x32_bf16(w2f[s][t], hf[rt], acc2[rt][s][t], 0, 0, 0);
+    }
+    load_rows(P.t2, pn, gB);
+    bf16x8_t dor[2][3];
+    load_rows(P.dout, pn, dor);
+#pragma unroll
+    for (int rt = 0; rt < 2; ++rt) {
+      const int row = pn * 32 + rt * 16 + li, rowc = min(row, P.M - 1);
+      const float2 ms = rt_ld<float2>(P.st2, (unsigned)rowc * 8);
+      const float vm = row < P.M ? 1.f : 0.f;
+      float xh[3][8], ge[3][8], s1 = 0.f, s2 = 0.f;
+#pragma unroll
+      for (int s = 0; s < 3; ++s) {
+        const int c0 = s * 32 + 8 * grp;
+        const float4 g0 = *reinterpret_cast<const float4*>(sga + c0), g1 = *reinterpret_cast<const float4*>(sga + c0 + 4);
+        const float gg[8] = {g0.x, g0.y, g0.z, g0.w, g1.x, g1.y, g1.z, g1.w};
+        float xv[8];
+        rw_unpack8(gB[rt][s], xv);
+#pragma unroll
+        for (int e = 0; e < 8; ++e) {
+          const float dv = acc2[rt][s][e >> 2][e & 3] * vm;
+          xh[s][e] = (xv[e] - ms.x) * ms.y;
+          ge[s][e] = dv * gg[e];
+          s1 += ge[s][e]; s2 += ge[s][e] * xh[s][e];
+          adg[s][e] += dv * xh[s][e]; adb[s][e] += dv;
+        }
+      }
+      s1 += __shfl_xor(s1, 32, 64); s1 += __shfl_xor(s1, 16, 64);
+      s2 += __shfl_xor(s2, 32, 64); s2 += __shfl_xor(s2, 16, 64);
+      s1 *= (1.f / (float)RW_C); s2 *= (1.f / (float)RW_C);
+      const float nsc = P.nds ? P.nds[rowc / P.rps] : 1.f;
+#pragma unroll
+      for (int s = 0; s < 3; ++s) {
+        float o[8], r[8];
+        rw_unpack8(dor[rt][s], r);
+#pragma unroll
+        for (int e = 0; e < 8; ++e) o[e] = ms.y * (ge[s][e] - s1 - xh[s][e] * s2) + r[e];
+        if (row < P.M) {
+          const unsigned off = ((unsigned)row * RW_C + s * 32 + 8 * grp) * 2;
+          rt_st(P.dt2, off, rw_pack8(o));
+          if (P.nds) {
+#pragma unroll
+            for (int e = 0; e < 8; ++e) o[e] *= nsc;
+            rt_st(P.g2, off, rw_pack8(o));
+          }
+        }
+      }
+    }
+#pragma unroll
+    for (int rt = 0; rt < 2; ++rt)
+#pragma unroll
+      for (int ks = 0; ks < 3; ++ks) gB[rt][ks] = nxt[rt][ks];
+  }
+  if (!g.partial) return;
+  __syncthreads();
+  float* const red = reinterpret_cast<float*>(smem);
+  {
+    float* w = red + (wave * 16 + li) * (2 * RW_C);
+#pragma unroll
+    for (int s = 0; s < 3; ++s) {
+      const int c0 = s * 32 + 8 * grp;
+      *reinterpret_cast<float4*>(w + c0) = make_float4(adg[s][0], adg[s][1], adg[s][2], adg[s][3]);
+      *reinterpret_cast<float4*>(w + c0 + 4) = make_float4(adg[s][4], adg[s][5], adg[s][6], adg[s][7]);
+      *reinterpret_cast<float4*>(w + RW_C + c0) = make_float4(adb[s][0], adb[s][1], adb[s][2], adb[s][3]);
+      *reinterpret_cast<float4*>(w + RW_C + c0 + 4) = make_float4(adb[s][4], adb[s][5], adb[s][6], adb[s][7]);
+    }
+  }
+  __syncthreads();
+  if (tid < 2 * RW_C) {
+    float s = 0.f;
+    for (int r = 0; r < 128; ++r) s += red[r * (2 * RW_C) + tid];
+    g.partial[(long long)blockIdx.x * (2 * RW_C) + tid] = s;
+  }
+}
+
+void rw_split(const int64_t* rows, int n, int cap, int* want) {
+  want[0] = want[1] = 0;
+  for (int i = 0; i < n; ++i) { const int panels = (int)((rows[i] + 31) / 32); want[i] = (panels + 7) / 8; }
+  if (want[0] + want[1] > cap) {
+    if (n == 1) { want[0] = cap; return; }
+    const int small = want[0] <= want[1] ? 0 : 1, big = 1 - small;
+    if (want[small] > cap / 2) want[small] = cap / 2;
+    want[big] = cap - want[small];
+  }
+}
+int rw_train_cap(int callers = 0) {
+  int c = lmv_config().mlp96_max_wg;
+  if (c <= 0) c = callers;
+  return c > 0 ? (c < 2 ? 2 : c > 256 ? 256 : c) : 256;
+}
+template <typename K> int rw_reserve_lds(K kernel, int bytes, std::atomic<unsigned long long>& done) {
+  int dev = 0;
+  (void)hipGetDevice(&dev);
+  const unsigned long long bit = 1ull << (dev & 63);
+  if (!(done.load(std::memory_order_acquire) & bit)) {
+    if (hipFuncSetAttribute(reinterpret_cast<const void*>(kernel), hipFuncAttributeMaxDynamicSharedMemorySize, bytes) != hipSuccess)
+      LMV_FAIL(LMV_ERR_LAUNCH, "mlp96_train: cannot reserve LDS");
+    done.fetch_or(bit, std::memory_order_release);
+  }
+  return LMV_OK;
+}
+
+}
+
+extern "C" int lmv_mlp96_train_supported(int C, int hidden, int dtype) { return C == RW_C && hidden == RW_H && dtype == LMV_BF16; }
+extern "C" size_t lmv_mlp96_train_bwd_workspace_bytes(void) { return (size_t)256 * 2 * RW_C * sizeof(float); }
+
+extern "C" int lmv_mlp96_train_fwd(const lmv_mlp96_fwd_problem* p, int nproblems, const lmv_mlp96_weights* w, float eps, void* stream) {
+  return lmv_mlp96_train_fwd_cap(p, nproblems, w, eps, 0, (hipStream_t)stream);
+}
+
+int lmv_mlp96_train_fwd_cap(const lmv_mlp96_fwd_problem* p, int nproblems, const lmv_mlp96_weights* w, float eps, int cap, hipStream_t stream) {
+  if (nproblems < 1 || nproblems > 2 || !p || !w) LMV_FAIL(LMV_ERR_SHAPE, "mlp96_train_fwd: nproblems must be 1 or 2");
+  const void* wp[] = {w->fc1_w, w->fc1_b, w->fc2_w, w->fc2_b, w->gamma, w->beta};
+  for (const void* q : wp) if (!q || !lmv_aligned16(q)) LMV_FAIL(LMV_ERR_SHAPE, "mlp96_train_fwd: null / misaligned parameter");
+  int64_t rows[2] = {0, 0};
+  for (int i = 0; i < nproblems; ++i) {
+    const lmv_mlp96_fwd_problem& q = p[i];
+    if (q.rows <= 0 || q.rows > 0x7fffffffLL / 2048) LMV_FAIL(LMV_ERR_SHAPE, "mlp96_train_fwd: bad rows %lld", (long long)q.rows);
+    const void* tp[] = {q.x, q.n2, q.st2, q.u, q.h, q.out};
+    for (const void* t : tp) if (!t || !lmv_aligned16(t)) LMV_FAIL(LMV_ERR_SHAPE, "mlp96_train_fwd: x / n2 / st2 / u / h / out must be non-null and 16-byte aligned");
+    if (q.row_scale && q.rows_per_sample <= 0) LMV_FAIL(LMV_ERR_SHAPE, "mlp96_train_fwd: row_scale needs rows_per_sample");
+    rows[i] = q.rows;
+  }
+  hipStream_t st = stream;
+  RtFwdArgs a{};
+  a.w1 = (const bf16_t*)w->fc1_w; a.b1 = w->fc1_b; a.w2 = (const bf16_t*)w->fc2_w; a.b2 = w->fc2_b; a.gamma = w->gamma; a.beta = w->beta; a.eps = eps;
+  int want[2], nwg = 0;
+  rw_split(rows, nproblems, rw_train_cap(cap), want);
+  double trows = 0.;
+  for (int i = 0; i < nproblems; ++i) {
+    RtFwdProb& q = a.p[i];
+    q.x = (const bf16_t*)p[i].x; q.n2 = (bf16_t*)p[i].n2; q.st2 = p[i].st2; q.u = (bf16_t*)p[i].u; q.h = (bf16_t*)p[i].h; q.out = (bf16_t*)p[i].out;
+    q.row_scale = p[i].row_scale; q.M = (int)p[i].rows; q.rps = p[i].rows_per_sample > 0 ? p[i].rows_per_sample : 1;
+    q.wg_begin = nwg; q.nwg = want[i];
+    nwg += want[i];
+    trows += (double)p[i].rows;
+  }
+  a.nwg0 = a.p[0].nwg;
+  static std::atomic<unsigned long long> attr_done{0};
+  { const int rc = rw_reserve_lds(rw_mlp96_train_fwd_kernel, RT_LDS_FWD, attr_done); if (rc) return rc; }
+  LmvTimedLaunch tl(stream, 4.0 * trows * RW_C * RW_H, trows * (2.0 * (3 * RW_C + 2 * RW_H) + 8.0) + 4.0 * RW_C * RW_H, LMV_TK_MLP96_FWD);
+  hipLaunchKernelGGL(rw_mlp96_train_fwd_kernel, dim3(nwg), dim3(512), RT_LDS_FWD, st, a);
+  LMV_CHECK_LAUNCH("mlp96_train_fwd");
+  return LMV_OK;
+}
+
+extern "C" int lmv_mlp96_train_bwd(const lmv_mlp96_bwd_problem* p, int nproblems, const lmv_mlp96_weights* w, void* workspace, size_t workspace_bytes, int* ws_rows,
+                                   void* stream) {
+  if (nproblems < 1 || nproblems > 2 || !p || !w) LMV_FAIL(LMV_ERR_SHAPE, "mlp96_train_bwd: nproblems must be 1 or 2");
+  const void* wp[] = {w->fc1_w, w->fc2_w, w->gamma};
+  for (const void* q : wp) if (!q || !lmv_aligned16(q)) LMV_FAIL(LMV_ERR_SHAPE, "mlp96_train_bwd: null / misaligned parameter");
+  int64_t rows[2] = {0, 0};
+  for (int i = 0; i < nproblems; ++i) {
+    const lmv_mlp96_bwd_problem& q = p[i];
+    if (q.rows <= 0 || q.rows > 0x7fffffffLL / 2048) LMV_FAIL(LMV_ERR_SHAPE, "mlp96_train_bwd: bad rows %lld", (long long)q.rows);
+    const void* tp[] = {q.dout, q.u, q.t2, q.st2, q.du, q.dt2};
+    for (const void* t : tp) if (!t || !lmv_aligned16(t)) LMV_FAIL(LMV_ERR_SHAPE, "mlp96_train_bwd: dout / u / t2 / st2 / du / dt2 must be non-null and 16-byte aligned");
+    if ((q.ds && (!q.g || !lmv_aligned16(q.g))) || (q.nds && (!q.g2 || !lmv_aligned16(q.g2)))) LMV_FAIL(LMV_ERR_SHAPE, "mlp96_train_bwd: ds needs g, nds needs g2 (16-byte aligned)");
+    if ((q.ds || q.nds) && q.rows_per_sample <= 0) LMV_FAIL(LMV_ERR_SHAPE, "mlp96_train_bwd: ds / nds need rows_per_sample");
+    rows[i] = q.rows;
+  }
+  hipStream_t st = (hipStream_t)stream;
+  RtBwdArgs a{};
+  a.w1 = (const bf16_t*)w->fc1_w; a.w2 = (const bf16_t*)w->fc2_w; a.gamma = w->gamma;
+  int want[2], nwg = 0;
+  rw_split(rows, nproblems, rw_train_cap(), want);
+  double trows = 0., tbytes = 4.0 * RW_C * RW_H;
+  for (int i = 0; i < nproblems; ++i) {
+    RtBwdProb& q = a.p[i];
+    q.dout = (const bf16_t*)p[i].dout; q.u = (const bf16_t*)p[i].u; q.t2 = (const bf16_t*)p[i].t2; q.st2 = p[i].st2; q.ds = p[i].ds; q.nds = p[i].nds;
+    q.g = (bf16_t*)p[i].g; q.du = (bf16_t*)p[i].du; q.dt2 = (bf16_t*)p[i].dt2; q.g2 = (bf16_t*)p[i].g2;
+    q.M = (int)p[i].rows; q.rps = p[i].rows_per_sample > 0 ? p[i].rows_per_sample : 1;
+    q.wg_begin = nwg; q.nwg = want[i];
+    nwg += want[i];
+    trows += (double)p[i].rows;
+    tbytes += (double)p[i].rows * (2.0 * (3 * RW_C + 2 * RW_H + (p[i].ds ? RW_C : 0) + (p[i].nds ? RW_C : 0)) + 8.0);
+  }
+  a.nwg0 = a.p[0].nwg;
+  if (workspace) {
+    if (workspace_bytes < (size_t)nwg * 2 * RW_C * sizeof(float) || !lmv_aligned16(workspace)) LMV_FAIL(LMV_ERR_WORKSPACE, "mlp96_train_bwd: workspace %zu bytes for %d rows", workspace_bytes, nwg);
+    a.partial = (float*)workspace;
+  }
+  if (ws_rows) *ws_rows = workspace ? nwg : 0;
+  static std::atomic<unsigned long long> attr_done{0};
+  { const int rc = rw_reserve_lds(rw_mlp96_train_bwd_kernel, RT_LDS_BWD, attr_done); if (rc) return rc; }
+  LmvTimedLaunch tl(stream, 4.0 * trows * RW_C * RW_H, tbytes, LMV_TK_MLP96_BWD);
+  hipLaunchKernelGGL(rw_mlp96_train_bwd_kernel, dim3(nwg), dim3(512), RT_LDS_BWD, st, a);
+  LMV_CHECK_LAUNCH("mlp96_train_bwd");
+  return LMV_OK;
 }
 
 bool lmv_mlp_rw96_eligible(const lmv_mlp_problem* p, int nproblems, int C, int hidden) {
diff --git a/lemevit_amd/ops.py b/lemevit_amd/ops.py
--- a/lemevit_amd/ops.py
+++ b/lemevit_amd/ops.py
@@ -146,6 +146,66 @@
         s.g, s.u, s.dn2, s.rows = _ptr(g), _ptr(u), _ptr(o), g.numel() // C_
     check(lib.lmv_mlp_dx_fused(arr, len(gs), _ptr(fc2_wt), _ptr(fc1_wt), C_, Hd, dtype_code(gs[0]), _stream()), "lmv_mlp_dx_fused")
     return outs
+
+
+def mlp96_train_supported(C_: int, hidden: int, dtype: torch.dtype) -> bool:
+    return dtype == torch.bfloat16 and bool(lib.lmv_mlp96_train_supported(C_, hidden, _lib.LMV_BF16))
+
+
+def _mlp96_weights(fc1_w, fc1_b, fc2_w, fc2_b, gamma, beta):
+    if tuple(fc1_w.shape) != (384, 96) or tuple(fc2_w.shape) != (96, 384) or fc1_w.dtype != torch.bfloat16 or fc2_w.dtype != torch.bfloat16:
+        raise TypeError("mlp96_train: bf16 fc1_w [384, 96] and fc2_w [96, 384]")
+    return _lib.Mlp96Weights(_ptr(fc1_w), _f32(fc1_b), _ptr(fc2_w), _f32(fc2_b), _f32(gamma), _f32(beta))
+
+
+def mlp96_train_fwd(xs: Sequence[Tensor], gamma: Tensor, beta: Tensor, fc1_w: Tensor, fc1_b: Tensor, fc2_w: Tensor, fc2_b: Tensor, eps: float,
+                    scales: Optional[Sequence[Optional[Tensor]]] = None):
+    res = []
+    arr = (_lib.Mlp96FwdProblem * len(xs))()
+    for i, (s, x) in enumerate(zip(arr, xs)):
+        rows = x.numel() // 96
+        out, n2 = torch.empty_like(x), torch.empty_like(x)
+        st2 = torch.empty((rows, 2), device=x.device, dtype=torch.float32)
+        u = torch.empty(tuple(x.shape[:-1]) + (384,), device=x.device, dtype=x.dtype)
+        h = torch.empty_like(u)
+        sc = scales[i] if scales is not None else None
+        s.x, s.n2, s.st2, s.u, s.h, s.out, s.rows = _ptr(x), _ptr(n2), _ptr(st2), _ptr(u), _ptr(h), _ptr(out), rows
+        s.row_scale, s.rows_per_sample = _f32(sc), (x.shape[1] if sc is not None else 0)
+        res.append((out, n2, st2, u, h))
+    if dtype_code(xs[0]) != _lib.LMV_BF16:
+        raise TypeError("mlp96_train_fwd: bf16 only")
+    w = _mlp96_weights(fc1_w, fc1_b, fc2_w, fc2_b, gamma, beta)
+    check(lib.lmv_mlp96_train_fwd(arr, len(xs), C.byref(w), eps, _stream()), "lmv_mlp96_train_fwd")
+    return res
+
+
+def mlp96_train_bwd(douts: Sequence[Tensor], us: Sequence[Tensor], t2s: Sequence[Tensor], st2s: Sequence[Tensor], gamma: Tensor, fc1_w: Tensor, fc2_w: Tensor,
+                    dgamma: Optional[Tensor], dbeta: Optional[Tensor], scales: Optional[Sequence[Optional[Tensor]]] = None,
+                    next_scales: Optional[Sequence[Optional[Tensor]]] = None):
+    res = []
+    arr = (_lib.Mlp96BwdProblem * len(douts))()
+    for i, (s, d, u, t2, st2) in enumerate(zip(arr, douts, us, t2s, st2s)):
+        rows = d.numel() // 96
+        ds = scales[i] if scales is not None else None
+        nds = next_scales[i] if next_scales is not None else None
+        g = torch.empty_like(d) if ds is not None else None
+        g2 = torch.empty_like(d) if nds is not None else None
+        du, dt2 = torch.empty_like(u), torch.empty_like(d)
+        s.dout, s.ds, s.u, s.t2, s.st2 = _ptr(d), _f32(ds), _ptr(u), _ptr(t2), _f32(st2)
+        s.g, s.du, s.dt2, s.nds, s.g2 = _ptr(g), _ptr(du), _ptr(dt2), _f32(nds), _ptr(g2)
+        s.rows, s.rows_per_sample = rows, (d.shape[1] if (ds is not None or nds is not None) else 0)
+        res.append((d if g is None else g, du, dt2, g2))
+    if dtype_code(douts[0]) != _lib.LMV_BF16:
+        raise TypeError("mlp96_train_bwd: bf16 only")
+    w = _lib.Mlp96Weights(_ptr(fc1_w), None, _ptr(fc2_w), None, _f32(gamma), None)
+    if dgamma is None:
+        check(lib.lmv_mlp96_train_bwd(arr, len(douts), C.byref(w), None, 0, None, _stream()), "lmv_mlp96_train_bwd")
+        return res
+    ws = _workspace(lib.lmv_mlp96_train_bwd_workspace_bytes(), douts[0].device)
+    rows = C.c_int(0)
+    check(lib.lmv_mlp96_train_bwd(arr, len(douts), C.byref(w), ws.data_ptr(), ws.numel(), C.byref(rows), _stream()), "lmv_mlp96_train_bwd")
+    check(lib.lmv_layernorm_bwd_reduce(ws.data_ptr(), rows.value, 96, _f32(dgamma), _f32(dbeta), _stream()), "lmv_layernorm_bwd_reduce")
+    return res
 
 
 def wgrad_launches() -> int:
```

Measured after the change: 4439 images/sec (median of 4 runs). No clear change (+0.9%).
